# DiltheyLab/HLA-LA

Measured on AMD Instinct MI355X. Metric: paired reads/sec aligned to PRG graph, higher is better.
Workload: dtype int32

## Files before the change

hla-la_amd/csrc/batch.h:

```cpp
#pragma once
#include "device_common.h"

namespace hlala {

struct DevBatch {
    int n_pairs, n_reads, n_chains, stride;
    int from_seeds;
    int unpaired;
    const int* read_off;
    const uint8_t* read_bases;
    const uint8_t* read_quals;
    const int* chain_off;
    const int* read_primary;
    const int* chain_read;
    const int* chain_contig;
    const int* chain_pos;
    const int* chain_offset;
    const int* chain_as;
    const uint8_t* chain_reverse;
    const int* cigar_off;
    const u32* cigar;
    int* seed_status;
    int* seed_ncols;
    int* seed_begin;
    int* seed_end;
    int* seed_removed;
    int* seed_level;
    int* seed_edge;
    uint8_t* seed_g;
    uint8_t* seed_s;
    int* ext_status;
    int* ext_ncols;
    int* ext_begin;
    int* ext_end;
    double* ext_ll;
    int* dp_iters;
    int* dp_score;
    int* dp_ncols;
    int* dp_sb;
    int* dp_se;
    int* dp_err;
    int* dp_alias_head;
    int* dp_alias_next;
    int* ext_level;
    int* ext_edge;
    uint8_t* ext_g;
    uint8_t* ext_s;
    uint8_t* ext_fromseed;
    int* ext_firstlast;
    int* pair_status;
    int* best_chain;
    int* n_comb;
    double* pair_ll;
    double* pair_mapq;
    double* mate_mapq;
    uint8_t* strands_valid;
    uint8_t* sel_mapq;
    u64* counters;
    int* work_counter;
    int* retry_list;
    int* pair_multi;
    uint8_t* pair_deferred;
    int* chain_order;
    int* chain_bucket;
    int* order_hist;
    int order_shift, order_nb;
    int long_chunk_nodes, long_max_segs;
    int order_cost;
    int* chain_row;
    int n_rows;
    int* dp_blk;
    int* dp_list;
    int dp_nblk;
    int dp_band;
    int dp_band_risky;
    int dp_jf;
    void* dp_items;
    int* dbg;
};

__device__ __forceinline__ int ordered_chains(const DevBatch& B) { return B.chain_order ? __builtin_amdgcn_readfirstlane(B.order_hist[B.order_nb - 1]) : B.n_chains; }

__device__ __forceinline__ size_t row_base(const DevBatch& B, int c) { return (size_t)(B.chain_row ? B.chain_row[c] : c) * (size_t)B.stride; }

enum { DPL_BAND16 = 0, DPL_BAND32 = 2, DPL_BAND64 = 4, DPL_JF = 6, DPL_GEN = 8, DPL_N = 10 };
__host__ __device__ inline int dpl_of_class(int cls) { return cls == 0 ? DPL_GEN : (cls == 1 ? DPL_JF : (cls == 2 ? DPL_BAND16 : (cls == 3 ? DPL_BAND32 : DPL_BAND64))); }
enum { WC_PAIR_MULTI = 40, WC_BAND_FETCH = 48, WC_FO_COUNT = 54, WC_FO_FETCH = 56, WC_BAND_FAILED = 58, WC_BAND_CALLS = 59, WC_JF_FAILED = 60, WC_BAND_WHY = 62, WC_BAND_TIED = 68,
       WC_N = 88 };
constexpr int BAND_MAXJ16 = 15, BAND_MAXJ32 = 31, BAND_MAXJ64 = 48;

enum {
    CNT_CHAINS_EXT = 0, CNT_DP_CALLS, CNT_DP_ITERS, CNT_DP_CELLS, CNT_SEED_COLS, CNT_OUT_COLS, CNT_EDGES, CNT_ERRORS, CNT_DP_SHARED
};

}
```

hla-la_amd/csrc/device_common.h:

```cpp
#pragma once
#include <hip/hip_runtime.h>
#include <stdint.h>

namespace hlala {

typedef unsigned long long u64;
typedef unsigned int u32;

struct DevGraph {
    int L, N, E, P;
    const int* level_off;
    const int* node_level;
    const int* node_orig;
    const int* out_off;
    const int* out_to;
    const uint8_t* out_label;
    const int* out_eid;
    const int* in_off;
    const int* in_from;
    const uint8_t* in_label;
    const int* in_eid;
    const unsigned int* in_rec;
    const uint8_t* level_fast;
    const int* edge_from_new;
    const int* edge_to_new;
    const uint8_t* edge_label;
    const int* jf_off; const int* jf_node; const int* jf_path; const int* jf_lvl;
    const int* jb_off; const int* jb_node; const int* jb_path; const int* jb_lvl;
    const uint8_t* out_prank; const uint8_t* in_prank; const uint8_t* jf_prank; const uint8_t* jb_prank;
    const uint8_t* jfree_out; const uint8_t* jfree_in;
    const u32* lin_label; const uint8_t* lin_out; const uint8_t* lin_in; const int* lin_eid;
    const int4* nrec_out;
    const int4* nrec_in;
    const int* path_len;
    const long long* path_off;
    const int* path_edges;
    const uint8_t* gap_stretch;
    const long long* lp_off;
    const int* lp_seqid;
    const int* lp_pos;
};

struct DevTables {
    double ll_match[256];
    double ll_mismatch[256];
    double rate_indel;
    double rate_ins_quarter;
    double rate_match_mismatch;
    double is_penalty;
    int    is_dmin, is_n;
    const double* is_logpdf;
    double phred_thr[256];
    double pcorrect[256];
};

constexpr int DP_WCAP      = 128;
constexpr int DP_HC        = 512;
constexpr int DP_SEQCAP    = 1024;
constexpr int DP_CELLS     = 16384;
constexpr int DP_EARLY     = 4096;
constexpr int DP_STEPS     = 8192;
constexpr int DP_COMPLETED = 2048;
constexpr int DP_CELLS_LARGE     = 65536;
constexpr int DP_COMPLETED_LARGE = 16384;
constexpr int DP_MAX_PARALLEL = 127;
constexpr int DP_NEG       = -30000;

__device__ __forceinline__ int lane_id() { return threadIdx.x & 63; }
#define HLALA_AS_GLOBAL __attribute__((address_space(1)))
template <class T> struct GPtr {
    typedef HLALA_AS_GLOBAL T GT;
    T* p;
    __device__ __forceinline__ GPtr& operator=(T* q) { p = q; return *this; }
    __device__ __forceinline__ GT* g() const { return (GT*)p; }
    __device__ __forceinline__ GT& operator[](int i) const { return g()[i]; }
    __device__ __forceinline__ GT& operator[](unsigned i) const { return g()[i]; }
    __device__ __forceinline__ GT& operator[](long long i) const { return g()[i]; }
    __device__ __forceinline__ GT& operator[](size_t i) const { return g()[i]; }
    __device__ __forceinline__ operator GT*() const { return g(); }
};
template <class T> __device__ __forceinline__ HLALA_AS_GLOBAL T* glob(T* p) { return (HLALA_AS_GLOBAL T*)p; }
#define WSYNC() do { __builtin_amdgcn_fence(__ATOMIC_RELEASE, "wavefront"); __builtin_amdgcn_wave_barrier(); __builtin_amdgcn_fence(__ATOMIC_ACQUIRE, "wavefront"); } while(0)
__device__ __forceinline__ int uni(int v) { return __builtin_amdgcn_readfirstlane(v); }
__device__ __forceinline__ int next_work(int* counter)
{
    int w = 0;
    if(lane_id() == 0) w = atomicAdd(counter, 1);
    return __builtin_amdgcn_readfirstlane(w);
}

template <int CTRL>
__device__ __forceinline__ int dpp_mov(int oldv, int v) { return __builtin_amdgcn_update_dpp(oldv, v, CTRL, 0xF, 0xF, false); }
#define HLALA_DPP_REDUCE(v, IDENT, OP)                                                     \
    do {                                                                                    \
        int t_;                                                                             \
        t_ = dpp_mov<0x111>(IDENT, v); v = OP(v, t_);                        \
        t_ = dpp_mov<0x112>(IDENT, v); v = OP(v, t_);                        \
        t_ = dpp_mov<0x114>(IDENT, v); v = OP(v, t_);                        \
        t_ = dpp_mov<0x118>(IDENT, v); v = OP(v, t_);                        \
        t_ = __builtin_amdgcn_update_dpp(IDENT, v, 0x142, 0xA, 0xF, false); v = OP(v, t_);   \
        t_ = __builtin_amdgcn_update_dpp(IDENT, v, 0x143, 0xC, 0xF, false); v = OP(v, t_);   \
    } while(0)
__device__ __forceinline__ int op_max_(int a, int b) { return a > b ? a : b; }
__device__ __forceinline__ int op_add_(int a, int b) { return a + b; }
__device__ __forceinline__ int wave_max_i32(int v)
{
    HLALA_DPP_REDUCE(v, (int)0x80000000, op_max_);
    return __builtin_amdgcn_readlane(v, 63);
}
__device__ __forceinline__ int wave_sum_i32(int v)
{
    HLALA_DPP_REDUCE(v, 0, op_add_);
    return __builtin_amdgcn_readlane(v, 63);
}
__device__ __forceinline__ u64 wave_min_u64(u64 v)
{
    int hi = (int)(~(u32)(v >> 32) ^ 0x80000000u);
    int mh = wave_max_i32(hi);
    int lo = (hi == mh) ? (int)(~(u32)v ^ 0x80000000u) : (int)0x80000000;
    int ml = wave_max_i32(lo);
    return ((u64)(~((u32)mh ^ 0x80000000u)) << 32) | (u64)(~((u32)ml ^ 0x80000000u));
}
__device__ inline double exp_cr_nonpos(double x)
{
#pragma clang fp contract(off)
    if(!(x < 0.0)) return 1.0;
    if(x < -700.0) return exp(x);
    const double n = rint(x * 0x1.71547652b82fep+0);
    const double r0 = fma(-n, 0x1.62e42fee00000p-1, x);
    const double t1 = n * 0x1.a39ef35600000p-33;
    double rh = r0 - t1; double bb = rh - r0; double rl = (r0 - (rh - bb)) + (-t1 - bb);
    const double t2 = n * 0x1.93c7673007e5fp-65;
    { double s = rh - t2; double b2 = s - rh; double e = (rh - (s - b2)) + (-t2 - b2); e += rl; rh = s + e; rl = e - (rh - s); }
    const double ch[25] = {0x1.0000000000000p+0, 0x1.0000000000000p+0, 0x1.0000000000000p-1, 0x1.5555555555555p-3, 0x1.5555555555555p-5, 0x1.1111111111111p-7, 0x1.6c16c16c16c17p-10,
        0x1.a01a01a01a01ap-13, 0x1.a01a01a01a01ap-16, 0x1.71de3a556c734p-19, 0x1.27e4fb7789f5cp-22, 0x1.ae64567f544e4p-26, 0x1.1eed8eff8d898p-29, 0x1.6124613a86d09p-33,
        0x1.93974a8c07c9dp-37, 0x1.ae7f3e733b81fp-41, 0x1.ae7f3e733b81fp-45, 0x1.952c77030ad4ap-49, 0x1.6827863b97d97p-53, 0x1.2f49b46814157p-57, 0x1.e542ba4020225p-62,
        0x1.71b8ef6dcf572p-66, 0x1.0ce396db7f853p-70, 0x1.761b41316381ap-75, 0x1.f2cf01972f578p-80};
    const double cl[25] = {0.0, 0.0, 0.0, 0x1.5555555555555p-57, 0x1.5555555555555p-59, 0x1.1111111111111p-63, -0x1.f49f49f49f49fp-65, 0x1.a01a01a01a01ap-73, 0x1.a01a01a01a01ap-76,
        -0x1.c154f8ddc6c00p-73, 0x1.cbbc05b4fa99ap-76, -0x1.c062e06d1f209p-80, -0x1.2aec959e14c06p-83, 0x1.f28e0cc748ebep-87, 0x1.05d6f8a2efd1fp-92, 0x1.1d8656b0ee8cbp-97,
        0x1.1d8656b0ee8cbp-101, 0x1.ac981465ddc6cp-103, 0x1.eec01221a8b0bp-107, 0x1.2650f61dbdcb4p-112, 0x1.ea72b4afe3c2fp-120, -0x1.d043ae40c4647p-120, -0x1.aebcdbd20331cp-124,
        -0x1.3423c7d91404fp-130, -0x1.9ada5fcc1ab14p-135};
    double ph = ch[24], pl = cl[24];
#pragma unroll
    for(int k = 23; k >= 0; k--) {
        const double m = ph * rh; double e = fma(ph, rh, -m); e = fma(ph, rl, e); e = fma(pl, rh, e);
        double mh = m + e; double ml = e - (mh - m);
        const double s = mh + ch[k]; const double b2 = s - mh; double e2 = (mh - (s - b2)) + (ch[k] - b2); e2 += ml + cl[k];
        ph = s + e2; pl = e2 - (ph - s);
    }
    return ldexp(ph, (int)n);
}

__device__ __forceinline__ unsigned long long wave_sum_u64(unsigned long long v)
{
    for(int o = 32; o > 0; o >>= 1) {
        const unsigned lo = (unsigned)__shfl_xor((int)(unsigned)v, o), hi = (unsigned)__shfl_xor((int)(unsigned)(v >> 32), o);
        v += ((unsigned long long)hi << 32) | lo;
    }
    return v;
}

__device__ __forceinline__ int wave_incl_scan_add(int v) { HLALA_DPP_REDUCE(v, 0, op_add_); return v; }
__device__ __forceinline__ int wave_incl_scan_max(int v) { HLALA_DPP_REDUCE(v, (int)0x80000000, op_max_); return v; }
__device__ __forceinline__ int wave_excl_scan(int v, int& total)
// ... 31 lines not shown
```

hla-la_amd/csrc/hlala_api.hip:

```cpp
#include <cmath>
#include <cstdio>
#include <cstring>
#include <cstdlib>
#include <algorithm>
#include <map>
#include <mutex>
#include <chrono>
#include <thread>
#include <set>
#include <string>
#include <unordered_map>
#include <vector>

#include "../../include/hlala_gpu.h"
#include "batch.h"
#include "flat_graph.hpp"
#include "host_internal.h"

#include "kernel_dp.hip"
#include "kernel_project.hip"
#include "kernel_order.hip"
#include "kernel_pair.hip"
#include "kernel_typer.hip"
#include "kernel_call.hip"
// ... 739 lines not shown
    for(int k = 0; k < nc; k++) {
        int n = in->col_off[k + 1] - in->col_off[k];
        if(in->chain_read[k] < 0 || in->chain_read[k] >= nr) { c->err = "chain_read out of range"; return fail(HLALA_E_ARG); }
        if(n > stride || n < 1) { st[k] = HLALA_CHAIN_ERR_COLUMNS; ncols[k] = 0; continue; }
        ncols[k] = n;
        for(int j = 0; j < n; j++) {
            size_t o = (size_t)k * stride + j; int i = in->col_off[k] + j;
            lev[o] = in->col_level[i]; edg[o] = in->col_edge[i]; g[o] = in->col_gchar[i]; s[o] = in->col_schar[i];
        }
    }
    HIP_TRY_F(c, hipMemcpyAsync(B.seed_status, st.data(), (size_t)nc * 4, hipMemcpyHostToDevice, c->active), fail);
    HIP_TRY_F(c, hipMemcpyAsync(B.seed_ncols, ncols.data(), (size_t)nc * 4, hipMemcpyHostToDevice, c->active), fail);
    HIP_TRY_F(c, hipMemcpyAsync(B.seed_begin, in->chain_seq_begin, (size_t)nc * 4, hipMemcpyHostToDevice, c->active), fail);
    HIP_TRY_F(c, hipMemcpyAsync(B.seed_end, in->chain_seq_end, (size_t)nc * 4, hipMemcpyHostToDevice, c->active), fail);
    HIP_TRY_F(c, hipMemcpyAsync(B.seed_level, lev.data(), lev.size() * 4, hipMemcpyHostToDevice, c->active), fail);
    HIP_TRY_F(c, hipMemcpyAsync(B.seed_edge, edg.data(), edg.size() * 4, hipMemcpyHostToDevice, c->active), fail);
    HIP_TRY_F(c, hipMemcpyAsync(B.seed_g, g.data(), g.size(), hipMemcpyHostToDevice, c->active), fail);
    HIP_TRY_F(c, hipMemcpyAsync(B.seed_s, s.data(), s.size(), hipMemcpyHostToDevice, c->active), fail);
    HIP_TRY_F(c, hipStreamSynchronize(c->active), fail);
    b->staged = 1; b->outputs_ready = true;
    *out = b;
    return HLALA_OK;
}

int hlala_batch_set_first_chain(hlala_batch* b, uint32_t first_chain)
{
    if(!b) return HLALA_E_ARG;
    b->first_chain = first_chain;
    return HLALA_OK;
}

void hlala_batch_destroy(hlala_batch* b)
{
    if(!b) return;
    hlala_ctx* c = b->ctx;
    DEV_GUARD(c);
    if(c) {
        if(b->tail_pooled) (void)flush_tail(c);
        c->tail.erase(std::remove(c->tail.begin(), c->tail.end(), b), c->tail.end());
        c->batches.erase(b);
        if(b->side_inflight) (void)hipEventSynchronize(b->evDone);
        if(b->mainValid) (void)hipEventSynchronize(b->evMain);
        for(void* p : b->allocs) pool_release(c, p);
    } else for(void* p : b->allocs) if(p) (void)hipFree(p);
    if(b->evDone) (void)hipEventDestroy(b->evDone);
    if(b->evMain) (void)hipEventDestroy(b->evMain);
    for(int i = 0; i < 14; i++) { if(b->ev[i]) (void)hipEventDestroy(b->ev[i]); if(b->evC[i / 2][i % 2]) (void)hipEventDestroy(b->evC[i / 2][i % 2]); }
    for(int i = 0; i < 8; i++) if(b->evSide[i]) (void)hipEventDestroy(b->evSide[i]);
    if(b->evJF) (void)hipEventDestroy(b->evJF);
    for(int i = 0; i < 2; i++) if(b->evBand[i]) (void)hipEventDestroy(b->evBand[i]);
    delete b;
}

static int check_launch(hlala_ctx* c, const char* what)
{
    hipError_t e = hipGetLastError();
    if(e != hipSuccess) { c->err = std::string(what) + ": " + hipGetErrorString(e); return HLALA_E_DEVICE; }
    return 0;
}

int hlala_project_chains(hlala_ctx* c, hlala_batch* b)
{
    DEV_GUARD(c);
    if(!c || !b) return HLALA_E_ARG;
    { int rj = join_side(c, b); if(rj) return rj; }
    if(b->B.from_seeds) { c->err = "batch was created from seeds: stage A not available"; return HLALA_E_STATE; }
    { int re = batch_events(c, b); if(re) return re; }
    { int ro = ensure_outputs(c, b); if(ro) return ro; }
    DevBatch& B = b->B;
    HIP_TRY(c, hipMemsetAsync(B.work_counter, 0, WC_N * sizeof(int), c->active));
    HIP_TRY(c, hipMemsetAsync(B.counters, 0, 32 * sizeof(u64), c->active));
    HIP_TRY(c, hipEventRecord(b->ev[0], c->active));
    if(B.n_chains > 0) {
        int threads = 256, blocks = (B.n_reads + threads - 1) / threads;
        if(!b->prepared && B.order_hist) HIP_TRY(c, hipMemsetAsync(B.order_hist, 0, ((size_t)B.order_nb + 1) * sizeof(int), c->active));
        if(!b->prepared) hipLaunchKernelGGL(k_filter_chains, dim3(blocks), dim3(threads), 0, c->active, c->dG, b->dB, c->d_contig_off, c->d_contig_level);
        if(!b->prepared && B.order_hist) {
            hipLaunchKernelGGL(k_order_scan, dim3(1), dim3(ORDER_SCAN_THREADS), 0, c->active, B.order_hist, B.order_nb);
            hipLaunchKernelGGL(k_order_scatter, dim3((B.n_chains + 255) / 256), dim3(256), 0, c->active, b->dB);
            int rco = check_launch(c, "k_order_scatter"); if(rco) return rco;
        }
        int grid = B.n_chains < c->proj_grid ? B.n_chains : c->proj_grid;
        if(c->proj_long_slabs)
            hipLaunchKernelGGL((k_project_chains<ProjLdsLong>), dim3(grid), dim3(64), 0, c->active, c->dG, b->dB, c->d_contig_off, c->d_contig_seq, c->d_contig_level,
                               c->proj_slabs, c->proj_slab_bytes, c->proj_long_slabs, c->proj_long_slab_bytes, 0);
        else
            if(c->params.max_columns <= PROJ_CAP_SHORT)
                hipLaunchKernelGGL((k_project_chains<ProjLdsShort>), dim3(grid), dim3(64), 0, c->active, c->dG, b->dB, c->d_contig_off, c->d_contig_seq, c->d_contig_level,
                                   c->proj_slabs, c->proj_slab_bytes, (char*)nullptr, (size_t)0, c->rethread_slabs ? 1 : 0);
            else
                hipLaunchKernelGGL((k_project_chains<ProjLds>), dim3(grid), dim3(64), 0, c->active, c->dG, b->dB, c->d_contig_off, c->d_contig_seq, c->d_contig_level,
                               c->proj_slabs, c->proj_slab_bytes, (char*)nullptr, (size_t)0, c->rethread_slabs ? 1 : 0);
        int rc = check_launch(c, "k_project_chains"); if(rc) return rc;
        if(c->rethread_slabs) {
            hipLaunchKernelGGL(k_rethread_chains, dim3(c->rethread_grid), dim3(64), 0, c->active, c->dG, b->dB, c->rethread_slabs, c->rethread_slab_bytes);
            rc = check_launch(c, "k_rethread_chains"); if(rc) return rc;
        }
    }
    HIP_TRY(c, hipEventRecord(b->ev[1], c->active));
    b->staged |= 1;
    return mark_main(c, b);
}

static int extend_impl(hlala_ctx* c, hlala_batch* b, bool fused, int phase = 0);
int hlala_extend_chains(hlala_ctx* c, hlala_batch* b) { return extend_impl(c, b, false); }

static int extend_impl(hlala_ctx* c, hlala_batch* b, bool fused, int phase)
{
    DEV_GUARD(c);
    if(!c || !b) return HLALA_E_ARG;
    if(!(b->staged & 1)) { c->err = "hlala_extend_chains before seed chains exist"; return HLALA_E_STATE; }
    const bool sidePartOnly = phase == 2 || phase == 4;
    if(!sidePartOnly) { int rj = join_side(c, b); if(rj) return rj; }
    { int re = batch_events(c, b); if(re) return re; }
    DevBatch& B = b->B;
    if(B.unpaired || B.from_seeds || B.n_pairs <= 0 || B.n_chains <= 0) { fused = false; if(sidePartOnly) return HLALA_OK; phase = 0; }
    const bool mainPart = !sidePartOnly;
    if(mainPart) {
    b->side_used = false; b->side_pending = false;
    if(B.n_pairs > 0) HIP_TRY(c, hipMemsetAsync(B.pair_deferred, 0, (size_t)B.n_pairs, c->active));
    HIP_TRY(c, hipMemsetAsync(B.work_counter + 1, 0, sizeof(int), c->active));
    HIP_TRY(c, hipMemsetAsync(B.work_counter + 4, 0, (WC_N - 4) * sizeof(int), c->active));
    if(B.from_seeds) HIP_TRY(c, hipMemsetAsync(B.counters, 0, 32 * sizeof(u64), c->active));
    HIP_TRY(c, hipEventRecord(b->ev[2], c->active));
    }
    if(B.n_chains > 0) {
        DpItem* items = (DpItem*)B.dp_items;
        const u32 seed = c->params.rng_seed + 2u * b->first_chain;
        int rc = 0;
        if(mainPart) {
        HIP_TRY(c, hipMemsetAsync(B.dp_alias_head, 0xFF, (size_t)2 * B.n_chains * sizeof(int), c->active));
        HIP_TRY(c, hipMemsetAsync(B.dp_alias_next, 0xFF, (size_t)2 * B.n_chains * sizeof(int), c->active));
        HIP_TRY(c, hipMemsetAsync(B.dp_blk, 0, ((size_t)DPL_N * B.dp_nblk + 1) * sizeof(int), c->active));
        hipLaunchKernelGGL(k_dp_items, dim3(B.dp_nblk), dim3(256), 0, c->active, c->dG, b->dB, items);
        rc = check_launch(c, "k_dp_items"); if(rc) return rc;
        hipLaunchKernelGGL(k_order_scan, dim3(1), dim3(ORDER_SCAN_THREADS), 0, c->active, B.dp_blk, DPL_N * B.dp_nblk + 1);
        hipLaunchKernelGGL(k_dp_lists, dim3(B.dp_nblk), dim3(256), 0, c->active, b->dB, (const DpItem*)items);
        rc = check_launch(c, "k_dp_lists"); if(rc) return rc;
        }
        hipStream_t ws = c->active;
        const DpPoolArgs noPool{};
        DpPoolArgs one{}; one.n = 1; one.seed[0] = seed; one.B[0] = b->dB; one.items[0] = items; one.bases[0] = (const uint8_t*)B.read_bases;
        auto run_class = [&](int tier) -> int {
            if(fused && tier == DP_SIDE_TIER) {
                if(!b->evDone) HIP_TRY(c, hipEventCreateWithFlags(&b->evDone, hipEventDisableTiming));
                HIP_TRY(c, hipEventRecord(b->evSide[0], c->active)); HIP_TRY(c, hipStreamWaitEvent(c->side, b->evSide[0], 0));
                ws = c->side;
                HIP_TRY(c, hipEventRecord(b->evSide[1], c->side));
            }
            if(!fused && tier == DP_SIDE_TIER && c->sideTailValid) HIP_TRY(c, hipStreamWaitEvent(c->stream, c->evSideTail, 0));
            HIP_TRY(c, hipEventRecord(b->evC[tier][0], ws));
            switch(tier) {
            case 0: {
                hipLaunchKernelGGL((k_dp<DpTinyJF, 0>), dim3(c->jf_grid), dim3(DpTinyJF::THREADS), 0, ws, c->dG, b->dB, items, c->tiny_slabs, c->tiny_slab_bytes, seed, c->G.nrec_out, c->G.nrec_in, B.read_bases, noPool);
                int rcj = check_launch(c, "k_dp<DpTinyJF>"); if(rcj) return rcj;
                HIP_TRY(c, hipEventRecord(b->evJF, ws));
                hipLaunchKernelGGL((k_dp<DpTiny, 0>), dim3(c->tiny_grid), dim3(DpTiny::THREADS), 0, ws, c->dG, b->dB, items, c->tiny_slabs, c->tiny_slab_bytes, seed, c->G.nrec_out, c->G.nrec_in, B.read_bases, noPool); break; }
            case 1: hipLaunchKernelGGL((k_dp<DpMid, 1>), dim3(c->mid_grid), dim3(DpMid::THREADS), 0, ws, c->dG, b->dB, items, c->mid_slabs, c->mid_slab_bytes, seed, c->G.nrec_out, c->G.nrec_in, B.read_bases, noPool); break;
            case 2: hipLaunchKernelGGL((k_dp<DpSmall, 2>), dim3(c->ext_grid), dim3(DpSmall::THREADS), 0, ws, c->dG, b->dB, items, c->ext_slabs, c->ext_slab_bytes, seed, c->G.nrec_out, c->G.nrec_in, B.read_bases, noPool); break;
            case 3: hipLaunchKernelGGL((k_dp<DpWide, 3>), dim3(c->wide_grid), dim3(DpWide::THREADS), 0, ws, c->dG, b->dB, items, c->wide_slabs, c->ext_slab_bytes, seed, c->G.nrec_out, c->G.nrec_in, B.read_bases, noPool); break;
            case 4: hipLaunchKernelGGL((k_dp<DpBroad, 4>), dim3(c->broad_grid), dim3(DpBroad::THREADS), 0, ws, c->dG, b->dB, items, c->large_slabs, c->large_slab_bytes, seed, c->G.nrec_out, c->G.nrec_in, B.read_bases, one); break;
            case 5: hipLaunchKernelGGL((k_dp<DpLarge, 5>), dim3(c->retry_grid), dim3(DpLarge::THREADS), 0, ws, c->dG, b->dB, items, c->large_slabs + c->large_slab_bytes * (size_t)c->broad_grid, c->large_slab_bytes, seed, c->G.nrec_out, c->G.nrec_in, B.read_bases, one); break;
            default: hipLaunchKernelGGL((k_dp<DpHuge, 6>), dim3(c->huge_grid), dim3(DpHuge::THREADS), 0, ws, c->dG, b->dB, items, c->huge_slabs, c->huge_slab_bytes, seed, c->G.nrec_out, c->G.nrec_in, B.read_bases, one); break;
            }
            int rc_ = check_launch(c, "k_dp"); if(rc_) return rc_;
            HIP_TRY(c, hipEventRecord(b->evC[tier][1], ws));
            return 0;
        };
        if(mainPart) {
        b->band_used = c->band_grid > 0;
        if(b->band_used) {
            HIP_TRY(c, hipEventRecord(b->evBand[0], c->active));
            hipLaunchKernelGGL((k_dp_band<16>), dim3(c->band_grid), dim3(64), 0, c->active, c->dG, b->dB, (const DpItem*)items, seed, (const uint8_t*)B.read_bases, c->G.lin_label, c->G.lin_eid);
            hipLaunchKernelGGL((k_dp_band<32>), dim3(c->band_grid), dim3(64), 0, c->active, c->dG, b->dB, (const DpItem*)items, seed, (const uint8_t*)B.read_bases, c->G.lin_label, c->G.lin_eid);
            hipLaunchKernelGGL((k_dp_band<64>), dim3(c->band_grid), dim3(64), 0, c->active, c->dG, b->dB, (const DpItem*)items, seed, (const uint8_t*)B.read_bases, c->G.lin_label, c->G.lin_eid);
            rc = check_launch(c, "k_dp_band"); if(rc) return rc;
            HIP_TRY(c, hipEventRecord(b->evBand[1], c->active));
        }
        HIP_TRY(c, hipEventRecord(b->ev[7], c->active));
        rc = run_class(0); if(rc) return rc;
        HIP_TRY(c, hipEventRecord(b->ev[6], c->active));
        }
        for(int tier = 1; tier <= DP_LAST_TIER; tier++) {
            if(phase == 4) break;
            if(phase == 1 && tier >= DP_SIDE_TIER) break;
            if(phase == 2 && tier < DP_SIDE_TIER) continue;
            if(phase == 3 && tier >= DP_POOL_TIER) break;
            rc = run_class(tier); if(rc) return rc;
            if(tier == 2) HIP_TRY(c, hipEventRecord(b->ev[10], c->active));
        }
        if(!fused) HIP_TRY(c, hipEventRecord(b->ev[8], c->active));
        const int sgrid = B.n_chains < c->stitch_grid ? B.n_chains : c->stitch_grid;
        if(fused && phase == 1) b->side_pending = true;
        if(fused && phase == 3) { b->side_pending = true; b->side_used = true; }
        if(fused && phase != 1 && phase != 3) {
            { const int pgrid = (B.n_pairs + 63) / 64, cap = c->stitch_grid / 20;
              hipLaunchKernelGGL(k_stitch_chains, dim3(pgrid < cap ? (pgrid > 0 ? pgrid : 1) : cap), dim3(64), 0, c->side, c->dG, c->dT, b->dB, (const uint8_t*)B.pair_deferred, 2, 0, 0); }
            rc = check_launch(c, "k_stitch_chains (side)"); if(rc) return rc;
            HIP_TRY(c, hipEventRecord(b->evDone, c->side));
            HIP_TRY(c, hipEventRecord(c->evSideTail, c->side)); c->sideTailValid = true;
            b->side_inflight = true; b->side_used = true; b->side_pending = true;
        }
        if(mainPart) {
        hipLaunchKernelGGL(k_stitch_chains, dim3(sgrid), dim3(64), 0, c->active, c->dG, c->dT, b->dB, (const uint8_t*)B.pair_deferred, fused ? 1 : 0, c->stitch_draw, c->stitch_by_row);
        rc = check_launch(c, "k_stitch_chains"); if(rc) return rc;
        }
    }
    if(sidePartOnly) return HLALA_OK;
    HIP_TRY(c, hipEventRecord(b->ev[3], c->active));
    b->staged |= 2;
    return mark_main(c, b);
}

static int pair_impl(hlala_ctx* c, hlala_batch* b, int phase);
int hlala_pair_chains(hlala_ctx* c, hlala_batch* b) { return pair_impl(c, b, 0); }
static int pair_impl(hlala_ctx* c, hlala_batch* b, int phase)
{
    DEV_GUARD(c);
    if(!c || !b) return HLALA_E_ARG;
    if(b->B.from_seeds) { c->err = "batch was created from seeds: stage C not available"; return HLALA_E_STATE; }
    if(!(b->staged & 2)) { c->err = "hlala_pair_chains before hlala_extend_chains"; return HLALA_E_STATE; }
    { int re = batch_events(c, b); if(re) return re; }
    DevBatch& B = b->B;
    const bool fused = b->side_pending;
    if(!fused) { if(phase == 2) return HLALA_OK; phase = 0; }
    if(!fused) { int rj = join_side(c, b); if(rj) return rj; }
    if(phase != 2) {
    HIP_TRY(c, hipMemsetAsync(B.work_counter + 2, 0, sizeof(int), c->active));
    HIP_TRY(c, hipEventRecord(b->ev[4], c->active));
    }
    if(B.n_pairs > 0) {
        const int grid = B.n_pairs < c->pair_grid ? B.n_pairs : c->pair_grid;
        auto launch_pair = [&](hipStream_t st, int mode, int counterIdx) -> int {
            const int pass = st == c->side ? 1 : 0, multiBase = WC_PAIR_MULTI + 4 * pass;
            int* multiList = B.pair_multi + (size_t)pass * 2 * (size_t)B.n_pairs;
            double* scratch = c->pair_scratch + (pass ? (size_t)c->pair_grid * PAIR_COMB : 0);
            if(!fused) HIP_TRY(c, hipMemsetAsync(B.work_counter + multiBase, 0, 4 * sizeof(int), st));
            const int lean = B.n_pairs < c->pair_lean_grid ? B.n_pairs : c->pair_lean_grid;
            const int g0 = mode == 2 ? (grid < c->pair_grid / 5 ? grid : c->pair_grid / 5) : grid, g1 = grid < c->pair_grid / 5 ? grid : c->pair_grid / 5;
            if(B.unpaired) {
                hipLaunchKernelGGL((k_pair_chains<true>), dim3(lean), dim3(64), 0, st, c->dG, c->dT, b->dB, (const uint8_t*)B.pair_deferred, mode, counterIdx, multiList, multiBase);
                hipLaunchKernelGGL((k_pair_multi<true, false>), dim3(g0), dim3(64), 0, st, c->dG, c->dT, b->dB, (const int*)multiList, multiBase, scratch);
                hipLaunchKernelGGL((k_pair_multi<true, true>), dim3(g1), dim3(64), 0, st, c->dG, c->dT, b->dB, (const int*)multiList, multiBase, scratch);
            } else {
                hipLaunchKernelGGL((k_pair_chains<false>), dim3(lean), dim3(64), 0, st, c->dG, c->dT, b->dB, (const uint8_t*)B.pair_deferred, mode, counterIdx, multiList, multiBase);
                hipLaunchKernelGGL((k_pair_multi<false, false>), dim3(g0), dim3(64), 0, st, c->dG, c->dT, b->dB, (const int*)multiList, multiBase, scratch);
                hipLaunchKernelGGL((k_pair_multi<false, true>), dim3(g1), dim3(64), 0, st, c->dG, c->dT, b->dB, (const int*)multiList, multiBase, scratch);
            }
            return check_launch(c, "k_pair_chains / k_pair_multi");
        };
        int rc = 0;
        if(phase != 2) { rc = launch_pair(c->active, fused ? 1 : 0, 2); if(rc) return rc; }
        if(fused && phase != 1) {
            rc = launch_pair(c->side, 2, 37); if(rc) return rc;
            HIP_TRY(c, hipEventRecord(b->evSide[6], c->side));
            HIP_TRY(c, hipEventRecord(b->evDone, c->side));
            HIP_TRY(c, hipEventRecord(c->evSideTail, c->side)); c->sideTailValid = true;
            b->side_inflight = true; b->side_pending = false;
        }
    }
    if(phase == 2) return HLALA_OK;
    HIP_TRY(c, hipEventRecord(b->ev[5], c->active));
    b->staged |= 4;
    return mark_main(c, b);
}

static int flush_tail(hlala_ctx* c)
{
    if(c->tail.empty()) return HLALA_OK;
    DEV_GUARD(c);
    std::vector<hlala_batch*> pool; pool.swap(c->tail);
    for(hlala_batch* b : pool) b->tail_pooled = false;
    DpPoolArgs a{}; a.n = (int)pool.size();
    for(int i = 0; i < a.n; i++) { hlala_batch* b = pool[i]; a.seed[i] = c->params.rng_seed + 2u * b->first_chain; a.B[i] = b->dB; a.items[i] = (const DpItem*)b->B.dp_items; a.bases[i] = (const uint8_t*)b->B.read_bases; }
    const hipStream_t ws = c->side;
    for(int tier = DP_POOL_TIER; tier <= DP_LAST_TIER; tier++) {
        for(hlala_batch* b : pool) HIP_TRY(c, hipEventRecord(b->evC[tier][0], ws));
        hlala_batch* b0 = pool[0];
        switch(tier) {
        case 4: hipLaunchKernelGGL((k_dp<DpBroad, 4>), dim3(c->broad_grid), dim3(DpBroad::THREADS), 0, ws, c->dG, b0->dB, (DpItem*)b0->B.dp_items, c->large_slabs, c->large_slab_bytes, a.seed[0], c->G.nrec_out, c->G.nrec_in, b0->B.read_bases, a); break;
        case 5: hipLaunchKernelGGL((k_dp<DpLarge, 5>), dim3(c->retry_grid), dim3(DpLarge::THREADS), 0, ws, c->dG, b0->dB, (DpItem*)b0->B.dp_items, c->large_slabs + c->large_slab_bytes * (size_t)c->broad_grid, c->large_slab_bytes, a.seed[0], c->G.nrec_out, c->G.nrec_in, b0->B.read_bases, a); break;
        default: hipLaunchKernelGGL((k_dp<DpHuge, 6>), dim3(c->huge_grid), dim3(DpHuge::THREADS), 0, ws, c->dG, b0->dB, (DpItem*)b0->B.dp_items, c->huge_slabs, c->huge_slab_bytes, a.seed[0], c->G.nrec_out, c->G.nrec_in, b0->B.read_bases, a); break;
        }
        int rc_ = check_launch(c, "k_dp (pooled)"); if(rc_) return rc_;
        for(hlala_batch* b : pool) HIP_TRY(c, hipEventRecord(b->evC[tier][1], ws));
    }
    for(hlala_batch* b : pool) {
        int rc = extend_impl(c, b, true, 4); if(rc) return rc;
        rc = pair_impl(c, b, 2); if(rc) return rc;
    }
    return HLALA_OK;
}

int hlala_set_tail_pool(hlala_ctx* c, int k)
{
    if(!c || k < 1 || k > DP_POOL_MAX) { if(c) c->err = "hlala_set_tail_pool: k must be 1 .. " + std::to_string(DP_POOL_MAX); return HLALA_E_ARG; }
    if(k < (int)c->tail.size() || k == 1) { int rf = flush_tail(c); if(rf) return rf; }
    c->tail_pool_k = k;
    return HLALA_OK;
}
int hlala_flush(hlala_ctx* c)
{
    if(!c) return HLALA_E_ARG;
    return flush_tail(c);
}

int hlala_align_batch(hlala_ctx* c, hlala_batch* b)
{
    int rc = hlala_project_chains(c, b); if(rc) return rc;
    if(c->tail_pool_k > 1 && DP_POOL_TIER > DP_SIDE_TIER) {
        rc = extend_impl(c, b, true, 3); if(rc) return rc;
        if(!b->side_pending) return hlala_pair_chains(c, b);
        rc = pair_impl(c, b, 1); if(rc) return rc;
        c->tail.push_back(b); b->tail_pooled = true;
        if((int)c->tail.size() >= c->tail_pool_k) return flush_tail(c);
        return HLALA_OK;
    }
    if(!c->side_after_pair) {
        rc = extend_impl(c, b, true); if(rc) return rc;
        return hlala_pair_chains(c, b);
    }
    rc = extend_impl(c, b, true, 1); if(rc) return rc;
    rc = pair_impl(c, b, 1); if(rc) return rc;
    rc = extend_impl(c, b, true, 2); if(rc) return rc;
    return pair_impl(c, b, 2);
}

int hlala_batch_get_chains(hlala_ctx* c, hlala_batch* b, int stage, hlala_chains_out* o)
{
    DEV_GUARD(c);
// ... 1211 lines not shown
```

hla-la_amd/csrc/kernel_dp.hip:

```cpp
#include "batch.h"
#include "../../include/hlala_gpu.h"

namespace hlala {

enum { K_DIAG = 0, K_GGAP = 1, K_SGAP = 2, K_HOP = 3, K_JUMP = 4 };
enum { M_D = 0, M_GG = 1, M_SG = 2 };
enum { PH_IDLE = 0, PH_RUN, PH_SELECT, PH_BT, PH_EXPAND, PH_DONE };

constexpr u64 HKEY_EMPTY = ~0ull;
#ifndef HLALA_DP_PROFILE_LOG2
#define HLALA_DP_PROFILE_LOG2 18
#endif
#ifndef HLALA_EARLY_GEN_MAX
#define HLALA_EARLY_GEN_MAX 0xFFFFFE
#endif
constexpr int DP_EARLY_GEN_MAX = HLALA_EARLY_GEN_MAX;
constexpr int EXT_PENDING = 0x7FFFFFFF;
constexpr int DP_BT_STEPS_PER_TRIP = 32;

#ifndef HLALA_DP_TAIL_THREADS
#define HLALA_DP_TAIL_THREADS 128
#endif
constexpr int DP_TAIL_THREADS = HLALA_DP_TAIL_THREADS;
#ifndef HLALA_DP_TINY_WAVES
// ... 387 lines not shown
    u32 h = early_hash<C>(key);
    const u64 w = early_word(gen, key);
    for(int probe = 0; probe < C::EARLY; probe++) {
        u64 cur = __hip_atomic_load(&sl.early_key()[h], __ATOMIC_RELAXED, __HIP_MEMORY_SCOPE_AGENT);
        if(cur == w) return __hip_atomic_load(&sl.early_val()[h], __ATOMIC_RELAXED, __HIP_MEMORY_SCOPE_AGENT);
        if((int)(cur >> 40) != gen) return -1;
        h = (h + 1) & (C::EARLY - 1);
    }
    return -1;
}
template <class C>
__device__ inline bool early_insert(const DpSlabT<C>& sl, int gen, u64 key, int slot)
{
    u32 h = early_hash<C>(key);
    const u64 w = early_word(gen, key);
    for(int probe = 0; probe < C::EARLY; probe++) {
        u64 cur = __hip_atomic_load(&sl.early_key()[h], __ATOMIC_RELAXED, __HIP_MEMORY_SCOPE_AGENT);
        while((int)(cur >> 40) != gen) {
            const u64 old = atomicCAS(&sl.early_key()[h], cur, w);
            if(old == cur) { cur = w; break; }
            cur = old;
        }
        if(cur == w) { __hip_atomic_store(&sl.early_val()[h], slot, __ATOMIC_RELAXED, __HIP_MEMORY_SCOPE_AGENT); return true; }
        h = (h + 1) & (C::EARLY - 1);
    }
    return false;
}

__device__ inline int dec_len(int v) { int n = 1; while(v >= 10) { v /= 10; n++; } return n; }
__device__ inline int pow10i(int n) { int p = 1; while(n-- > 0) p *= 10; return p; }
__device__ __forceinline__ int dec_len_cmp(int v)
{
    return 1 + (v >= 10) + (v >= 100) + (v >= 1000) + (v >= 10000) + (v >= 100000) + (v >= 1000000) + (v >= 10000000) + (v >= 100000000) + (v >= 1000000000);
}
__device__ __forceinline__ u32 pow10_u32(int k)
{
    u32 p = (k & 1) ? 10u : 1u;
    if(k & 2) p *= 100u;
    if(k & 4) p *= 10000u;
    if(k & 8) p *= 100000000u;
    return p;
}
__device__ __forceinline__ int xz_part(int a, int b)
{
    if(a == b) return 0;
    const int la = dec_len_cmp(a), lb = dec_len_cmp(b);
    u64 A = (u64)(u32)a, Bv = (u64)(u32)b;
    if(la < lb) A *= (u64)pow10_u32(lb - la); else if(lb < la) Bv *= (u64)pow10_u32(la - lb);
    if(A != Bv) return A < Bv ? -1 : 1;
    return la < lb ? -1 : 1;
}
__device__ __forceinline__ bool xz_less(int x1, int z1, int x2, int z2)
{
    const int c = xz_part(x1, x2);
    if(c) return c < 0;
    return xz_part(z1, z2) < 0;
}

__device__ inline u64 xz_key(int x, int z)
{
    const int lx = dec_len(x), lz = dec_len(z);
    u64 k = 0; int n = 0;
    for(int i = 0; i < lx; i++, n++) k = k * 12 + (u64)(2 + (x / pow10i(lx - 1 - i)) % 10);
    k = k * 12 + 1; n++;
    for(int i = 0; i < lz && n < 14; i++, n++) k = k * 12 + (u64)(2 + (z / pow10i(lz - 1 - i)) % 10);
    for(; n < 14; n++) k *= 12;
    return k;
}

struct __align__(16) DpItem { int item, rOff, seqLen, start_seq, startLevel, startNode, pad0, pad1; };

#ifndef HLALA_DP_SIDE_TIER
#define HLALA_DP_SIDE_TIER 3
#endif
constexpr int DP_SIDE_TIER = HLALA_DP_SIDE_TIER;
constexpr int DP_LAST_TIER = 6;
constexpr int DP_POOL_TIER = DP_SIDE_TIER > 4 ? DP_SIDE_TIER : 4;
constexpr int DP_POOL_MAX = 8;
__device__ __forceinline__ int tier_for_frontier(int n) { return n <= DpMid::WCAP ? 1 : (n <= DpSmall::WCAP ? 2 : (n <= DpWide::WCAP ? 3 : (n <= DpBroad::WCAP ? 4 : (n <= DpLarge::WCAP ? 5 : 6)))); }
__device__ __forceinline__ int tier_for_targets(int n) { return n <= (DpMid::HC * 3) / 4 ? 1 : (n <= (DpSmall::HC * 3) / 4 ? 2 : (n <= (DpWide::HC * 3) / 4 ? 3 : (n <= (DpBroad::HC * 3) / 4 ? 4 : (n <= (DpLarge::HC * 3) / 4 ? 5 : 6)))); }

#define DP_FAIL(code) do { if(gl == 0 && S.err == 0) S.err = (code); } while(0)

template <class C>
__device__ inline int dp_begin(DpLdsT<C>& S, const DpSlabT<C>& sl, const DevGraph& G, const DpItem& it, int itemIdx)
{
    constexpr int GW = C::GW;
    const int gl = grp_lane<GW>();
    for(int i = gl; i < C::HC; i += GW) { S.hkey[i] = HKEY_EMPTY; S.hbest[0][i] = 0; S.hbest[1][i] = 0; S.hbest[2][i] = 0; }
    if(gl == 0) {
        DpState& st = S.st;
        st.itemIdx = itemIdx;
        st.item = it.item; st.rOff = it.rOff; st.seqLen = it.seqLen; st.start_seq = it.start_seq; st.startLevel = it.startLevel; st.startNode = it.startNode;
        st.diagonals = it.seqLen + G.L - 1;
        st.d = 1; st.b1 = 0; st.b2 = 1; st.n1 = 1; st.n2 = 0; st.nCells = 1; st.nCompleted = 0;
        st.curMax = 0; st.firstMaxSlot = 0; st.lastInc = 0; st.earlyInit = 0; st.earlyMaxNat = -1; st.itersRun = 0;
        st.cellsEvaluated = 0;
        st.endSlot = -1; st.endScore = 0; st.nSteps = 0; st.nCols = 0;
        st.have = 0; st.sb = 0; st.se = -1; st.err = 0; st.needTier = 0; st.isAlias = 0;
        S.err = 0; S.nTa = 0; S.jumpMet = 0;
#ifdef HLALA_DP_PROFILE
        S.pfStart = clock64(); S.pfSlow = 0; S.pfImp = 0; S.pfPre = 0; S.pfMaxNT = 0; S.pfMaxF = 0; for(int i = 0; i < 16; i++) S.pfPh[i] = 0;
#endif
        CellRec c0; c0.key = mk_key(it.startLevel, it.start_seq, it.startNode);
        c0.sc[0] = 0; c0.sc[1] = (short)DP_NEG; c0.sc[2] = (short)DP_NEG; c0.sc[3] = 0; c0.bt[0] = 0; c0.bt[1] = 0; c0.bt[2] = 0; c0.pad = 0;
        sl.cell()[0] = c0;
        S.fkey[0][0] = mk_key(it.startLevel, it.start_seq, it.startNode); S.fslot[0][0] = 0;
        S.fD[0][0] = 0; S.fG[0][0] = (short)DP_NEG; S.fS[0][0] = (short)DP_NEG;
    }
    DSYNC();
    return PH_RUN;
}

template <class C>
__device__ inline int dp_iterate(DpLdsT<C>& S, const DpSlabT<C>& sl, const DevGraph& G, const int4* nrec, const uint8_t* readBases, const bool fwd, int& edgesAcc, u64* sortScratch)
{
    constexpr int GW = C::GW;
    const int gl = grp_lane<GW>();
    DpState& st = S.st;
    const int dir = fwd ? 1 : -1;
    const int seqLen = guni<GW>(st.seqLen);
    const int max_levelI = G.L - 1, max_seqI = seqLen;
    const int limitY = fwd ? seqLen : 0;
    const int d = guni<GW>(st.d);
    const int n1 = guni<GW>(st.n1), n2 = guni<GW>(st.n2);
    const int b1 = guni<GW>(st.b1), b2 = guni<GW>(st.b2), bn = b2;
    const int lastInc0 = guni<GW>(st.lastInc), diagonals = guni<GW>(st.diagonals);
    const uint8_t* seqp = readBases + guni<GW>(st.rOff);

    if(d > diagonals || (d - lastInc0) > 40) return PH_SELECT;
    if(n1 == 0 && n2 == 0) {
        int last = lastInc0 + 40; if(last > diagonals) last = diagonals;
        if(gl == 0) st.itersRun = last;
        DSYNC();
        return PH_SELECT;
    }
    if(d > 60000) { if(gl == 0) { st.itersRun = d; st.err = __LINE__; } DSYNC(); return PH_DONE; }

#if defined(HLALA_DP_TIMING)
    long long tq0 = clock64();
#define DP_TQ(i) do { __builtin_amdgcn_s_waitcnt(0); long long t_ = clock64(); if(gl == 0) S.tPh[i] += t_ - tq0; tq0 = t_; } while(0)
#elif defined(HLALA_DP_PROFILE)
    long long tq0 = clock64();
#define DP_TQ(i) do { __builtin_amdgcn_s_waitcnt(0); long long t_ = clock64(); if(gl == 0) S.pfPh[i] += t_ - tq0; tq0 = t_; } while(0)
#else
#define DP_TQ(i) do { } while(0)
#endif
    const int* eoff = fwd ? G.out_off : G.in_off; const int* eto = fwd ? G.out_to : G.in_from; const uint8_t* elab = fwd ? G.out_label : G.in_label;
    const int* joff = fwd ? G.jf_off : G.jb_off; const int* jnode = fwd ? G.jf_node : G.jb_node; const int* jlvl = fwd ? G.jf_lvl : G.jb_lvl;
    const uint8_t* eprk = fwd ? G.out_prank : G.in_prank; const uint8_t* jprk = fwd ? G.jf_prank : G.jb_prank;
    int edges = 0;
    const int nMax = n1 > n2 ? n1 : n2;
    constexpr bool APPEND = (GW >= 64) && (C::WCAP > 64);
    typedef typename TlistT<(C::HC <= 256)>::type TlT;
    int nTa = 0;
    auto append = [&](const bool claimed, const u32 h) {
        if constexpr (APPEND && GW == 64) {
            const u64 m = __ballot(claimed);
            if(claimed) S.tlist[nTa + (int)__builtin_amdgcn_mbcnt_hi((u32)(m >> 32), __builtin_amdgcn_mbcnt_lo((u32)m, 0u))] = (TlT)h;
            nTa += __popcll(m);
        } else if constexpr (APPEND) {
            const u64 m = __ballot(claimed);
            if(m) {
                int base = 0;
                if(lane_id() == 0) base = atomicAdd(&S.nTa, (int)__popcll(m));
                base = __builtin_amdgcn_readfirstlane(base);
                const int pos = base + (int)__builtin_amdgcn_mbcnt_hi((u32)(m >> 32), __builtin_amdgcn_mbcnt_lo((u32)m, 0u));
                if(claimed && pos < C::HC) S.tlist[pos] = (TlT)h;
            }
        }
    };
    for(int i = gl; i < nMax; i += GW) {
        const bool hasA = i < n2, hasB = i < n1;
        u64 pkA = hasA ? S.fkey[b2][i] : 0, pkB = hasB ? S.fkey[b1][i] : 0;
        const int pxA = key_x(pkA), pyA = key_y(pkA), nodeA = key_node(pkA);
        const int pxB = key_x(pkB), pyB = key_y(pkB), nodeB = key_node(pkB);
        const int nxA = pxA + dir, nyA = pyA + dir;
        const bool doA = hasA && !(nxA > max_levelI || nyA > max_seqI || nxA < 0 || nyA < 0);
        const int pDA = hasA ? (int)S.fD[b2][i] : 0;
        const int pD = hasB ? (int)S.fD[b1][i] : 0, pG = hasB ? (int)S.fG[b1][i] : 0, pS = hasB ? (int)S.fS[b1][i] : 0;
        int4 ra0 = make_int4(0, 0, 0, 0), ra1 = ra0, rb0 = ra0, rb1 = ra0; unsigned char rc = 0;
        if(doA) { ra0 = nrec[2 * (size_t)nodeA]; ra1 = nrec[2 * (size_t)nodeA + 1]; rc = fwd ? seqp[pyA] : seqp[pyA - 1]; }
        if(hasB) { rb0 = nrec[2 * (size_t)nodeB]; rb1 = nrec[2 * (size_t)nodeB + 1]; }
        const int a0 = ra0.x, degA = ra0.y & 0xFFFF, tnA0 = ra0.z, tnA1 = ra0.w;
        const unsigned char labA0 = (unsigned char)(ra1.w & 0xFF), labA1 = (unsigned char)((ra1.w >> 8) & 0xFF);
        const int rkA1 = (ra1.w >> 16) & 1, rkB1 = (rb1.w >> 16) & 1;
        const int e0 = rb0.x, degB = rb0.y & 0xFFFF, tnB0 = rb0.z, tnB1 = rb0.w;
        const int j0 = rb1.x, j1 = j0 + (int)((u32)rb0.y >> 16), jn0 = rb1.y, jx0 = rb1.z;
        const unsigned char labB0 = (unsigned char)(rb1.w & 0xFF), labB1 = (unsigned char)((rb1.w >> 8) & 0xFF);
        DP_TQ(4);
        const int ord0 = (1 << (C::IBITS + 8)) | (i << 8);
        const int nyG = pyB + dir, nxB = pxB + dir;
        const bool okA = doA, okB = hasB;
        const bool sgB = okB && nxB >= 0 && nxB <= max_levelI;
        typedef typename C::Best BestT;
        {
            bool cv[3]; u64 ck[3]; u32 ch[3]; u64 cold[3];
            cv[0] = okA && degA > 0; ck[0] = mk_key(nxA, nyA, tnA0);
// ... 360 lines not shown
        for(int t = gl; t < nT; t += GW) { int h = S.tlist[t]; if((u32)S.hbest[0][h] != 0xFFFFFFFFu) { int v = (short)((u32)S.hbest[1][h] & 0xFFFF); mx = max(mx, v); } }
        mx = grp_max_i32<GW>(mx);
    }
    int nNew = 0;
    for(int t0 = 0; t0 < nT; t0 += GW) {
        int t = t0 + gl;
        bool pass = false; u64 key = 0; int h = 0;
        if(t < nT) { h = S.tlist[t]; key = S.hkey[h]; if((u32)S.hbest[0][h] != 0xFFFFFFFFu) { int v = (short)((u32)S.hbest[1][h] & 0xFFFF); pass = (mx - v) <= 15; } }
        int passTot; const int pos = nNew + grp_rank<GW>(pass, passTot);
        if(pass && pos < C::WCAP) {
            S.fkey[bn][pos] = key; S.fslot[bn][pos] = (typename C::Slot)(int)S.hbest[0][h];
            S.fD[bn][pos] = (short)((u32)S.hbest[1][h] & 0xFFFF); S.fG[bn][pos] = (short)((u32)S.hbest[1][h] >> 16); S.fS[bn][pos] = (short)((u32)S.hbest[2][h] & 0xFFFF);
        }
        nNew += passTot;
    }
    if(nNew > C::WCAP) { if(gl == 0) { st.itersRun = d; st.err = __LINE__; st.needTier = tier_for_frontier(nNew); } DSYNC(); return PH_DONE; }
    DSYNC();
    const bool wideSort = C::WCAP > GW && nNew > GW;
    if(wideSort) for(int t = gl; t < nT; t += GW) { int h = S.tlist[t]; S.hkey[h] = HKEY_EMPTY; S.hbest[0][h] = 0; S.hbest[1][h] = 0; S.hbest[2][h] = 0; }
    if(nNew > 1 && nNew <= GW) {
        const bool act = gl < nNew;
        u64 key = 0; typename C::Slot vs = 0; short vD = 0, vG = 0, vS = 0; int rank = 0;
        if(act) {
            key = S.fkey[bn][gl]; vs = S.fslot[bn][gl]; vD = S.fD[bn][gl]; vG = S.fG[bn][gl]; vS = S.fS[bn][gl];
            for(int u = 0; u < nNew; u++) rank += (S.fkey[bn][u] < key) ? 1 : 0;
        }
        DSYNC();
        if(act) { S.fkey[bn][rank] = key; S.fslot[bn][rank] = vs; S.fD[bn][rank] = vD; S.fG[bn][rank] = vG; S.fS[bn][rank] = vS; }
    } else if(wideSort) {
        DSYNC();
        int Pn = GW * 2; while(Pn < nNew) Pn <<= 1;
        u64* keys; u64* pay;
        if constexpr (C::IN_MEMORY) {
            if(Pn <= DP_SORT_SCRATCH) { keys = sortScratch; pay = sortScratch + DP_SORT_SCRATCH; }
            else { keys = sl.sort_spill(); pay = keys + C::WCAP; }
        } else { keys = &S.fkey[bn][0]; pay = (u64*)&S.hbest[2][0]; }
        auto enc = [](int v) -> u64 { return v == DP_NEG ? 0ull : (u64)(u32)(v + 64); };
        auto dec = [](u64 e) -> short { return e == 0 ? (short)DP_NEG : (short)((int)e - 64); };
        for(int i = gl; i < Pn; i += GW) {
            if(i < nNew) {
                pay[i] = ((u64)(u32)(int)S.fslot[bn][i] << 36) | (enc(S.fD[bn][i]) << 24) | (enc(S.fG[bn][i]) << 12) | enc(S.fS[bn][i]);
                if constexpr (C::IN_MEMORY) keys[i] = S.fkey[bn][i];
            } else { keys[i] = ~0ull; pay[i] = 0; }
        }
        DSYNC();
        for(int k = 2; k <= Pn; k <<= 1)
            for(int j = k >> 1; j > 0; j >>= 1) {
                for(int idx = gl; idx < (Pn >> 1); idx += GW) {
                    const int i = ((idx & ~(j - 1)) << 1) | (idx & (j - 1)), l = i | j;
                    const bool up = (i & k) == 0;
                    const u64 ka = keys[i], kb = keys[l];
                    if((ka > kb) == up) { const u64 pa = pay[i], pb = pay[l]; keys[i] = kb; keys[l] = ka; pay[i] = pb; pay[l] = pa; }
                }
                if constexpr (C::IN_MEMORY) { if(Pn <= DP_SORT_SCRATCH) { if constexpr (GW > 64) blk_barrier(); else { WSYNC(); } } else DSYNC(); }
                else DSYNC();
            }
        for(int i = gl; i < Pn; i += GW) {
            const u64 pv = pay[i];
            if(i < nNew) {
                S.fD[bn][i] = dec((pv >> 24) & 0xFFF); S.fG[bn][i] = dec((pv >> 12) & 0xFFF); S.fS[bn][i] = dec(pv & 0xFFF); S.fslot[bn][i] = (typename C::Slot)(int)(pv >> 36);
                if constexpr (C::IN_MEMORY) S.fkey[bn][i] = keys[i];
            }
            if constexpr (!C::IN_MEMORY) pay[i] = 0;
        }
    }
    DSYNC();
    if(!wideSort) for(int t = gl; t < nT; t += GW) { int h = S.tlist[t]; S.hkey[h] = HKEY_EMPTY; S.hbest[0][h] = 0; S.hbest[1][h] = 0; S.hbest[2][h] = 0; }
    if(gl == 0) {
        st.b2 = b1; st.b1 = bn;
        st.n2 = n1; st.n1 = nNew;
        st.d = d + 1; st.itersRun = d;
        st.nCells = nCells; st.nCompleted = nCompletedNew; st.earlyInit = earlyInit; st.earlyMaxNat = earlyMaxNat;
        st.curMax = curMax; st.lastInc = lastInc; if(firstMaxSlot >= 0) st.firstMaxSlot = firstMaxSlot;
        st.cellsEvaluated += (u32)nT;
#ifdef HLALA_DP_PROFILE
        if(slow) S.pfSlow++; S.pfImp += S.nImp; if(prepass) S.pfPre++; if(nT > S.pfMaxNT) S.pfMaxNT = nT; if(nNew > S.pfMaxF) S.pfMaxF = nNew;
#endif
    }
    DSYNC();
    DP_TQ(2);
    return PH_RUN;
}

template <class C>
__device__ inline int dp_select_many(const DpSlabT<C>& sl, const DevGraph& G, int nCompleted, int best, int selectedIndex)
{
    constexpr int GW = C::GW;
    const int gl = grp_lane<GW>();
    int found = -1;
    int nt = 0;
    for(int i0 = 0; i0 < nCompleted; i0 += GW) {
        int i = i0 + gl; bool tie = false; int s = 0; u64 kk = 0;
        if(i < nCompleted) { s = sl.completed()[i]; if(sl.cell()[s].sc[0] == best) { tie = true; u64 k = sl.cell()[s].key; kk = xz_key(key_x(k), key_node(k) - G.level_off[key_x(k)]); } }
        int tieTot; const int rk = grp_rank<GW>(tie, tieTot);
        if(tie) { const int pos = nt + rk; sl.tie_slot()[pos] = s; sl.tie_key()[pos] = kk; }
        nt += tieTot;
    }
    dp_sync<C>();
    u64 prefix = 0; int k = selectedIndex;
    for(int bit = 51; bit >= 0; bit--) {
        int cnt = 0;
        for(int i = gl; i < nt; i += GW) { const u64 kk = sl.tie_key()[i]; if((kk >> (bit + 1)) == (prefix >> (bit + 1)) && !((kk >> bit) & 1ull)) cnt++; }
        cnt = grp_sum_i32<GW>(cnt);
        if(k >= cnt) { k -= cnt; prefix |= 1ull << bit; }
    }
    for(int i = gl; i < nt; i += GW) if(sl.tie_key()[i] == prefix) found = sl.tie_slot()[i];
    return found;
}

template <class C>
__device__ inline int dp_select(DpLdsT<C>& S, const DpSlabT<C>& sl, const DevGraph& G, u32 rng_seed, const bool fwd)
{
    constexpr int GW = C::GW;
    const int gl = grp_lane<GW>();
    DpState& st = S.st;
    const int nCompleted = guni<GW>(st.nCompleted);
    const u32 seed = rng_seed + (u32)guni<GW>(st.item);
    const int curMax = guni<GW>(st.curMax), firstMaxSlot = guni<GW>(st.firstMaxSlot), start_seq = guni<GW>(st.start_seq);
    int endSlot = -1, endScore = 0;
    if(GW <= 64 && nCompleted > 0 && nCompleted <= GW) {
        int s = -1, sc0 = DP_NEG; u64 k = 0;
        if(gl < nCompleted) { s = sl.completed()[gl]; const CellRec* cr = sl.cell() + s; sc0 = cr->sc[0]; k = cr->key; }
        const int best = grp_max_i32<GW>(sc0);
        const bool tie = gl < nCompleted && sc0 == best;
        const int nTies = grp_sum_i32<GW>(tie ? 1 : 0);
        u32 sd = seed;
        const int selectedIndex = glibc_rand_r(&sd) % nTies;
        int found = -1;
        if(nTies == 1) { if(tie) found = s; }
        else {
            const int kx = key_x(k), kz = tie ? key_node(k) - G.level_off[kx] : 0;
            const int l0 = (int)(lane_id() & ~(u32)(GW - 1));
            int rank = 0;
            for(int u = 0; u < nCompleted; u++) {
                const int ux = __shfl(kx, l0 + u), uz = __shfl(kz, l0 + u), ut = __shfl(tie ? 1 : 0, l0 + u);
                if(ut && u != gl && xz_less(ux, uz, kx, kz)) rank++;
            }
            if(tie && rank == selectedIndex) found = s;
        }
        endSlot = grp_max_i32<GW>(found); endScore = best;
    } else if(nCompleted > 0) {
        int best = DP_NEG;
        for(int i = gl; i < nCompleted; i += GW) best = max(best, (int)sl.cell()[sl.completed()[i]].sc[0]);
        best = grp_max_i32<GW>(best);
        int nTies = 0;
        for(int i = gl; i < nCompleted; i += GW) if(sl.cell()[sl.completed()[i]].sc[0] == best) nTies++;
        nTies = grp_sum_i32<GW>(nTies);
        u32 sd = seed;
        int selectedIndex = glibc_rand_r(&sd) % nTies;
        int found = -1;
        if(C::WCAP <= 64 || nTies <= 2 * GW) {
            for(int i0 = 0; i0 < nCompleted; i0 += GW) {
                int i = i0 + gl;
                if(i < nCompleted) {
                    int s = sl.completed()[i];
                    if(sl.cell()[s].sc[0] == best) {
                        u64 k = sl.cell()[s].key; int rank = 0;
                        if(nTies > 1) {
                            int kz = key_node(k) - G.level_off[key_x(k)];
                            for(int u = 0; u < nCompleted; u++) { int su = sl.completed()[u]; if(su != s && sl.cell()[su].sc[0] == best) { u64 ku = sl.cell()[su].key;
                                if(xz_less(key_x(ku), key_node(ku) - G.level_off[key_x(ku)], key_x(k), kz)) rank++; } }
                        }
                        if(rank == selectedIndex) found = s;
                    }
                }
            }
        } else if constexpr (C::WCAP > 64) found = dp_select_many<C>(sl, G, nCompleted, best, selectedIndex);
        endSlot = grp_max_i32<GW>(found); endScore = best;
    } else if(curMax > 0) {
        endSlot = firstMaxSlot; endScore = sl.cell()[firstMaxSlot].sc[0];
    }
    if(endSlot < 0) return PH_DONE;
    u64 ek = sl.cell()[endSlot].key;
    const int yEnd = key_y(ek);
    if(gl == 0) {
        st.endSlot = endSlot; st.endScore = endScore;
        if(fwd) { st.sb = start_seq; st.se = yEnd - 1; }
        else { st.sb = yEnd; st.se = start_seq - 1; }
        S.btSlot = endSlot; S.btM = 0; S.btX = key_x(ek); S.btY = yEnd; S.btGuard = 0; S.btDone = 0; S.nNew = 0; S.nKeepF = 0;
    }
    DSYNC();
    return PH_BT;
}

template <class C>
__device__ inline int dp_backtrace(DpLdsT<C>& S, const DpSlabT<C>& sl, int maxSteps, const bool fwd)
{
    constexpr int GW = C::GW;
    const int gl = grp_lane<GW>();
    DpState& st = S.st;
    const int dir = fwd ? 1 : -1;
    if(gl == 0) {
        const int startLevel = st.startLevel, start_seq = st.start_seq;
        int slot = S.btSlot, m = S.btM, x = S.btX, y = S.btY, guardSteps = S.btGuard;
        int nSteps = S.nNew, nCols = S.nKeepF;
        int done = 0;
        for(int it = 0; it < maxSteps; it++) {
            if(!((x != startLevel || y != start_seq) && nSteps < C::STEPS && guardSteps++ < 4 * C::STEPS)) { done = 1; break; }
            const CellRec* cr = sl.cell() + slot;
            u32 b = cr->bt[m]; const u64 ckey = cr->key;
            int kind = bt_kind(b);
            int prev = bt_prev(b);
            int px = 0;
            if(kind == K_JUMP) px = key_x(sl.cell()[prev].key);
            if(kind != K_HOP) {
                int len = 1;
                if(kind == K_JUMP) len = px > x ? px - x : x - px;
                sl.step_bt()[nSteps] = b; sl.step_xy()[nSteps] = ckey; nSteps++; nCols += len;
            }
            if(kind == K_DIAG) { x -= dir; y -= dir; }
            else if(kind == K_GGAP) { y -= dir; }
            else if(kind == K_SGAP) { x -= dir; }
            else if(kind == K_JUMP) { x = px; }
            slot = prev; m = bt_src(b);
        }
        if(!done && !(x != startLevel || y != start_seq)) done = 1;
        S.btSlot = slot; S.btM = m; S.btX = x; S.btY = y; S.btGuard = guardSteps; S.nNew = nSteps; S.nKeepF = nCols;
        if(done) {
            if(nSteps >= C::STEPS || guardSteps >= 4 * C::STEPS) st.err = __LINE__;
            st.nSteps = nSteps; st.nCols = nCols;
        }
        S.btDone = done;
    }
    DSYNC();
    if(guni<GW>(S.btDone)) return guni<GW>(st.err) ? PH_DONE : PH_EXPAND;
    return PH_BT;
}

template <class C>
__device__ inline int dp_expand(DpLdsT<C>& S, const DpSlabT<C>& sl, const DevGraph& G, const DevBatch& B, const int4* nrec, const bool fwd)
{
    constexpr int GW = C::GW;
    const int gl = grp_lane<GW>();
    DpState& st = S.st;
    const int nSteps = guni<GW>(st.nSteps), nCols = guni<GW>(st.nCols);
    const int stride = B.stride;
    const int max_seqI = guni<GW>(st.seqLen);
    const int sb = guni<GW>(st.sb), se = guni<GW>(st.se);
    const uint8_t* seqp = B.read_bases + guni<GW>(st.rOff);
    if(nCols > stride) { if(gl == 0) st.err = -1000000 - nCols; DSYNC(); return PH_DONE; }
    if(sb > se) { if(gl == 0) { st.err = __LINE__; st.have = 0; } DSYNC(); return PH_DONE; }
    if(gl == 0) st.have = 1;
    DSYNC();
    const int c = guni<GW>(st.item) >> 1;
    const int rowOff = fwd ? stride - nCols : sb;
    if(rowOff + nCols > stride) return PH_DONE;
    const size_t cb = row_base(B, c) + rowOff;
    int* oL = B.ext_level + cb; int* oE = B.ext_edge + cb; uint8_t* oG = B.ext_g + cb; uint8_t* oS = B.ext_s + cb;
    int base = 0;
    for(int s0 = 0; s0 < nSteps; s0 += GW) {
        int s = s0 + gl; bool act = s < nSteps;
        u32 b = act ? sl.step_bt()[s] : 0; u64 xy = act ? sl.step_xy()[s] : 0;
        int kind = bt_kind(b);
        int pnode = 0, robj = -1, recLab = -1;
        if(act && kind != K_GGAP) {
            u64 pkey = sl.cell()[bt_prev(b)].key; pnode = key_node(pkey);
            const int node = key_node(xy);
            int j = bt_edge(b);
            const int4 r0 = nrec[2 * (size_t)pnode], r1 = nrec[2 * (size_t)pnode + 1];
            if(kind == K_JUMP) {
                const int* jn = fwd ? G.jf_node : G.jb_node;
                const int nj = (int)((u32)r0.y >> 16); int q = r1.x; const int q1 = q + nj;
                if(!(nj > 0 && r1.y == node && j == 0)) for(; q < q1; q++) if(jn[q] == node && j-- == 0) break;
                if(q < q1) robj = (fwd ? G.jf_path : G.jb_path)[q];
            } else {
                const int* et = fwd ? G.out_to : G.in_from;
                const int deg = r0.y & 0xFFFF; int q = r0.x; const int q1 = q + deg;
                if(deg > 0 && r0.z == node && j == 0) recLab = r1.w & 0xFF;
                else if(deg > 1 && r0.w == node && j == ((r1.w >> 16) & 1)) { q++; recLab = (r1.w >> 8) & 0xFF; }
                else for(; q < q1; q++) if(et[q] == node && j-- == 0) break;
                if(q < q1) robj = (fwd ? G.out_eid : G.in_eid)[q];
            }
            if(robj < 0) { st.err = __LINE__; act = false; }
        }
        int len = act ? (kind == K_JUMP ? G.path_len[robj] : 1) : 0;
        int total; int off = grp_excl_scan<GW>(len, total);
        if(act) {
            int x = key_x(xy), y = key_y(xy);
            int start = fwd ? (nCols - (base + off) - len) : (base + off);
            if(kind == K_JUMP) {
                int p = robj; long long po = G.path_off[p];
                int lvl0 = G.node_level[G.edge_from_new[G.path_edges[po]]];
                for(int j = 0; j < len; j++) { oL[start + j] = lvl0 + j; oE[start + j] = G.path_edges[po + j]; oG[start + j] = '_'; oS[start + j] = '_'; }
            } else {
                int eid = robj;
                unsigned char sc = fwd ? (y >= 1 ? seqp[y - 1] : 0) : (y < max_seqI ? seqp[y] : 0);
                int lvl = fwd ? x - 1 : x;
                const unsigned char gch = kind == K_GGAP ? (unsigned char)'_' : (recLab >= 0 ? (unsigned char)recLab : G.edge_label[eid]);
                if(kind == K_DIAG) { oL[start] = lvl; oE[start] = eid; oG[start] = gch; oS[start] = sc; }
                else if(kind == K_GGAP) { oL[start] = -1; oE[start] = -1; oG[start] = '_'; oS[start] = sc; }
                else { oL[start] = lvl; oE[start] = eid; oG[start] = gch; oS[start] = '_'; }
            }
        }
        base += total;
    }
    return PH_DONE;
}

__device__ inline bool dp_item_for(const DevGraph& G, const DevBatch& B, int c, int d, DpItem& it)
{
    if(B.unpaired) return false;
    if(B.seed_status[c] != HLALA_CHAIN_OK) return false;
    const int r = B.chain_read[c];
    const int rOff = B.read_off[r], seqLen = B.read_off[r + 1] - rOff;
    const int nSeed = B.seed_ncols[c], sBegin = B.seed_begin[c], sEnd = B.seed_end[c];
    if(seqLen > DP_SEQCAP || seqLen < 1 || nSeed < 1 || sBegin < 0 || sEnd >= seqLen || sBegin > sEnd) return false;
    const size_t cb = row_base(B, c);
    const int e0 = B.seed_edge[cb], e1 = B.seed_edge[cb + nSeed - 1];
    if(e0 < 0 || e1 < 0 || e0 >= G.E || e1 >= G.E) return false;
    it.rOff = rOff; it.seqLen = seqLen; it.pad0 = 0; it.pad1 = 0; it.item = 2 * c + d;
    if(d == 0) {
        if(sBegin == 0) return false;
        const int firstNode = G.edge_from_new[e0]; const int lvl = G.node_level[firstNode];
        if(lvl <= 0) return false;
        it.start_seq = sBegin; it.startLevel = lvl; it.startNode = firstNode;
    } else {
        if(sEnd == seqLen - 1) return false;
        const int lastNode = G.edge_to_new[e1]; const int lvl = G.node_level[lastNode];
        if(lvl >= G.L - 1) return false;
        it.start_seq = sEnd + 1; it.startLevel = lvl; it.startNode = lastNode;
    }
    return true;
}

__global__ void k_dp_items(const DevGraph* __restrict__ Gp, const DevBatch* __restrict__ Bp, DpItem* items)
{
    const DevGraph& G = *Gp;
    const DevBatch& B = *Bp;
    const int t = blockIdx.x * blockDim.x + threadIdx.x;
    if(t < B.n_chains) {
        const int st = B.seed_status[t];
        B.dp_iters[2 * t] = 0; B.dp_iters[2 * t + 1] = 0; B.dp_score[2 * t] = INT32_MIN; B.dp_score[2 * t + 1] = INT32_MIN;
        B.dp_ncols[2 * t] = -1; B.dp_ncols[2 * t + 1] = -1; B.dp_err[2 * t] = 0; B.dp_err[2 * t + 1] = 0;
        if(st != HLALA_CHAIN_OK) {
            B.ext_status[t] = st; B.ext_ncols[t] = 0;
            if(st < 0) atomicAdd(&B.counters[CNT_ERRORS], 1ull);
        }
    }
    const int nOrd = ordered_chains(B);
    const int c = t < nOrd ? (B.chain_order ? B.chain_order[t] : t) : -1;
    bool needL = false, needR = false;
    int nShared = 0;
    DpItem itL, itR;
    if(c >= 0 && B.seed_status[c] == HLALA_CHAIN_OK) {
        const int stride = B.stride;
        const int r = B.chain_read[c];
        const int rOff = B.read_off[r], seqLen = B.read_off[r + 1] - rOff;
        const size_t cb = row_base(B, c);
        const int nSeed = B.seed_ncols[c], sBegin = B.seed_begin[c], sEnd = B.seed_end[c];
        int err = 0;
        if((!B.unpaired && seqLen > DP_SEQCAP) || seqLen < 1 || nSeed < 1 || sBegin < 0 || sEnd >= seqLen || sBegin > sEnd) err = HLALA_CHAIN_ERR_INPUT;
        if(!err) {
            const int e0 = B.seed_edge[cb], e1 = B.seed_edge[cb + nSeed - 1];
            if(e0 < 0 || e1 < 0 || e0 >= G.E || e1 >= G.E) err = HLALA_CHAIN_ERR_INPUT;
        }
        if(err) { B.ext_status[c] = err; B.ext_ncols[c] = 0; B.ext_ll[c] = 0.0; atomicAdd(&B.counters[CNT_ERRORS], 1ull); }
        else {
            B.ext_status[c] = EXT_PENDING;
            needL = dp_item_for(G, B, c, 0, itL);
            needR = dp_item_for(G, B, c, 1, itR);
            if(!B.from_seeds && (needL || needR)) {
                for(int c2 = B.chain_off[r]; c2 < c && (needL || needR); c2++) {
                    DpItem o;
                    if(needL && dp_item_for(G, B, c2, 0, o) && o.start_seq == itL.start_seq && o.startNode == itL.startNode) { B.dp_alias_next[2 * c] = atomicExch(&B.dp_alias_head[2 * c2], 2 * c); needL = false; nShared++; }
                    if(needR && dp_item_for(G, B, c2, 1, o) && o.start_seq == itR.start_seq && o.startNode == itR.startNode) { B.dp_alias_next[2 * c + 1] = atomicExch(&B.dp_alias_head[2 * c2 + 1], 2 * c + 1); needR = false; nShared++; }
                }
            }
        }
    }
    bool jfL = false, jfR = false;
    if(needL && B.dp_jf) { const int reach = itL.start_seq + B.dp_jf - 1; jfL = reach < 255 && (int)G.jfree_in[itL.startLevel] > reach; }
    if(needR && B.dp_jf) { const int reach = itR.seqLen - itR.start_seq + B.dp_jf - 1; jfR = reach < 255 && (int)G.jfree_out[itR.startLevel] > reach; }
    bool bdL = false, bdR = false;
    int runL = 0, runR = 0;
    int clsL = jfL ? 1 : 0, clsR = jfR ? 1 : 0;
    if(needL && B.dp_band) { const int jm = itL.start_seq, reach = jm + B.dp_band - 1; runL = (int)G.lin_in[itL.startLevel]; bdL = jm <= BAND_MAXJ64 && runL >= (B.dp_band_risky ? jm : reach + min(jm + 6, 40)); if(bdL) clsL = jm <= BAND_MAXJ16 ? 2 : (jm <= BAND_MAXJ32 ? 3 : 4); }
    if(needR && B.dp_band) { const int jm = itR.seqLen - itR.start_seq, reach = jm + B.dp_band - 1; runR = (int)G.lin_out[itR.startLevel]; bdR = jm <= BAND_MAXJ64 && runR >= (B.dp_band_risky ? jm : reach + min(jm + 6, 40)); if(bdR) clsR = jm <= BAND_MAXJ16 ? 2 : (jm <= BAND_MAXJ32 ? 3 : 4); }
    if(t < nOrd) {
        int4* sl = (int4*)(items + t); int4* sr = (int4*)(items + (size_t)B.n_chains + t);
        if(needL) { sl[0] = make_int4(itL.item, itL.rOff, itL.seqLen, itL.start_seq); sl[1] = make_int4(itL.startLevel, itL.startNode, clsL, runL); } else sl[0] = make_int4(-1, 0, 0, 0);
        if(needR) { sr[0] = make_int4(itR.item, itR.rOff, itR.seqLen, itR.start_seq); sr[1] = make_int4(itR.startLevel, itR.startNode, clsR, runR); } else sr[0] = make_int4(-1, 0, 0, 0);
    }
    __shared__ int blkCnt[DPL_N];
    if(threadIdx.x < DPL_N) blkCnt[threadIdx.x] = 0;
    __syncthreads();
    const int lane = lane_id();
    nShared = wave_sum_i32(nShared);
    if(lane == 0 && nShared) atomicAdd(&B.counters[CNT_DP_SHARED], (u64)nShared);
    const u64 mL = __ballot(needL), mR = __ballot(needR);
    const int kL = needL ? dpl_of_class(clsL) : -1, kR = needR ? dpl_of_class(clsR) + 1 : -1;
    const u64 mJL = __ballot(needL && clsL == 1), mJR = __ballot(needR && clsR == 1), mBL = __ballot(needL && clsL >= 2), mBR = __ballot(needR && clsR >= 2);
    if(lane == 0) {
        if(mL) atomicAdd(&B.work_counter[8], __popcll(mL));
        if(mR) atomicAdd(&B.work_counter[9], __popcll(mR));
        if(mJL | mJR) atomicAdd(&B.work_counter[6], __popcll(mJL) + __popcll(mJR));
        if(mBL | mBR) atomicAdd(&B.work_counter[WC_BAND_CALLS], __popcll(mBL) + __popcll(mBR));
    }
#pragma unroll
    for(int k = 0; k < DPL_N; k++) {
        const u64 mk = __ballot((k & 1) ? kR == k : kL == k);
        if(lane == 0 && mk) atomicAdd(&blkCnt[k], __popcll(mk));
    }
    __syncthreads();
    if(threadIdx.x < DPL_N) B.dp_blk[(size_t)threadIdx.x * gridDim.x + blockIdx.x] = blkCnt[threadIdx.x];
}

__global__ void k_dp_lists(const DevBatch* __restrict__ Bp, const DpItem* __restrict__ items)
{
    const DevBatch& B = *Bp;
    const int t = blockIdx.x * blockDim.x + threadIdx.x;
    const int nOrd = ordered_chains(B);
    int kL = -1, kR = -1;
    if(t < nOrd) {
        const int4* sl = (const int4*)(items + t); const int4* sr = (const int4*)(items + (size_t)B.n_chains + t);
        if(sl[0].x >= 0) kL = dpl_of_class(sl[1].z);
        if(sr[0].x >= 0) kR = dpl_of_class(sr[1].z) + 1;
    }
    __shared__ int waveCnt[DPL_N][4];
    const int lane = lane_id(), wv = (int)(threadIdx.x >> 6);
    u64 m[DPL_N];
#pragma unroll
    for(int k = 0; k < DPL_N; k++) m[k] = __ballot((k & 1) ? kR == k : kL == k);
    if(lane == 0) {
#pragma unroll
        for(int k = 0; k < DPL_N; k++) waveCnt[k][wv] = (int)__popcll(m[k]);
    }
    __syncthreads();
    const u64 below = (1ull << lane) - 1ull;
#pragma unroll
    for(int k = 0; k < DPL_N; k++) {
        const bool mine = (k & 1) ? kR == k : kL == k;
        if(mine) {
            int before = 0;
            for(int w2 = 0; w2 < wv; w2++) before += waveCnt[k][w2];
            const int pos = B.dp_blk[(size_t)k * gridDim.x + blockIdx.x] + before + (int)__popcll(m[k] & below);
            B.dp_list[pos] = (k & 1) ? B.n_chains + t : t;
        }
    }
}

struct DpPoolArgs {
    int n;
    u32 seed[DP_POOL_MAX];
    const DevBatch* B[DP_POOL_MAX];
    const DpItem* items[DP_POOL_MAX];
    const uint8_t* bases[DP_POOL_MAX];
};

template <class C, int TIER>
__device__ __forceinline__ void dp_class_run(const DevGraph& G, const DevBatch& B, const DpItem* __restrict__ items, DpLdsT<C>& S, DpSlabT<C> sl, u64* sortScratch, const u32 rng_seed,
                                             const int4* __restrict__ nrecOut, const int4* __restrict__ nrecIn, const uint8_t* __restrict__ readBases);

template <class C, int TIER>
__global__ __launch_bounds__(C::THREADS, C::WAVES) void k_dp(const DevGraph* __restrict__ Gp, const DevBatch* __restrict__ Bp, const DpItem* __restrict__ items,
                                                        char* slabs, size_t slabBytes, u32 rng_seed,
                                                        const int4* __restrict__ nrecOut, const int4* __restrict__ nrecIn, const uint8_t* __restrict__ readBasesArg, const DpPoolArgs pool)
{
    constexpr int GW = C::GW;
    constexpr int NG = GW >= 64 ? 1 : 64 / GW;
    static_assert(C::THREADS == (GW >= 64 ? GW : 64), "block size");
    const DevGraph& G = *Gp;
    const int g = (int)((threadIdx.x & 63) / GW);
    DpLdsT<C>* Sp; DpSlabT<C> sl; u64* sortScratch = nullptr;
    if constexpr (C::IN_MEMORY) {
        __shared__ u64 scratch[2 * DP_SORT_SCRATCH];
        char* base = slabs + (size_t)blockIdx.x * slabBytes;
        Sp = (DpLdsT<C>*)base; sl.base = base + ((sizeof(DpLdsT<C>) + 255) & ~(size_t)255); sortScratch = scratch;
    } else {
        __shared__ DpLdsT<C> SS[NG];
        Sp = &SS[g]; sl.base = slabs + ((size_t)blockIdx.x * NG + g) * slabBytes;
    }
    if constexpr (TIER >= DP_POOL_TIER) {
        const int nB = __builtin_amdgcn_readfirstlane(pool.n);
        for(int bi = 0; bi < nB; bi++) {
            dp_class_run<C, TIER>(G, *pool.B[bi], pool.items[bi], *Sp, sl, sortScratch, pool.seed[bi], nrecOut, nrecIn, pool.bases[bi]);
            DSYNC();
        }
    } else dp_class_run<C, TIER>(G, *Bp, items, *Sp, sl, sortScratch, rng_seed, nrecOut, nrecIn, readBasesArg);
}

template <class C, int TIER>
__device__ __forceinline__ void dp_class_run(const DevGraph& G, const DevBatch& B, const DpItem* __restrict__ items, DpLdsT<C>& S, DpSlabT<C> sl, u64* sortScratch, const u32 rng_seed,
                                             const int4* __restrict__ nrecOut, const int4* __restrict__ nrecIn, const uint8_t* __restrict__ readBases)
{
    constexpr int GW = C::GW;
    constexpr int NG = GW >= 64 ? 1 : 64 / GW;
#ifndef HLALA_DP_DRAW0
#define HLALA_DP_DRAW0 8
#endif
    constexpr int DRAW = (TIER == 0 && C::JF) ? HLALA_DP_DRAW0 : 1;
    const int gl = grp_lane<GW>();

    if(gl == 0) { S.accCalls = 0; S.accIters = 0; S.accCells = 0; S.accEdges = 0; }
#ifdef HLALA_DP_TIMING
    if(gl == 0) { for(int i = 0; i < 16; i++) S.tPh[i] = 0; }
#endif
#ifdef HLALA_DP_TIMING
    long long tAcc[6] = {0, 0, 0, 0, 0, 0}; long long trips = 0, runGroups = 0; long long tMark = clock64();
#define DP_T(i) do { long long t_ = clock64(); tAcc[i] += t_ - tMark; tMark = t_; } while(0)
#else
#define DP_T(i) do { } while(0)
#endif

    constexpr int NPASS = (TIER == 0 && !C::JF) ? 4 : 2;
    for(int pass = 0; pass < NPASS; pass++) {
        const int dirPass = pass & 1;
        const bool foPass = pass >= 2;
        int* fetchCounter = foPass ? &B.work_counter[WC_FO_FETCH + dirPass]
                          : &B.work_counter[TIER == 0 ? (C::JF ? 4 + dirPass : (dirPass ? 10 : 1)) : 13 + 4 * (TIER - 1) + 2 * dirPass];
        const int seg = (C::JF ? DPL_JF : DPL_GEN) + dirPass;
        const bool dense = TIER == 0 && !foPass;
        const int segStart = dense ? uni(B.dp_blk[(size_t)seg * B.dp_nblk]) : 0;
        const int nItems = dense ? uni(B.dp_blk[(size_t)(seg + 1) * B.dp_nblk]) - segStart
                         : (foPass ? uni(B.work_counter[WC_FO_COUNT + dirPass]) : uni(B.work_counter[12 + 4 * (TIER > 0 ? TIER - 1 : 0) + 2 * dirPass]));
        const int* srcList = dense ? B.dp_list + segStart
                           : (foPass ? B.retry_list + (size_t)(14 + dirPass) * (size_t)B.n_chains
                           : B.retry_list + (size_t)(2 * (TIER > 0 ? TIER - 1 : 0) + dirPass) * (size_t)B.n_chains);
        const bool fwd = dirPass != 0;
        if constexpr (DRAW > 1) { if(gl == 0) { S.chunkNext = 0; S.chunkEnd = 0; } DSYNC(); }
        int phase = PH_IDLE;
        bool more = true;
        int edgesAcc = 0;

        for(;;) {
            if(phase == PH_RUN) phase = dp_iterate<C>(S, sl, G, fwd ? nrecOut : nrecIn, readBases, fwd, edgesAcc, sortScratch);
            DP_T(5);
            if(phase == PH_SELECT) phase = dp_select<C>(S, sl, G, rng_seed, fwd);
            DP_T(4);
            if(phase == PH_BT) phase = dp_backtrace<C>(S, sl, DP_BT_STEPS_PER_TRIP, fwd);
            DP_T(3);
            if(phase == PH_EXPAND) phase = dp_expand<C>(S, sl, G, B, fwd ? nrecOut : nrecIn, fwd);
            DP_T(2);
            if(phase == PH_DONE) {
                const int edges = grp_sum_i32<GW>(edgesAcc);
                if(gl == 0) {
                    DpState& st = S.st;
                    S.nextPhase = PH_IDLE;
#ifdef HLALA_DP_PROFILE
                    if(B.dbg && TIER == HLALA_DP_PROFILE && !C::JF) {
                        const long long cyc = clock64() - S.pfStart;
                        if(cyc > (1ll << HLALA_DP_PROFILE_LOG2) && (HLALA_DP_PROFILE_LOG2 >= 12 || (((u32)st.item * 2654435761u) >> 24) == 0)) { int q = atomicAdd(&B.dbg[0], 1); if(q < 500) { int* r = B.dbg + 16 + 16 * q; r[0] = st.item; r[1] = st.itersRun; r[2] = (int)st.cellsEvaluated; r[3] = st.nCells;
                            r[4] = S.pfSlow; r[5] = S.pfImp; r[6] = S.pfPre; r[7] = (int)(cyc >> 10); r[8] = S.pfMaxNT;
                            r[9] = (int)(S.pfPh[4] >> 10); r[10] = (int)(S.pfPh[5] >> 10); r[11] = (int)(S.pfPh[0] >> 10); r[12] = (int)(S.pfPh[3] >> 10); r[13] = (int)(S.pfPh[6] >> 10); r[14] = (int)(S.pfPh[1] >> 10); r[15] = (int)(S.pfPh[2] >> 10); } }
                    }
#endif
                    const bool capacity = st.err != 0 && st.err > -1000000;
                    bool handed = false;
                    if constexpr (C::JF && TIER == 0) if(capacity && S.jumpMet) {
                        if(st.isAlias) ((int*)(items + st.itemIdx))[0] = st.item;
                        const int q = atomicAdd(&B.work_counter[WC_FO_COUNT + dirPass], 1); B.retry_list[(size_t)(14 + dirPass) * (size_t)B.n_chains + q] = st.itemIdx;
                        atomicAdd(&B.work_counter[WC_JF_FAILED], 1);
                        handed = true;
                    }
                    if(handed) { }
                    else if(capacity && TIER < DP_LAST_TIER) {
                        int to = TIER + 1; if(st.needTier > to) to = st.needTier; if(to > DP_LAST_TIER) to = DP_LAST_TIER;
                        int* cnt = &B.work_counter[12 + 4 * (to - 1) + 2 * dirPass]; int* lst = B.retry_list + (size_t)(2 * (to - 1) + dirPass) * (size_t)B.n_chains;
                        if(st.isAlias) ((int*)(items + st.itemIdx))[0] = st.item;
                        int q = atomicAdd(cnt, 1); lst[q] = st.itemIdx;
                        if(to >= DP_SIDE_TIER && B.n_pairs > 0 && !B.unpaired) B.pair_deferred[B.chain_read[st.item >> 1] >> 1] = 1;
                    } else {
                        const int item = st.item;
                        B.dp_iters[item] = st.itersRun; B.dp_score[item] = st.have ? st.endScore : INT32_MIN;
                        B.dp_ncols[item] = st.have ? st.nCols : -1; B.dp_sb[item] = st.sb; B.dp_se[item] = st.se; B.dp_err[item] = st.err;
                        S.accCalls++; S.accIters += (u64)st.itersRun; S.accCells += (u64)st.cellsEvaluated; S.accEdges += (u64)edges;
                        int nx = B.dp_alias_head[item]; if(nx < 0) nx = B.dp_alias_next[item];
                        const bool failed = st.err != 0 && st.err > -1000000;
                        while(nx >= 0 && failed) {
                            B.dp_iters[nx] = st.itersRun; B.dp_score[nx] = INT32_MIN; B.dp_ncols[nx] = -1; B.dp_sb[nx] = st.sb; B.dp_se[nx] = st.se; B.dp_err[nx] = st.err;
                            S.accCalls++; S.accIters += (u64)st.itersRun; S.accCells += (u64)st.cellsEvaluated; S.accEdges += (u64)edges;
                            nx = B.dp_alias_next[nx];
                        }
                        if(nx >= 0) {
                            st.item = nx; st.isAlias = 1;
                            st.endSlot = -1; st.endScore = 0; st.nSteps = 0; st.nCols = 0; st.have = 0; st.sb = 0; st.se = -1; st.err = 0;
                            S.nextPhase = PH_SELECT;
                        }
                    }
                }
                DSYNC();
                phase = guni<GW>(S.nextPhase);
            }
            DP_T(1);
            if(phase == PH_IDLE && more) {
                int w = 0;
                if(gl == 0) {
                    if constexpr (DRAW > 1) {
                        int nx = S.chunkNext;
                        if(nx >= S.chunkEnd) { nx = atomicAdd(fetchCounter, DRAW); S.chunkEnd = nx + DRAW; }
                        S.chunkNext = nx + 1; w = nx;
                    } else w = atomicAdd(fetchCounter, 1);
                }
                w = grp_bcast0<GW>(w);
                if(w >= nItems) more = false;
                else {
                    const int idx = guni<GW>(srcList[w]);
                    const int4* ip = (const int4*)(items + idx);
                    int4 a = ip[0], b = ip[1];
                    DpItem it; it.item = a.x; it.rOff = a.y; it.seqLen = a.z; it.start_seq = a.w; it.startLevel = b.x; it.startNode = b.y; it.pad0 = 0; it.pad1 = 0;
                    phase = dp_begin<C>(S, sl, G, it, idx);
                    edgesAcc = 0;
                }
            }
            DP_T(0);
            if(!__ballot(phase != PH_IDLE)) break;
#ifdef HLALA_DP_TIMING
            trips++; runGroups += __popcll(__ballot(phase == PH_RUN)) / GW;
#endif
            DP_T(5);
        }
    }
    if(gl == 0 && S.accCalls) {
        atomicAdd(&B.counters[CNT_DP_CALLS], S.accCalls); atomicAdd(&B.counters[CNT_DP_ITERS], S.accIters);
        atomicAdd(&B.counters[CNT_DP_CELLS], S.accCells); atomicAdd(&B.counters[CNT_EDGES], S.accEdges);
    }
#ifdef HLALA_DP_TIMING
    if(TIER == 0 && (threadIdx.x & 63) == 0) { for(int i = 0; i < 8; i++) atomicAdd(&B.counters[24 + i], (u64)S.tPh[i]); for(int i = 0; i < 8; i++) atomicAdd(&B.counters[16 + i], (u64)S.tPh[8 + i]);
        for(int i = 0; i < 6; i++) atomicAdd(&B.counters[8 + i], (u64)tAcc[i]); atomicAdd(&B.counters[14], (u64)trips); atomicAdd(&B.counters[15], (u64)runGroups); }
#endif
}

template <int PER>
__device__ __forceinline__ void stitch_rounds(const DevBatch& B, const DevTables& T, const size_t cb, const int rOff, const int total, const int padL, const int nL, const int nSeed,
                                              const int nR, const int newEnd, const int stride, const int lane, double& llOut, int& f0, int& f1, int& l0, int& l1)
{
    const int seedAt = padL + nL, rightAt = seedAt + nSeed, padRAt = rightAt + nR;
    const int srcShift = (stride - nR) - rightAt;
    double carry = 0.0; int baseIdx = 0;
    f0 = -1; f1 = -1; l0 = -1; l1 = -1;
    for(int c0 = 0; c0 < total; c0 += 64 * PER) {
        const int chunk = min(64 * PER, total - c0);
        const int per = (chunk + 63) / 64;
        const int j0 = c0 + lane * per, j1 = min(c0 + chunk, j0 + per);
        int lv[PER], ed[PER]; unsigned char gcv[PER], scv[PER], kind[PER];
#pragma unroll
        for(int k = 0; k < PER; k++) {
            const int j = j0 + k; const bool in = k < per && j < j1;
            lv[k] = -1; ed[k] = -1; gcv[k] = '_'; scv[k] = '_'; kind[k] = 4;
            if(in) {
                if(j < padL) { kind[k] = 0; scv[k] = B.read_bases[rOff + j]; }
                else if(j < seedAt) { kind[k] = 1; lv[k] = B.ext_level[cb + j]; gcv[k] = B.ext_g[cb + j]; scv[k] = B.ext_s[cb + j]; }
                else if(j < rightAt) { const int q = j - seedAt; kind[k] = 2; lv[k] = B.seed_level[cb + q]; ed[k] = B.seed_edge[cb + q]; gcv[k] = B.seed_g[cb + q]; scv[k] = B.seed_s[cb + q]; }
                else if(j < padRAt) { const size_t p = cb + j + srcShift; kind[k] = 3; lv[k] = B.ext_level[p]; ed[k] = B.ext_edge[p]; gcv[k] = B.ext_g[p]; scv[k] = B.ext_s[p]; }
                else { kind[k] = 0; scv[k] = B.read_bases[rOff + newEnd + 1 + (j - padRAt)]; }
            }
        }
        WSYNC();
        int nb = 0;
#pragma unroll
        for(int k = 0; k < PER; k++) if(kind[k] != 4 && scv[k] != '_') nb++;
        int tot; const int before = baseIdx + wave_excl_scan(nb, tot);
        unsigned char qv[PER];
        {
            int idx = before;
#pragma unroll
            for(int k = 0; k < PER; k++) {
                qv[k] = 0;
                if(kind[k] != 4 && scv[k] != '_') { if(gcv[k] != '_') qv[k] = B.read_quals[rOff + idx]; idx++; }
            }
        }
#pragma unroll
        for(int k = 0; k < PER; k++) {
            const size_t o = cb + j0 + k;
            if(kind[k] == 1) B.ext_fromseed[o] = 0;
            else if(kind[k] != 4) {
                if(kind[k] != 3 || srcShift != 0) { B.ext_level[o] = lv[k]; B.ext_edge[o] = ed[k]; B.ext_g[o] = gcv[k]; B.ext_s[o] = scv[k]; }
                B.ext_fromseed[o] = kind[k] == 2 ? 1 : 0;
            }
        }
        double t1[PER], t2[PER];
#pragma unroll
        for(int k = 0; k < PER; k++) {
            const unsigned char sc = scv[k], gc = gcv[k];
            double a1 = 0.0, a2 = 0.0;
            if(kind[k] != 4) {
                if(sc != '_') {
                    if(gc == '_') a1 = T.rate_ins_quarter;
                    else { a1 = T.rate_match_mismatch; a2 = (sc == gc) ? T.ll_match[qv[k]] : T.ll_mismatch[qv[k]]; }
                } else if(gc != '_') a1 = T.rate_indel;
            }
            t1[k] = a1; t2[k] = a2;
        }
        const int lanesUsed = (chunk + per - 1) / per;
        double acc = 0.0;
        for(int l = 0; l < lanesUsed; l++) {
            double in = __shfl(acc, l > 0 ? l - 1 : 0);
            if(lane == l) {
                double a = (l == 0) ? carry : in;
#pragma unroll
                for(int k = 0; k < PER; k++) { a += t1[k]; a += t2[k]; }
                acc = a;
            }
        }
        carry = __shfl(acc, lanesUsed - 1); baseIdx += tot;
        {
            int cnt = 0, a0 = -1, a1 = -1, z0 = -1, z1 = -1;
#pragma unroll
            for(int k = 0; k < PER; k++) if(kind[k] != 4 && lv[k] != -1) { if(cnt == 0) a0 = lv[k]; else if(cnt == 1) a1 = lv[k]; z1 = z0; z0 = lv[k]; cnt++; }
            const u64 m1 = __ballot(cnt >= 1);
            if(m1) {
                const int F = __ffsll((long long)m1) - 1, Lz = 63 - __clzll((long long)m1);
                if(f1 < 0) {
                    const int fa0 = __shfl(a0, F), fa1 = __shfl(a1, F);
                    int nx = -1; { const u64 m2 = m1 & ~(1ull << F); if(m2) nx = __shfl(a0, __ffsll((long long)m2) - 1); }
                    if(f0 < 0) { f0 = fa0; f1 = fa1 >= 0 ? fa1 : nx; }
                    else f1 = fa0;
                }
                const int lz0 = __shfl(z0, Lz), lz1 = __shfl(z1, Lz);
                int pv = -1; { const u64 m2 = m1 & ~(1ull << Lz); if(m2) pv = __shfl(z0, 63 - __clzll((long long)m2)); }
                const int second = lz1 >= 0 ? lz1 : (pv >= 0 ? pv : l0);
                l0 = lz0; l1 = second;
            }
        }
    }
    llOut = carry;
}

__device__ __forceinline__ void stitch_draw(const DevBatch& B, const DevTables& T, const uint8_t* __restrict__ deferPairs, const int deferMode, const int lane, const int cq,
                                            u64& accChains, u64& accCols)
{
    const int stride = B.stride;
    const bool has = cq >= 0;
    int dSt = 0, dRead = 0, dNSeed = 0, dSB = 0, dSE = 0, dNcL = -1, dNcR = -1, dErrL = 0, dErrR = 0, dSbL = 0, dSeR = 0;
    if(has) dSt = B.ext_status[cq];
    if(has && dSt == EXT_PENDING) {
        dRead = B.chain_read[cq]; dNSeed = B.seed_ncols[cq]; dSB = B.seed_begin[cq]; dSE = B.seed_end[cq];
        const int2 nc = ((const int2*)B.dp_ncols)[cq], er = ((const int2*)B.dp_err)[cq];
        dNcL = nc.x; dNcR = nc.y; dErrL = er.x; dErrR = er.y; dSbL = B.dp_sb[2 * cq]; dSeR = B.dp_se[2 * cq + 1];
    }
    int dR0 = 0, dR1 = 0; bool dMine = has && dSt == EXT_PENDING;
    if(dMine) {
        dR0 = B.read_off[dRead]; dR1 = B.read_off[dRead + 1];
        if(deferMode == 1) dMine = deferPairs[dRead >> 1] == 0;
    }
    u64 mine = __ballot(dMine);
    for(; mine; mine &= mine - 1) {
        const int q = __ffsll((long long)mine) - 1;
        const int c = __builtin_amdgcn_readlane(cq, q);
        const int rOff = __builtin_amdgcn_readlane(dR0, q), seqLen = __builtin_amdgcn_readlane(dR1, q) - rOff;
        const size_t cb = row_base(B, c);
        const int nSeed = __builtin_amdgcn_readlane(dNSeed, q), sBegin = __builtin_amdgcn_readlane(dSB, q), sEnd = __builtin_amdgcn_readlane(dSE, q);
        const int ncL = __builtin_amdgcn_readlane(dNcL, q), ncR = __builtin_amdgcn_readlane(dNcR, q);
        const int errL = __builtin_amdgcn_readlane(dErrL, q), errR = __builtin_amdgcn_readlane(dErrR, q);
        int err = 0;
        if(errL || errR) err = ((errL <= -1000000) || (errR <= -1000000)) ? HLALA_CHAIN_ERR_COLUMNS : HLALA_CHAIN_ERR_FRONTIER;
        const bool haveL = ncL >= 0 && !errL, haveR = ncR >= 0 && !errR;
        const int nL = haveL ? ncL : 0, nR = haveR ? ncR : 0;
        const int newBegin = haveL ? __builtin_amdgcn_readlane(dSbL, q) : sBegin, newEnd = haveR ? __builtin_amdgcn_readlane(dSeR, q) : sEnd;
        const int padL = newBegin, padR = seqLen - 1 - newEnd;
        const int total = padL + nL + nSeed + nR + padR;
        if(!err && total > stride) err = HLALA_CHAIN_ERR_COLUMNS;
        if(err) {
            if(lane == 0) { B.ext_status[c] = err; B.ext_ncols[c] = 0; B.ext_ll[c] = (double)(errL ? errL : errR); atomicAdd(&B.counters[CNT_ERRORS], 1ull); }
        } else {
            double ll; int f0, f1, l0, l1;
            if(total <= 192) stitch_rounds<3>(B, T, cb, rOff, total, padL, nL, nSeed, nR, newEnd, stride, lane, ll, f0, f1, l0, l1);
            else stitch_rounds<8>(B, T, cb, rOff, total, padL, nL, nSeed, nR, newEnd, stride, lane, ll, f0, f1, l0, l1);
            if(lane == 0) {
                ((int4*)B.ext_firstlast)[c] = make_int4(f0, f1, l0, l1);
                B.ext_status[c] = HLALA_CHAIN_OK; B.ext_ncols[c] = total; B.ext_begin[c] = 0; B.ext_end[c] = seqLen - 1; B.ext_ll[c] = ll;
                accChains++; accCols += (u64)total;
            }
        }
        WSYNC();
    }
}

__global__ __launch_bounds__(64, 5) void k_stitch_chains(const DevGraph* __restrict__ Gp, const DevTables* __restrict__ Tp, const DevBatch* __restrict__ Bp,
                                                        const uint8_t* __restrict__ deferPairs, const int deferMode, const int draw, const int byRow)
{
    const DevBatch& B = *Bp;
    const DevTables& T = *Tp;
    const int lane = lane_id();
    u64 accChains = 0, accCols = 0;
    if(deferMode == 2) {
        const int nP = B.n_pairs;
        for(int p0 = (int)blockIdx.x * 64; p0 < nP; p0 += (int)gridDim.x * 64) {
            const int p = p0 + lane;
            u64 dm = __ballot(p < nP && deferPairs[p] != 0);
            for(; dm; dm &= dm - 1) {
                const int q = __ffsll((long long)dm) - 1;
                const int pp = p0 + q;
                const int c0 = uni(B.chain_off[2 * pp]), c1 = uni(B.chain_off[2 * pp + 2]);
                for(int cb = c0; cb < c1; cb += 64) stitch_draw(B, T, deferPairs, 0, lane, cb + lane < c1 ? cb + lane : -1, accChains, accCols);
            }
        }
    } else {
        const bool rows = byRow && B.chain_order && B.chain_row;
        const int nList = rows ? ordered_chains(B) : B.n_chains;
        for(;;) {
            int w0 = 0;
            if(lane == 0) w0 = atomicAdd(&B.work_counter[7], draw);
            w0 = __builtin_amdgcn_readfirstlane(w0);
            if(w0 >= nList) break;
            const int wq = w0 + lane;
            int cq = (lane < draw && wq < nList) ? wq : -1;
            if(rows && cq >= 0) cq = B.chain_order[cq];
            stitch_draw(B, T, deferPairs, deferMode, lane, cq, accChains, accCols);
        }
    }
    if(lane == 0 && accChains) { atomicAdd(&B.counters[CNT_CHAINS_EXT], accChains); atomicAdd(&B.counters[CNT_OUT_COLS], accCols); }
}

}
```

hla-la_amd/csrc/kernel_dp_band.hip:

```cpp
#include "batch.h"

namespace hlala {

constexpr int BAND_ABSENT = -20000;
constexpr int BAND_DRAW = 16;
constexpr int BAND_TIES = 16;

template <int GW_> struct BandCfg;
template <> struct BandCfg<16> { static constexpr int GW = 16, MAXJ = BAND_MAXJ16, REACH = 64, MAXD = 96, WAVES = 5; };
template <> struct BandCfg<32> { static constexpr int GW = 32, MAXJ = BAND_MAXJ32, REACH = 96, MAXD = 128, WAVES = 5; };
template <> struct BandCfg<64> { static constexpr int GW = 64, MAXJ = BAND_MAXJ64, REACH = 112, MAXD = 160, WAVES = 5; };

template <class C>
struct __align__(16) BandLds {
    u32 bt[C::MAXD / 8][C::GW];
    unsigned short steps[C::MAXD];
    unsigned short tieD[BAND_TIES];
    u32 ls[C::REACH];
};

template <int GW> __device__ __forceinline__ int band_prev(int v, int gl)
{
    if(GW == 16) return dpp_mov<0x111>(DP_NEG, v);
    int r = __builtin_amdgcn_update_dpp(DP_NEG, v, 0x138, 0xF, 0xF, false);
    if(GW == 32) r = (gl == 0) ? DP_NEG : r;
    return r;
}

#ifdef HLALA_BAND_TIMING
#define BAND_T(i) do { __builtin_amdgcn_s_waitcnt(0); const long long t_ = clock64(); tAcc[i] += t_ - tMark; tMark = t_; } while(0)
#else
#define BAND_T(i) do { } while(0)
#endif

template <class C, bool FWD>
__device__ __forceinline__ void band_pass(const DevGraph& G, const DevBatch& B, const DpItem* __restrict__ items, const u32 rng_seed, const uint8_t* __restrict__ readBases,
                                          const u32* __restrict__ linLabel, const int* __restrict__ linEid, BandLds<C>& S,
                                          u64& accCalls, u64& accIters, u64& accCells, u64& accEdges)
{
    constexpr int GW = C::GW, NG = 64 / GW;
    const int lane = lane_id(), g = lane / GW, gl = lane & (GW - 1), rowBase = lane & ~(GW - 1);
    constexpr int dirPass = FWD ? 1 : 0;
    constexpr int listK = (GW == 16 ? DPL_BAND16 : (GW == 32 ? DPL_BAND32 : DPL_BAND64)) + dirPass;
    const int segStart = uni(B.dp_blk[(size_t)listK * B.dp_nblk]);
    const int nItems = uni(B.dp_blk[(size_t)(listK + 1) * B.dp_nblk]) - segStart;
    const int* srcList = B.dp_list + segStart;
    int* fetchCounter = &B.work_counter[WC_BAND_FETCH + (GW == 16 ? 0 : (GW == 32 ? 2 : 4)) + dirPass];
    const int stride = B.stride;
    const int levelsL = G.L;
#ifdef HLALA_BAND_TIMING
    long long tAcc[6] = {0, 0, 0, 0, 0, 0}; long long tMark = clock64();
#endif
    int chunkNext = 0, chunkEnd = 0;
    for(;;) {
        BAND_T(4);
        if(chunkNext >= chunkEnd) {
            int w0 = 0;
            if(lane == 0) w0 = atomicAdd(fetchCounter, NG * BAND_DRAW);
            chunkNext = __builtin_amdgcn_readfirstlane(w0); chunkEnd = chunkNext + NG * BAND_DRAW;
        }
        if(chunkNext >= nItems) break;
        const int w = chunkNext + g;
        chunkNext += NG;
        const bool has = w < nItems;
        int idx = 0; int4 a = make_int4(-1, 0, 0, 0), b4 = make_int4(0, 0, 0, 0);
        if(has) { idx = srcList[w]; const int4* ip = (const int4*)(items + idx); a = ip[0]; b4 = ip[1]; }
        const int item0 = a.x, rOff = a.y, seqLen = a.z, y0 = a.w, x0 = b4.x;
        const int linRun = b4.w;
        const int jmax = has ? (FWD ? seqLen - y0 : y0) : 0;
        const int reach = min(linRun, C::REACH);
        int myRc = 0;
        if(has) {
            for(int t = gl; t < reach; t += GW) S.ls[t] = linLabel[FWD ? x0 + t : x0 - 1 - t];
            if(gl >= 1 && gl <= jmax) myRc = readBases[rOff + (FWD ? y0 + gl - 1 : y0 - gl)];
        }
        const u32 rcRep = (u32)myRc * 0x01010101u;
        WSYNC();
        BAND_T(0);

        int D1 = (has && gl == 0) ? 0 : DP_NEG, G1 = DP_NEG, S1 = DP_NEG, D2 = DP_NEG;
        int curMax = 0, lastInc = 0, firstPos = 0;
        int cBest = DP_NEG, cCount = 0, cFirstD = 0;
        u32 btAcc = 0;
        int cellsAcc = 0, edgesAcc = 0, itersRun = 0;
        int fail = 0; bool running = has;
        const int diagonals = seqLen + levelsL - 1;
        const bool inRead = gl <= jmax;
        int d = 1;
        for(;; d++) {
            const bool anyLive = grp_ballot<GW>(D1 > BAND_ABSENT || D2 > BAND_ABSENT) != 0;
            if(running) {
                if(d > diagonals || d - lastInc > 40) running = false;
                else if(!anyLive) { running = false; itersRun = min(lastInc + 40, diagonals); }
                else if(d > C::MAXD) { running = false; fail = 4; }
            }
            if(__ballot(running) == 0) break;
            const int i = d - gl;
            const u32 lw = S.ls[min(max(i - 1, 0), C::REACH - 1)], lx = lw ^ rcRep;
            const int m = ((lx - 0x01010101u) & ~lx & 0x80808080u) ? 2 : -5;
            const int nPar = 4 - (__clz((int)lw) >> 3);
            const int Dd = band_prev<GW>(D2, gl), Dg = band_prev<GW>(D1, gl), Gg = band_prev<GW>(G1, gl);
            const int Ds = D1, Ss = S1;
            const int cD = Dd + m;
            const int gO = Dg - 6, gE = Gg - 2; const bool gbit = gE > gO; const int GGv = gbit ? gE : gO;
            const int sO = Ds - 6, sE = Ss - 2; const bool sbit = sE > sO; const int SGv = sbit ? sE : sO;
            int Dv = cD, dsel = 0;
            if(GGv > Dv) { Dv = GGv; dsel = 1; }
            if(SGv > Dv) { Dv = SGv; dsel = 2; }
            if(!inRead) Dv = DP_NEG;
            const bool exists = Dv > BAND_ABSENT;
            const bool keep = Dv >= -16;
            const int mk = grp_max_i32<GW>(keep ? (((Dv + 64) << 6) | (FWD ? gl : GW - 1 - gl)) : 0);
            const int mx = (mk >> 6) - 64;
            const bool survive = keep && (mx - Dv) <= 15;
            if(running) {
                itersRun = d;
                cellsAcc += exists ? 1 : 0;
                edgesAcc += ((Dd > BAND_ABSENT && inRead) ? nPar : 0) + ((Ds > BAND_ABSENT) ? nPar : 0);
                if(mk != 0) {
// ... 56 lines not shown
                        if(__ballot(go) == 0) break;
                        if(go) {
                            guard++;
                            const int dd = d_ - 1;
                            const int bits = (int)((S.bt[dd >> 3][l_ & (GW - 1)] >> (4 * (dd & 7))) & 15u);
                            const int i_ = d_ - l_, j_ = l_;
                            int kind = -1;
                            if(m_ == 0) { const int ds = bits >> 2; if(ds == 0) { kind = K_DIAG; d_ -= 2; l_ -= 1; } else m_ = ds; }
                            else if(m_ == 1) { kind = K_GGAP; d_ -= 1; l_ -= 1; m_ = (bits & 1) ? 1 : 0; }
                            else { kind = K_SGAP; d_ -= 1; m_ = (bits & 2) ? 2 : 0; }
                            if(kind >= 0) { if(gl == 0 && n < C::MAXD) S.steps[n] = (unsigned short)(kind | (i_ << 2) | (j_ << 9)); n++; }
                        }
                    }
                    nSteps = n;
                    WSYNC();
                }
            }
            BAND_T(2);
            const int endScore = nTies > 0 ? best : curMax;
            bool have = endPos >= 0;
            int sb = 0, se = -1, err = 0;
            if(have) {
                const int jE = endPos & 63;
                if(FWD) { sb = y0; se = y0 + jE - 1; } else { sb = y0 - jE; se = y0 - 1; }
                const int nCols = nSteps;
                if(nCols > stride || nCols > C::MAXD) { err = -1000000 - nCols; have = false; }
                else if(sb > se) { err = __LINE__; have = false; }
                else {
                    const int rowOff = FWD ? stride - nCols : sb;
#ifdef BAND_X_NOCOLS
                    if(false) {
#else
                    if(live && rowOff + nCols <= stride) {
#endif
                        const size_t cb = row_base(B, item >> 1) + rowOff;
                        int* oL = B.ext_level + cb; int* oE = B.ext_edge + cb; uint8_t* oG = B.ext_g + cb; uint8_t* oS = B.ext_s + cb;
                        for(int s = gl; s < nCols; s += GW) {
                            const int st = S.steps[s]; const int kind = st & 3, i_ = (st >> 2) & 127, j_ = st >> 9;
                            const int lvl = FWD ? x0 + i_ - 1 : x0 - i_;
                            const int at = FWD ? nCols - 1 - s : s;
                            const unsigned char sc = j_ > 0 ? readBases[rOff + (FWD ? y0 + j_ - 1 : y0 - j_)] : (unsigned char)0;
                            const u32 lw = S.ls[i_ > 0 ? i_ - 1 : 0];
                            int par = 0;
                            if(kind == K_DIAG) { if(((lw >> 8) & 255u) == sc) par = 1; if(((lw >> 16) & 255u) == sc && par == 0) par = 2; if((lw >> 24) == sc && par == 0) par = 3; if((lw & 255u) == sc) par = 0; }
                            if(kind == K_GGAP) { oL[at] = -1; oE[at] = -1; oG[at] = '_'; oS[at] = sc; }
                            else {
                                oL[at] = lvl; oE[at] = par == 0 ? linEid[lvl] : G.out_eid[G.out_off[G.level_off[lvl]] + par];
                                oG[at] = (unsigned char)((lw >> (8 * par)) & 255u); oS[at] = (kind == K_DIAG) ? sc : (unsigned char)'_';
                            }
                        }
                    }
                }
            }
            int nx = -1;
            if(live && gl == 0) {
                B.dp_iters[item] = itersRun; B.dp_score[item] = have ? endScore : INT32_MIN; B.dp_ncols[item] = have ? nSteps : -1;
                B.dp_sb[item] = sb; B.dp_se[item] = se; B.dp_err[item] = err;
                accCalls++; accIters += (u64)itersRun; accCells += (u64)nCells; accEdges += (u64)nEdges;
#ifndef BAND_X_NOALIAS
                nx = B.dp_alias_head[item]; if(nx < 0) nx = B.dp_alias_next[item];
#endif
            }
            nx = __shfl(nx, rowBase);
            if(nx < 0) live = false; else item = nx;
            first = false;
            BAND_T(3);
        }
        if(has && fail && gl == 0) {
            const int q = atomicAdd(&B.work_counter[WC_FO_COUNT + dirPass], 1);
            B.retry_list[(size_t)(14 + dirPass) * (size_t)B.n_chains + q] = idx;
            atomicAdd(&B.work_counter[WC_BAND_FAILED], 1); atomicAdd(&B.work_counter[WC_BAND_WHY + fail], 1);
        }
        WSYNC();
#ifdef HLALA_BAND_TIMING
        tAcc[4] += 0; if(lane == 0) atomicAdd(&B.counters[22], 1ull);
#endif
    }
#ifdef HLALA_BAND_TIMING
    if(lane == 0 && GW == 16) { for(int i = 0; i < 5; i++) atomicAdd(&B.counters[16 + i], (u64)tAcc[i]); atomicAdd(&B.counters[21], (u64)tAcc[5]); }
#endif
}

template <int GW>
__global__ __launch_bounds__(64, BandCfg<GW>::WAVES) void k_dp_band(const DevGraph* __restrict__ Gp, const DevBatch* __restrict__ Bp, const DpItem* __restrict__ items, const u32 rng_seed,
                                                                    const uint8_t* __restrict__ readBases, const u32* __restrict__ linLabel, const int* __restrict__ linEid)
{
    typedef BandCfg<GW> C;
    const DevGraph& G = *Gp;
    const DevBatch& B = *Bp;
    __shared__ BandLds<C> SS[64 / GW];
    BandLds<C>& S = SS[lane_id() / GW];
    u64 accCalls = 0, accIters = 0, accCells = 0, accEdges = 0;
    band_pass<C, false>(G, B, items, rng_seed, readBases, linLabel, linEid, S, accCalls, accIters, accCells, accEdges);
    band_pass<C, true>(G, B, items, rng_seed, readBases, linLabel, linEid, S, accCalls, accIters, accCells, accEdges);
    if((lane_id() & (GW - 1)) == 0 && accCalls) {
        atomicAdd(&B.counters[CNT_DP_CALLS], accCalls); atomicAdd(&B.counters[CNT_DP_ITERS], accIters);
        atomicAdd(&B.counters[CNT_DP_CELLS], accCells); atomicAdd(&B.counters[CNT_EDGES], accEdges);
    }
}

}
```

hla-la_amd/csrc/kernel_pair.hip:

```cpp
#include "batch.h"
#include "../../include/hlala_gpu.h"

namespace hlala {

constexpr int PAIR_CHAINS = 64;
constexpr int PAIR_COMB   = 1024;
#ifndef HLALA_PAIR_COMB_LDS
#define HLALA_PAIR_COMB_LDS 128
#endif
constexpr int PAIR_COMB_LDS = HLALA_PAIR_COMB_LDS;
#ifndef PAIR_LEAN_WAVES
#define PAIR_LEAN_WAVES 6
#endif
#ifndef PAIR_MULTI_WAVES
#define PAIR_MULTI_WAVES 4
#endif
constexpr int PAIR_COLS   = 512;

constexpr short PAIR_NOCOL = -32768;
constexpr short PAIR_NOLEVEL = -32767;
struct __align__(16) PairListLds {
    int list[2][PAIR_CHAINS];
    int nlist[2];
    unsigned char src[2][PAIR_CHAINS];
};
struct __align__(16) PairLds {
    PairListLds L;
    double LL[PAIR_COMB_LDS];
    double phredThr[256];
    short baseLev[PAIR_COLS];
    unsigned char baseG[PAIR_COLS];
    unsigned char levS[PAIR_COLS];
    unsigned char levG[PAIR_COLS];
    double red[4];
    int ired[8];
};

__device__ __forceinline__ unsigned char pair_phred(const PairLds& P, double pCorrect)
{
    double pWrong = 1 - pCorrect;
    if(pWrong == 0) pWrong = 1e-100;
    int lo = 0, hi = 255;
    while(lo < hi) { const int mid = (lo + hi + 1) >> 1; if(pWrong <= P.phredThr[mid]) lo = mid; else hi = mid - 1; }
    return (unsigned char)lo;
}

__device__ inline int lp_find(const DevGraph& G, int level, int id)
{
    long long lo = G.lp_off[level], hi = G.lp_off[level + 1];
    while(lo < hi) {
        const long long mid = (lo + hi) >> 1; const int v = G.lp_seqid[mid];
        if(v == id) return G.lp_pos[mid];
        if(v < id) lo = mid + 1; else hi = mid;
    }
    return -1;
}

__device__ inline double pair_insert_ll(const DevGraph& G, const DevTables& T, const int up0, const int up1, const int dn0, const int dn1)
{
    const int lane = lane_id();
    {
        const int g = lane >> 4, e = lane & 15;
        const int lvl = g == 0 ? up0 : (g == 1 ? up1 : (g == 2 ? dn0 : dn1));
        long long lo = 0; int n = 0;
        if(lvl >= 0) { lo = G.lp_off[lvl]; n = (int)(G.lp_off[lvl + 1] - lo); }
        if(__ballot(n > 16) == 0) {
            int id = -1, pos = -1;
            if(e < n) { id = G.lp_seqid[lo + e]; pos = G.lp_pos[lo + e]; }
            const int nU0 = __builtin_amdgcn_readlane(n, 0), nD0 = __builtin_amdgcn_readlane(n, 32), nD1 = __builtin_amdgcn_readlane(n, 48);
            bool cand = g < 2 && e < n;
            for(int u = 0; u < nU0; u++) {
                const int oid = __builtin_amdgcn_readlane(id, u), op = __builtin_amdgcn_readlane(pos, u);
                if(g == 1 && oid == id && op >= 0) cand = false;
            }
            int beginPos = -1;
            for(int u = 0; u < nD0; u++) {
                const int oid = __builtin_amdgcn_readlane(id, 32 + u), op = __builtin_amdgcn_readlane(pos, 32 + u);
                if(oid == id && beginPos < 0) beginPos = op;
            }
            for(int u = 0; u < nD1; u++) {
                const int oid = __builtin_amdgcn_readlane(id, 48 + u), op = __builtin_amdgcn_readlane(pos, 48 + u);
                if(oid == id && beginPos < 0) beginPos = op;
            }
            const bool have = cand && beginPos >= 0;
            double best = -1.0e300;
            if(have) {
                const long long d = (long long)beginPos - pos - 1;
                const long long k = d - T.is_dmin;
                best = (k >= 0 && k < T.is_n) ? T.is_logpdf[k] : T.is_penalty;
            }
            for(int o = 32; o; o >>= 1) { const double ov = __shfl_xor(best, o); if(ov > best) best = ov; }
            return __ballot(have) ? best : T.is_penalty;
        }
    }
    const int upL[2] = {up0, up1}, dnL[2] = {dn0, dn1};
    double best = -1.0e300; bool have = false;
    for(int a = 0; a < 2; a++) {
        if(upL[a] < 0) continue;
        const long long lo = G.lp_off[upL[a]], hi = G.lp_off[upL[a] + 1];
        for(long long ia = lo + lane; ia < hi; ia += 64) {
            const int id = G.lp_seqid[ia]; const int endPos = G.lp_pos[ia];
            if(a == 1 && upL[0] >= 0 && lp_find(G, upL[0], id) >= 0) continue;
            int beginPos = -1;
            if(dnL[0] >= 0) beginPos = lp_find(G, dnL[0], id);
            if(beginPos < 0 && dnL[1] >= 0) beginPos = lp_find(G, dnL[1], id);
            if(beginPos < 0) continue;
            const long long d = (long long)beginPos - endPos - 1;
            const long long k = d - T.is_dmin;
            const double v = (k >= 0 && k < T.is_n) ? T.is_logpdf[k] : T.is_penalty;
            if(!have || v > best) { best = v; have = true; }
        }
    }
    if(!have) best = -1.0e300;
    for(int o = 32; o; o >>= 1) { const double ov = __shfl_xor(best, o); if(ov > best) best = ov; }
    return __ballot(have) ? best : T.is_penalty;
}

constexpr int PAIR_MAXDIST = 32;
__global__ void k_pair_distances(const DevGraph* __restrict__ Gp, const DevBatch* __restrict__ Bp, int* __restrict__ out_n, int* __restrict__ out_d)
{
    const DevGraph& G = *Gp; const DevBatch& B = *Bp;
    const int p = blockIdx.x * blockDim.x + threadIdx.x;
    if(p >= B.n_pairs) return;
    const int ca = 2 * p, cb = 2 * p + 1;
    if(B.ext_status[ca] != HLALA_CHAIN_OK || B.ext_status[cb] != HLALA_CHAIN_OK) { out_n[p] = -1; return; }
    const int* fa = B.ext_firstlast + 4 * ca; const int* fb = B.ext_firstlast + 4 * cb;
    const bool ra = B.chain_reverse[ca] != 0, rb = B.chain_reverse[cb] != 0;
    bool valid = false;
    if(fa[0] != -1 && fb[0] != -1 && ra != rb) valid = (!ra) ? (fa[0] < fb[0]) : (fa[2] > fb[2]);
    if(!valid) { out_n[p] = -2; return; }
    const int* fl_up = (fa[0] < fb[0]) ? fa : fb; const int* fl_down = (fa[0] < fb[0]) ? fb : fa;
    int upL[2] = {fl_up[2], fl_up[3]}, dnL[2] = {fl_down[0], fl_down[1]};
    int n = 0;
    for(int a = 0; a < 2; a++) {
        if(upL[a] < 0) continue;
        for(long long ia = G.lp_off[upL[a]]; ia < G.lp_off[upL[a] + 1]; ia++) {
            int id = G.lp_seqid[ia]; int endPos = G.lp_pos[ia];
            if(a == 1 && upL[0] >= 0) {
                bool dup = false;
                for(long long q = G.lp_off[upL[0]]; q < G.lp_off[upL[0] + 1]; q++) if(G.lp_seqid[q] == id) { dup = true; break; }
                if(dup) continue;
            }
            int beginPos = -1;
            for(int b = 0; b < 2 && beginPos < 0; b++) {
                if(dnL[b] < 0) continue;
                for(long long q = G.lp_off[dnL[b]]; q < G.lp_off[dnL[b] + 1]; q++) if(G.lp_seqid[q] == id) { beginPos = G.lp_pos[q]; break; }
            }
            if(beginPos < 0) continue;
            const int d = beginPos - endPos - 1;
            bool seen = false;
            for(int k = 0; k < n && k < PAIR_MAXDIST; k++) if(out_d[(size_t)p * PAIR_MAXDIST + k] == d) seen = true;
            if(!seen) { if(n < PAIR_MAXDIST) out_d[(size_t)p * PAIR_MAXDIST + n] = d; n++; }
        }
    }
    out_n[p] = n;
}

struct PairChain { int4 fl; int rev, nk, row; double ll; };
__device__ __forceinline__ PairChain pair_chain_load(const DevBatch& B, const int c)
{
    PairChain x;
    x.fl = *(const int4*)(B.ext_firstlast + 4 * (size_t)c); x.rev = B.chain_reverse[c]; x.ll = B.ext_ll[c]; x.nk = B.ext_ncols[c]; x.row = B.chain_row ? B.chain_row[c] : c;
    return x;
}
__device__ __forceinline__ PairChain pair_chain_from_lane(const PairChain& x, const int srcLane)
{
    PairChain y;
    y.fl.x = __shfl(x.fl.x, srcLane); y.fl.y = __shfl(x.fl.y, srcLane); y.fl.z = __shfl(x.fl.z, srcLane); y.fl.w = __shfl(x.fl.w, srcLane);
    y.rev = __shfl(x.rev, srcLane); y.nk = __shfl(x.nk, srcLane); y.row = __shfl(x.row, srcLane);
    const long long b = __double_as_longlong(x.ll);
    y.ll = __longlong_as_double((long long)(((u64)(u32)__shfl((int)(b >> 32), srcLane) << 32) | (u64)(u32)__shfl((int)b, srcLane)));
    return y;
}

template <bool UNPAIRED, int PER>
__device__ __forceinline__ void pair_positions(const DevBatch& B, PairLds& P, const double* __restrict__ LL, const int p, const int n1, const int n2, const int nComb,
                                               const int best1, const int best2, const PairChain& cA, const PairChain& cB, const int lane, const int stride)
{
    constexpr int NM = UNPAIRED ? 1 : 2;
    for(int m = 0; m < NM; m++) {
        const int r = UNPAIRED ? p : 2 * p + m;
        const int nl = m ? n2 : n1;
        const int nkL = m ? cB.nk : cA.nk, rowL = m ? cB.row : cA.row, f0L = m ? cB.fl.x : cA.fl.x;
        const int kSel = m ? best2 : best1;
        const int nSel = __builtin_amdgcn_readlane(nkL, kSel); const size_t sb = (size_t)__builtin_amdgcn_readlane(rowL, kSel) * (size_t)stride; const size_t ob = (size_t)r * stride;
        if(nComb == 1) {
            const unsigned char ph = (unsigned char)P.ired[7];
            for(int j = lane; j < nSel; j += 64) B.sel_mapq[ob + j] = ph;
            continue;
        }
        u64 mask[PER];
        int selLv[PER], selInfo[PER];
        #pragma unroll
        for(int t = 0; t < PER; t++) { const int j = t * 64 + lane; mask[t] = 0; selLv[t] = -1; selInfo[t] = (int)((u32)'_' << 24); if(j < nSel) { selLv[t] = B.ext_level[sb + j]; selInfo[t] = (int)((u32)B.ext_g[sb + j] | ((u32)B.ext_s[sb + j] << 24)); } }
        {
            int carry = 0;
            #pragma unroll
            for(int t = 0; t < PER; t++) {
                if(t * 64 >= nSel) break;
                const int j = t * 64 + lane; const bool isBase = j < nSel && ((u32)selInfo[t] >> 24) != (u32)'_';
                const u64 bm = __ballot(isBase);
                const int ord = isBase ? carry + __popcll(bm & ((1ull << lane) - 1ull)) : 0xFFFF;
                selInfo[t] = (int)(((u32)selInfo[t] & 255u) | ((u32)ord << 8));
                carry += __popcll(bm);
            }
            #pragma unroll
            for(int t = 0; t < PER; t++) if(t * 64 >= nSel) selInfo[t] = (int)(((u32)selInfo[t] & 255u) | (0xFFFFu << 8));
        }
        for(int k = 0; k < nl; k++) {
            if(k == kSel) {
                #pragma unroll
                for(int t = 0; t < PER; t++) if(t * 64 + lane < nSel) mask[t] |= (1ull << k);
                continue;
            }
            const int nk = __builtin_amdgcn_readlane(nkL, k), firstK = __builtin_amdgcn_readlane(f0L, k);
            const size_t kb = (size_t)__builtin_amdgcn_readlane(rowL, k) * (size_t)stride;
            WSYNC();
            for(int i = lane; i < PAIR_COLS / 4; i += 64) { ((unsigned long long*)P.baseLev)[i] = 0x8000800080008000ull; }
            for(int i = lane; i < PAIR_COLS / 8; i += 64) { ((unsigned long long*)P.levS)[i] = 0ull; }
            WSYNC();
            int carry = 0;
            for(int t0 = 0; t0 * 64 < nk; t0 += 4) {
                unsigned char ks[4], kg[4]; int kl[4];
                #pragma unroll
                for(int u = 0; u < 4; u++) { const int j = (t0 + u) * 64 + lane; ks[u] = 0; kg[u] = 0; kl[u] = -1; if(j < nk) { ks[u] = B.ext_s[kb + j]; kg[u] = B.ext_g[kb + j]; kl[u] = B.ext_level[kb + j]; } }
                #pragma unroll
                for(int u = 0; u < 4; u++) {
                    if((t0 + u) * 64 >= nk) break;
                    const int j = (t0 + u) * 64 + lane; const bool act = j < nk;
                    const bool isBase = act && ks[u] != '_';
                    const u64 bm = __ballot(isBase);
                    const int rel = kl[u] == -1 ? (int)PAIR_NOLEVEL : kl[u] - firstK;
                    if(isBase) { const int bi = carry + __popcll(bm & ((1ull << lane) - 1ull)); if(bi < PAIR_COLS) { P.baseLev[bi] = (short)(rel > 32767 ? 32767 : rel); P.baseG[bi] = kg[u]; } }
                    carry += __popcll(bm);
                    if(act && kl[u] != -1 && firstK >= 0 && rel >= 0 && rel < PAIR_COLS) { P.levS[rel] = ks[u]; P.levG[rel] = kg[u]; }
                }
            }
            WSYNC();
            #pragma unroll
            for(int t = 0; t < PER; t++) {
                const int j = t * 64 + lane;
                if(j >= nSel) continue;
                const int lj = selLv[t]; const unsigned char gj = (unsigned char)(selInfo[t] & 255); const int myIdx = (int)(((u32)selInfo[t] >> 8) & 0xFFFFu);
                bool hit = false;
                if(myIdx != 0xFFFF) {
                    const short bl = myIdx < PAIR_COLS ? P.baseLev[myIdx] : PAIR_NOCOL;
                    if(bl != PAIR_NOCOL) {
                        int want = lj == -1 ? (int)PAIR_NOLEVEL : lj - firstK;
                        if(lj != -1 && (want > 32767 || want < -32766)) want = 32766;
                        hit = ((int)bl == want) && (P.baseG[myIdx] == gj);
                    }
                }
                else if(lj != -1 && firstK >= 0) { const int li = lj - firstK; if(li >= 0 && li < PAIR_COLS) hit = (P.levS[li] == '_') && (P.levG[li] == gj); }
                if(hit) mask[t] |= (1ull << k);
            }
        }
        WSYNC();
        #pragma unroll
        for(int t = 0; t < PER; t++) {
            const int j = t * 64 + lane;
            if(j >= nSel) continue;
            double Q = 0;
            if(m == 0) { for(int i1 = 0; i1 < n1; i1++) if(mask[t] & (1ull << i1)) for(int i2 = 0; i2 < n2; i2++) Q += LL[i1 * n2 + i2]; }
            else       { for(int i1 = 0; i1 < n1; i1++) for(int i2 = 0; i2 < n2; i2++) if(mask[t] & (1ull << i2)) Q += LL[i1 * n2 + i2]; }
            if(Q > 1) Q = 1;
            B.sel_mapq[ob + j] = pair_phred(P, Q);
        }
    }
}

#ifdef HLALA_PAIR_TIMING
#define PAIR_T(i) do { __builtin_amdgcn_s_waitcnt(0); const long long t_ = clock64(); tAcc[i] += t_ - tMark; tMark = t_; } while(0)
#else
#define PAIR_T(i) do { } while(0)
#endif

template <bool UNPAIRED, bool BIG>
__device__ __forceinline__ void pair_finish(const DevGraph& G, const DevTables& T, const DevBatch& B, PairLds& P, double* __restrict__ LL,
                                            const int p, const int n1, const int n2, const int nComb, const int mxc, const PairChain& cA, const PairChain& cB, const int lane, const int stride, long long* tAcc, long long& tMark)
{
    constexpr int NM = UNPAIRED ? 1 : 2;
        if(UNPAIRED) { if(lane < nComb) LL[lane] = cA.ll; }
        else {
            const int4 fA = cA.fl, fB = cB.fl; const int rA = cA.rev, rB = cB.rev; const double lA = cA.ll, lB = cB.ll;
            auto rl64 = [](double v, int l) -> double { const long long b = __double_as_longlong(v);
                return __longlong_as_double((long long)(((u64)(u32)__builtin_amdgcn_readlane((int)(b >> 32), l) << 32) | (u64)(u32)__builtin_amdgcn_readlane((int)b, l))); };
            for(int i = 0; i < nComb; i++) {
                const int i1 = i / n2, i2 = i % n2;
                const int fa0 = __builtin_amdgcn_readlane(fA.x, i1), fa1 = __builtin_amdgcn_readlane(fA.y, i1), fa2 = __builtin_amdgcn_readlane(fA.z, i1), fa3 = __builtin_amdgcn_readlane(fA.w, i1);
                const int fb0 = __builtin_amdgcn_readlane(fB.x, i2), fb1 = __builtin_amdgcn_readlane(fB.y, i2), fb2 = __builtin_amdgcn_readlane(fB.z, i2), fb3 = __builtin_amdgcn_readlane(fB.w, i2);
                const bool ra = __builtin_amdgcn_readlane(rA, i1) != 0, rb = __builtin_amdgcn_readlane(rB, i2) != 0;
                bool valid = false;
                if(fa0 != -1 && fb0 != -1 && ra != rb) valid = (!ra) ? (fa0 < fb0) : (fa2 > fb2);
                double llIS = T.is_penalty;
#ifndef PAIR_X_NOINSERT
                if(valid) llIS = (fa0 < fb0) ? pair_insert_ll(G, T, fa2, fa3, fb0, fb1) : pair_insert_ll(G, T, fb2, fb3, fa0, fa1);
#endif
                double combined = rl64(lA, i1) + rl64(lB, i2);
                combined += llIS;
                if(lane == 0) LL[i] = combined;
            }
        }
        WSYNC();
        PAIR_T(1);
        double mx = -1.0e300; int mi = 0x7FFFFFFF;
        for(int i = lane; i < nComb; i += 64) { double v = LL[i]; if(v > mx) { mx = v; mi = i; } }
        for(int o = 32; o; o >>= 1) { double ov = __shfl_xor(mx, o); int oi = __shfl_xor(mi, o); if(ov > mx || (ov == mx && oi < mi)) { mx = ov; mi = oi; } }
        const int bestI = uni(mi), best1 = bestI / n2, best2 = bestI % n2;
        const int selA = uni(P.L.list[0][best1]), selB = UNPAIRED ? selA : uni(P.L.list[1][best2]);
        double mapQ = 1, q1 = 1, q2 = 1;
        if(nComb > 1) {
            for(int i = lane; i < nComb; i += 64) LL[i] = exp_cr_nonpos(LL[i] - mx);
            WSYNC();
            if(lane == 0) {
                double S = 0; for(int i = 0; i < nComb; i++) S += LL[i];
                P.red[0] = S;
            }
            WSYNC();
            double S = P.red[0];
            for(int i = lane; i < nComb; i += 64) LL[i] = LL[i] / S;
            WSYNC();
            if(lane == 0) {
                double a = 0, b = 0;
                for(int i = 0; i < nComb; i++) { double pp = LL[i]; if(i / n2 == best1) a += pp; if(i % n2 == best2) b += pp; }
                if(a > 1) a = 1; if(b > 1) b = 1;
                P.red[1] = a; P.red[2] = b;
            }
            WSYNC();
            mapQ = LL[bestI]; q1 = P.red[1]; q2 = P.red[2];
        }
        bool svalid = false;
        if(!UNPAIRED) {
            const int fa0 = __builtin_amdgcn_readlane(cA.fl.x, best1), fa2 = __builtin_amdgcn_readlane(cA.fl.z, best1), fb0 = __builtin_amdgcn_readlane(cB.fl.x, best2), fb2 = __builtin_amdgcn_readlane(cB.fl.z, best2);
            const bool ra = __builtin_amdgcn_readlane(cA.rev, best1) != 0, rb = __builtin_amdgcn_readlane(cB.rev, best2) != 0;
            if(fa0 != -1 && fb0 != -1 && ra != rb) svalid = (!ra) ? (fa0 < fb0) : (fa2 > fb2);
        }
        if(lane == 0) {
            B.pair_status[p] = 0; B.n_comb[p] = nComb; B.pair_ll[p] = mx; B.pair_mapq[p] = mapQ;
            if(UNPAIRED) { B.best_chain[p] = selA; B.mate_mapq[p] = mapQ; B.strands_valid[p] = 0; }
            else {
            B.best_chain[2 * p] = selA; B.best_chain[2 * p + 1] = selB; B.mate_mapq[2 * p] = q1; B.mate_mapq[2 * p + 1] = q2;
            B.strands_valid[p] = svalid ? 1 : 0;
            }
        }
        PAIR_T(2);
#ifndef PAIR_X_NOPOS
        if(!BIG || mxc <= 192) pair_positions<UNPAIRED, 3>(B, P, LL, p, n1, n2, nComb, best1, best2, cA, cB, lane, stride);
        else pair_positions<UNPAIRED, PAIR_COLS / 64>(B, P, LL, p, n1, n2, nComb, best1, best2, cA, cB, lane, stride);
#endif
        PAIR_T(nComb == 1 ? 3 : 4);
#ifdef HLALA_PAIR_TIMING
        tAcc[nComb == 1 ? 5 : 6] += 1;
#endif
}

template <bool UNPAIRED>
__device__ __forceinline__ int pair_lists(const DevBatch& B, PairListLds& L, const int* cLo, const int* cHi, const int lane, int& n1, int& n2, int& mxcOut, PairChain* cL)
{
    constexpr int NM = UNPAIRED ? 1 : 2;
    int bad = 0;
    int stF[NM], ncF[NM];
    #pragma unroll
    for(int m = 0; m < NM; m++) { const int c = cLo[m] + lane; stF[m] = 1; ncF[m] = 0; if(c < cHi[m]) { stF[m] = B.ext_status[c]; ncF[m] = B.ext_ncols[c]; } }
    PairChain cF[NM];
    #pragma unroll
    for(int m = 0; m < NM; m++) { const int c = cLo[m] + lane; cF[m].fl = make_int4(-1, -1, -1, -1); cF[m].rev = 0; cF[m].nk = 0; cF[m].row = 0; cF[m].ll = 0.0; if(c < cHi[m]) { cF[m] = pair_chain_load(B, c); } }
    int mxc = 0;
    #pragma unroll
    for(int m = 0; m < NM; m++) {
        const int c0 = cLo[m], c1 = cHi[m];
        int cnt = 0;
        for(int b0 = c0; b0 < c1; b0 += 64) {
            int c = b0 + lane; int st, nc;
            if(b0 == c0) { st = stF[m]; nc = ncF[m]; } else { st = 1; nc = 0; if(c < c1) { st = B.ext_status[c]; nc = B.ext_ncols[c]; } }
            if(__ballot(st < 0)) bad = 1;
            u64 okm = __ballot(st == HLALA_CHAIN_OK);
            if(st == HLALA_CHAIN_OK) { int pos = cnt + __popcll(okm & ((1ull << lane) - 1ull)); if(pos < PAIR_CHAINS) { L.list[m][pos] = c; L.src[m][pos] = (unsigned char)lane; mxc = max(mxc, nc); } }
            cnt += __popcll(okm);
        }
        if(lane == 0) L.nlist[m] = cnt;
        if(cnt < 1 || cnt > PAIR_CHAINS) bad = 1;
    }
    WSYNC();
    n1 = uni(L.nlist[0]); n2 = UNPAIRED ? 1 : uni(L.nlist[1]);
    bad = uni(bad);
    const long long nCombLL = (long long)n1 * n2;
    if(!bad && nCombLL > PAIR_COMB) bad = 1;
    mxc = wave_max_i32(mxc);
    if(!bad && nCombLL > 1 && mxc > PAIR_COLS) bad = 1;
    mxcOut = mxc;
    if(bad) return 1;
    #pragma unroll
    for(int m = 0; m < NM; m++) {
        const int nl = m ? n2 : n1;
        if(cHi[m] - cLo[m] <= 64) cL[m] = pair_chain_from_lane(cF[m], lane < nl ? (int)L.src[m][lane] : lane);
        else { cL[m].fl = make_int4(-1, -1, -1, -1); cL[m].rev = 0; cL[m].nk = 0; cL[m].row = 0; cL[m].ll = 0.0; if(lane < nl) cL[m] = pair_chain_load(B, L.list[m][lane]); }
    }
    if(UNPAIRED) cL[1] = cL[0];
    return 0;
}

template <bool UNPAIRED>
__global__ __launch_bounds__(64, PAIR_LEAN_WAVES) void k_pair_chains(const DevGraph* __restrict__ Gp, const DevTables* __restrict__ Tp, const DevBatch* __restrict__ Bp,
                                                   const uint8_t* __restrict__ deferPairs, const int deferMode, const int counterIdx,
                                                   int* __restrict__ multiList, const int multiBase)
{
    const DevGraph& G = *Gp;
    const DevBatch& B = *Bp;
    __shared__ PairListLds L;
    const int lane = lane_id();
    const DevTables& T = *Tp;
    const int stride = B.stride;

    constexpr int CHUNK = 8;
    int sweep = 0;
    int ph1 = 0;
    if(lane == 0) { double pWrong = 1e-100; int lo = 0, hi = 255; while(lo < hi) { const int mid = (lo + hi + 1) >> 1; if(pWrong <= T.phred_thr[mid]) lo = mid; else hi = mid - 1; } ph1 = lo; }
    ph1 = __builtin_amdgcn_readfirstlane(ph1);
    for(;;) {
        int p0 = 0;
        if(deferMode == 2) { p0 = ((int)blockIdx.x + sweep * (int)gridDim.x) * CHUNK; sweep++; }
        else {
            if(lane == 0) p0 = atomicAdd(&B.work_counter[counterIdx], CHUNK);
            p0 = __builtin_amdgcn_readfirstlane(p0);
        }
        if(p0 >= B.n_pairs) break;
        const int pEnd = min(p0 + CHUNK, B.n_pairs);
        constexpr int NM = UNPAIRED ? 1 : 2;
        int hDf = 0, hC[NM + 1];
        #pragma unroll
        for(int m = 0; m <= NM; m++) hC[m] = 0;
        if(lane < CHUNK && p0 + lane < pEnd) {
            const int pq = p0 + lane;
            if(deferMode) hDf = deferPairs[pq];
            #pragma unroll
            for(int m = 0; m <= NM; m++) hC[m] = B.chain_off[NM * pq + m];
        }
        for(int p = p0; p < pEnd; p++) {
        const int hq = p - p0;
        if(deferMode) { const bool df = __builtin_amdgcn_readlane(hDf, hq) != 0; if(df == (deferMode == 1)) continue; }
        int cLo[NM], cHi[NM];
        #pragma unroll
        for(int m = 0; m < NM; m++) { cLo[m] = __builtin_amdgcn_readlane(hC[m], hq); cHi[m] = __builtin_amdgcn_readlane(hC[m + 1], hq); }
        int n1 = 0, n2 = 0, mxc = 0; PairChain cL[2];
        const int bad = pair_lists<UNPAIRED>(B, L, cLo, cHi, lane, n1, n2, mxc, cL);
        if(bad) {
            if(lane == 0) { B.pair_status[p] = -1; if(UNPAIRED) B.best_chain[p] = -1; else { B.best_chain[2 * p] = -1; B.best_chain[2 * p + 1] = -1; } B.n_comb[p] = 0; }
        } else if(n1 * n2 > 1) {
            if(lane == 0) { const int cls = (n1 * n2 <= PAIR_COMB_LDS && mxc <= 192) ? 0 : 1; const int q = atomicAdd(&B.work_counter[multiBase + 2 * cls], 1); multiList[(size_t)cls * (size_t)B.n_pairs + q] = p; }
        } else {
            double combined = cL[0].ll;
            bool svalid = false;
            if(!UNPAIRED) {
                const int fa0 = __builtin_amdgcn_readlane(cL[0].fl.x, 0), fa1 = __builtin_amdgcn_readlane(cL[0].fl.y, 0), fa2 = __builtin_amdgcn_readlane(cL[0].fl.z, 0), fa3 = __builtin_amdgcn_readlane(cL[0].fl.w, 0);
                const int fb0 = __builtin_amdgcn_readlane(cL[1].fl.x, 0), fb1 = __builtin_amdgcn_readlane(cL[1].fl.y, 0), fb2 = __builtin_amdgcn_readlane(cL[1].fl.z, 0), fb3 = __builtin_amdgcn_readlane(cL[1].fl.w, 0);
                const bool ra = __builtin_amdgcn_readlane(cL[0].rev, 0) != 0, rb = __builtin_amdgcn_readlane(cL[1].rev, 0) != 0;
                if(fa0 != -1 && fb0 != -1 && ra != rb) svalid = (!ra) ? (fa0 < fb0) : (fa2 > fb2);
                double llIS = T.is_penalty;
                if(svalid) llIS = (fa0 < fb0) ? pair_insert_ll(G, T, fa2, fa3, fb0, fb1) : pair_insert_ll(G, T, fb2, fb3, fa0, fa1);
                combined = cL[0].ll + cL[1].ll;
                combined += llIS;
            }
            const int selA = uni(L.list[0][0]), selB = UNPAIRED ? selA : uni(L.list[1][0]);
            if(lane == 0) {
                B.pair_status[p] = 0; B.n_comb[p] = 1; B.pair_ll[p] = combined; B.pair_mapq[p] = 1.0;
                if(UNPAIRED) { B.best_chain[p] = selA; B.mate_mapq[p] = 1.0; B.strands_valid[p] = 0; }
                else { B.best_chain[2 * p] = selA; B.best_chain[2 * p + 1] = selB; B.mate_mapq[2 * p] = 1.0; B.mate_mapq[2 * p + 1] = 1.0; B.strands_valid[p] = svalid ? 1 : 0; }
            }
            #pragma unroll
            for(int m = 0; m < NM; m++) {
                const int nSel = __builtin_amdgcn_readlane(cL[m].nk, 0); const size_t ob = (size_t)(UNPAIRED ? p : 2 * p + m) * stride;
                for(int j = lane; j < nSel; j += 64) B.sel_mapq[ob + j] = (unsigned char)ph1;
            }
        }
        WSYNC();
        }
    }
}

template <bool UNPAIRED, bool BIG>
__global__ __launch_bounds__(64, BIG ? 3 : PAIR_MULTI_WAVES) void k_pair_multi(const DevGraph* __restrict__ Gp, const DevTables* __restrict__ Tp, const DevBatch* __restrict__ Bp,
                                                  const int* __restrict__ multiList, const int multiBase, double* __restrict__ bigLL)
{
    const DevGraph& G = *Gp;
    const DevBatch& B = *Bp;
    __shared__ PairLds P;
    const int lane = lane_id();
    const DevTables& T = *Tp;
    const int stride = B.stride;
    constexpr int CHUNK = 4;
    constexpr int NM = UNPAIRED ? 1 : 2;
    const int* list = multiList + (BIG ? (size_t)B.n_pairs : (size_t)0);
    const int nList = uni(B.work_counter[multiBase + (BIG ? 2 : 0)]);
    int* fetch = &B.work_counter[multiBase + (BIG ? 3 : 1)];
    if(nList <= 0) return;
    for(int i = lane; i < 256; i += 64) P.phredThr[i] = T.phred_thr[i];
    WSYNC();
    if(lane == 0) P.ired[7] = (int)pair_phred(P, 1.0);
    WSYNC();
    long long tAcc[8] = {0, 0, 0, 0, 0, 0, 0, 0}; long long tMark = clock64();
    for(;;) {
        int q0 = 0;
        if(lane == 0) q0 = atomicAdd(fetch, CHUNK);
        q0 = __builtin_amdgcn_readfirstlane(q0);
        if(q0 >= nList) break;
        const int qEnd = min(q0 + CHUNK, nList);
        int hP = 0, hC[NM + 1];
        #pragma unroll
        for(int m = 0; m <= NM; m++) hC[m] = 0;
        if(lane < CHUNK && q0 + lane < qEnd) {
            hP = list[q0 + lane];
            #pragma unroll
            for(int m = 0; m <= NM; m++) hC[m] = B.chain_off[NM * hP + m];
        }
        for(int q = q0; q < qEnd; q++) {
            const int hq = q - q0;
            const int p = __builtin_amdgcn_readlane(hP, hq);
            int cLo[NM], cHi[NM];
            #pragma unroll
            for(int m = 0; m < NM; m++) { cLo[m] = __builtin_amdgcn_readlane(hC[m], hq); cHi[m] = __builtin_amdgcn_readlane(hC[m + 1], hq); }
            int n1 = 0, n2 = 0, mxc = 0; PairChain cL[2];
            const int bad = pair_lists<UNPAIRED>(B, P.L, cLo, cHi, lane, n1, n2, mxc, cL);
            if(!bad) {
                const int nComb = n1 * n2;
                PAIR_T(0);
                if(!BIG || nComb <= PAIR_COMB_LDS) pair_finish<UNPAIRED, BIG>(G, T, B, P, P.LL, p, n1, n2, nComb, mxc, cL[0], cL[1], lane, stride, tAcc, tMark);
                else pair_finish<UNPAIRED, BIG>(G, T, B, P, bigLL + (size_t)blockIdx.x * PAIR_COMB, p, n1, n2, nComb, mxc, cL[0], cL[1], lane, stride, tAcc, tMark);
            }
            WSYNC();
        }
    }
#ifdef HLALA_PAIR_TIMING
    if(lane == 0) for(int i = 0; i < 7; i++) atomicAdd(&B.counters[24 + i], (u64)tAcc[i]);
#endif
}

__global__ __launch_bounds__(64) void k_post_pairs(const DevBatch* __restrict__ Bp, int* __restrict__ cov, int nCov, const int* __restrict__ geneFirst,
                                                   const int* __restrict__ geneLast, int nGenes, uint8_t* __restrict__ include)
{
    const DevBatch& B = *Bp;
    const int lane = lane_id();
    const int stride = B.stride;
    constexpr int CHUNK = 8;
    for(;;) {
        int p0 = 0;
        if(lane == 0) p0 = atomicAdd(&B.work_counter[11], CHUNK);
        p0 = __builtin_amdgcn_readfirstlane(p0);
        if(p0 >= B.n_pairs) break;
        const int pEnd = min(p0 + CHUNK, B.n_pairs);
        for(int p = p0; p < pEnd; p++) {
            bool inc = false;
            if(uni(B.pair_status[p]) == 0) {
                const int nm = B.unpaired ? 1 : 2;
                for(int m = 0; m < nm; m++) {
                    const int ch = uni(B.best_chain[B.unpaired ? p : 2 * p + m]);
                    if(ch < 0 || ch >= B.n_chains) continue;
                    const int n = uni(B.ext_ncols[ch]);
                    const size_t so = row_base(B, ch);
                    for(int j = lane; j < n; j += 64) {
                        const int lv = B.ext_level[so + j];
                        if(lv != -1 && B.ext_g[so + j] != '_' && lv >= 0 && lv < nCov) atomicAdd(&cov[lv], 1);
                    }
                    const int first = uni(B.ext_firstlast[4 * ch + 0]), last = uni(B.ext_firstlast[4 * ch + 2]);
                    if(first != -1) {
                        bool hit = false;
                        for(int g = lane; g < nGenes; g += 64) hit = hit || (geneLast[g] >= first && geneFirst[g] <= last);
                        if(__ballot(hit)) inc = true;
                    }
// ... 69 lines not shown
```

hla-la_amd/csrc/kernel_project.hip:

```cpp
#include "batch.h"
#include "../../include/hlala_gpu.h"

namespace hlala {

constexpr int PROJ_CAP   = 512;
constexpr int PROJ_NODES = 512;
constexpr int PROJ_SN    = 640;
constexpr int PROJ_SE    = 768;
constexpr int PROJ_SEGMAX = 24;

struct ChoiceRec { int eid; short fromz; short S; };

constexpr int RT_SN = 416;
constexpr int RT_CE = 512;
constexpr int CHAIN_RETHREAD_PENDING = 64;


template <int CAP_, int SN_, int SE_>
struct __align__(16) ProjLdsT {
    static constexpr int CAP = CAP_, SN = SN_, SE = SE_; static constexpr bool LONG = false;
    typedef unsigned short LvT;
    LvT lvl[2][CAP_];
    unsigned char g[2][CAP_], s[2][CAP_];
    short Srow[2][PROJ_NODES];
// ... 75 lines not shown

__device__ inline int cigar_end_position(const u32* cig, int n, int pos)
{
    int e = pos;
    for(int i = 0; i < n; i++) { u32 op = cig[i] & 15u; if(op == 0 || op == 7 || op == 8 || op == 2 || op == 3) e += (int)(cig[i] >> 4); }
    return e - 1;
}

__global__ void k_filter_chains(const DevGraph* __restrict__ Gp, const DevBatch* __restrict__ Bp, const long long* contig_off, const int* contig_level)
{
    const DevBatch& B = *Bp;
    int r = blockIdx.x * blockDim.x + threadIdx.x;
    if(r >= B.n_reads) return;
    int c0 = B.chain_off[r], c1 = B.chain_off[r + 1];
    bool primRev = B.chain_reverse[B.read_primary[r]] != 0;
    for(int c = c0; c < c1; c++) {
        int st = HLALA_CHAIN_OK;
        int contig = B.chain_contig[c];
        long long clen = contig_off[contig + 1] - contig_off[contig];
        int a = B.chain_pos[c] - B.chain_offset[c];
        int b = cigar_end_position(B.cigar + B.cigar_off[c], B.cigar_off[c + 1] - B.cigar_off[c], B.chain_pos[c]) - B.chain_offset[c];
        int idA = -1, idB = -1;
        if(a < 0 || a >= clen || b < 0 || b >= clen) st = HLALA_CHAIN_ERR_INPUT;
        else { idA = contig_level[contig_off[contig] + a]; idB = contig_level[contig_off[contig] + b]; }
        if(st == HLALA_CHAIN_OK && (B.chain_reverse[c] != 0) != primRev) st = HLALA_CHAIN_SKIP_STRAND;
        if(st == HLALA_CHAIN_OK) {
            for(int p = c0; p < c; p++) {
                if(B.seed_status[p] != HLALA_CHAIN_OK) continue;
                int pc = B.chain_contig[p];
                int pa = B.chain_pos[p] - B.chain_offset[p];
                int pb = cigar_end_position(B.cigar + B.cigar_off[p], B.cigar_off[p + 1] - B.cigar_off[p], B.chain_pos[p]) - B.chain_offset[p];
                int pidA = contig_level[contig_off[pc] + pa], pidB = contig_level[contig_off[pc] + pb];
                if(pidA == idA && pidB == idB && B.chain_as[p] >= B.chain_as[c]) { st = HLALA_CHAIN_SKIP_DUP; break; }
            }
        }
        B.seed_status[c] = st;
        if(st != HLALA_CHAIN_OK) B.seed_ncols[c] = 0;
        if(B.chain_bucket) {
            int bk = -1;
            if(st == HLALA_CHAIN_OK) {
                if(B.order_cost) {
                    const int la = idA < idB ? idA : idB, lb = idA < idB ? idB : idA;
                    const int cost = (Gp->level_off[lb + 1] - Gp->level_off[la]) >> 5;
                    bk = B.order_nb - 2 - cost; if(bk < 0) bk = 0;
                } else { bk = (idA >= 0 ? idA : (idB >= 0 ? idB : 0)) >> B.order_shift; if(bk > B.order_nb - 2) bk = B.order_nb - 2; }
                atomicAdd(&B.order_hist[bk], 1);
            }
            B.chain_bucket[c] = bk;
        }
    }
}

template <int U, class LoadF, class StoreF>
__device__ __forceinline__ void staged_rows(int first, int end, int step, LoadF load, StoreF store)
{
    for(int base = first; base < end; base += U * step) {
        decltype(load(0)) v[U];
        #pragma unroll
        for(int u = 0; u < U; u++) { const int i = base + u * step; if(i < end) v[u] = load(i); }
        #pragma unroll
        for(int u = 0; u < U; u++) { const int i = base + u * step; if(i < end) store(i, v[u]); }
    }
}
struct FromLab { int from; unsigned char lab; };

#define PJ_FAIL(code) do { if(P.err == 0) P.err = (code); } while(0)
#ifdef HLALA_PROJ_TIMING
constexpr bool PJ_FINE = true;
#else
constexpr bool PJ_FINE = false;
#endif
#define PJ_T(i) do { if(B.dbg) tPh[i] = clock64(); } while(0)
#define LSYNC() do { asm volatile("s_waitcnt lgkmcnt(0)" ::: "memory"); __builtin_amdgcn_wave_barrier(); } while(0)
#define PJ_OK() (uni(P.err) == 0)

constexpr int PJL_U = 4;
#ifndef HLALA_PROJ_LONG_WPS
#define HLALA_PROJ_LONG_WPS 5
#endif
#ifndef HLALA_PROJ_WPS
#define HLALA_PROJ_WPS 2
#endif
template <class PL>
__global__ __launch_bounds__(64, PL::LONG ? HLALA_PROJ_LONG_WPS : HLALA_PROJ_WPS) void k_project_chains(const DevGraph* __restrict__ Gp, const DevBatch* __restrict__ Bp, const long long* contig_off, const uint8_t* contig_seq,
                                                       const int* contig_level, char* slabs, size_t slabBytes, char* longSlabs, size_t longSlabBytes,
                                                       int deferRethread)
{
    const DevGraph& G = *Gp;
    const DevBatch& B = *Bp;
    __shared__ PL P;
    const int lane = lane_id();
    if(PL::LONG) { if(lane == 0) proj_bind(P, longSlabs + (size_t)blockIdx.x * longSlabBytes); WSYNC(); }
    ChoiceRec* slabCh = (ChoiceRec*)(slabs + (size_t)blockIdx.x * slabBytes);
    const int slabEnt = (int)(slabBytes / sizeof(ChoiceRec));
    const int stride = B.stride;

    long long tAcc[7] = {0, 0, 0, 0, 0, 0, 0};
    int readOrd = -1;
    long long tSub[4] = {0, 0, 0, 0};
    long long tFine[12] = {0, 0, 0, 0, 0, 0, 0, 0, 0, 0, 0, 0}, tFineLast = 0;
#define PJ_F(i) do { if constexpr (PL::LONG && PJ_FINE) if(B.dbg) { const long long t_ = clock64(); if((i) >= 0) tFine[(i) < 0 ? 0 : (i)] += t_ - tFineLast; tFineLast = t_; } } while(0)
    u64 accCols = 0, accEdges = 0;
    constexpr int CHUNK = PL::LONG ? 1 : 4;
    const int nWork = ordered_chains(B);
    for(;;) {
        int c0 = 0;
        if(lane == 0) c0 = atomicAdd(&B.work_counter[0], CHUNK);
        c0 = __builtin_amdgcn_readfirstlane(c0);
        if(c0 >= nWork) break;
        const int cEnd = min(c0 + CHUNK, nWork);
        int hStatus = -1, hRead = 0, hContig = 0, hPos = 0, hOff = 0, hCg0 = 0, hCg1 = 0, hChain = 0;
        if(lane < CHUNK && c0 + lane < cEnd) {
            const int cq = B.chain_order ? B.chain_order[c0 + lane] : c0 + lane;
            hChain = cq;
            hStatus = B.seed_status[cq]; hRead = B.chain_read[cq]; hContig = B.chain_contig[cq]; hPos = B.chain_pos[cq]; hOff = B.chain_offset[cq];
            hCg0 = B.cigar_off[cq]; hCg1 = B.cigar_off[cq + 1];
        }
        int hR0 = 0, hR1 = 0, hC0lo = 0, hC0hi = 0, hC1lo = 0, hC1hi = 0;
        if(hStatus == HLALA_CHAIN_OK) {
            hR0 = B.read_off[hRead]; hR1 = B.read_off[hRead + 1];
            const long long a0 = contig_off[hContig], a1 = contig_off[hContig + 1];
            hC0lo = (int)(u32)a0; hC0hi = (int)(a0 >> 32); hC1lo = (int)(u32)a1; hC1hi = (int)(a1 >> 32);
        }
        for(int drawn = c0; drawn < cEnd; drawn++) {
        const int hq = drawn - c0;
        const int c = __builtin_amdgcn_readlane(hChain, hq);
        if(__builtin_amdgcn_readlane(hStatus, hq) == HLALA_CHAIN_OK) {
        const int r = __builtin_amdgcn_readlane(hRead, hq);
        const int rOff = __builtin_amdgcn_readlane(hR0, hq), readLen = __builtin_amdgcn_readlane(hR1, hq) - rOff;
        const int contig = __builtin_amdgcn_readlane(hContig, hq);
        const long long cOff = (long long)(((u64)(u32)__builtin_amdgcn_readlane(hC0hi, hq) << 32) | (u64)(u32)__builtin_amdgcn_readlane(hC0lo, hq));
        const long long cLen = (long long)(((u64)(u32)__builtin_amdgcn_readlane(hC1hi, hq) << 32) | (u64)(u32)__builtin_amdgcn_readlane(hC1lo, hq)) - cOff;
        const int pos = __builtin_amdgcn_readlane(hPos, hq), tOffset = __builtin_amdgcn_readlane(hOff, hq);
        const int cg0 = __builtin_amdgcn_readlane(hCg0, hq), nOps = __builtin_amdgcn_readlane(hCg1, hq) - cg0;
        typedef LvCodec<PL> LC;
        int lvBase = 0;
        const u32 cgFirst = lane < nOps ? B.cigar[cg0 + lane] : 0;
        if constexpr (LC::SHORT) {
            const long long t0 = (long long)pos - tOffset;
            for(long long q0 = t0 > 0 ? t0 : 0, qEnd = q0 + 2 * (long long)PL::CAP; q0 < cLen && q0 < qEnd; q0 += 64) {
                const long long q = q0 + lane;
                const int lv = q < cLen ? contig_level[cOff + q] : -1;
                const int m = -wave_max_i32(lv >= 0 ? -lv : -0x7FFFFFFF);
                if(m != 0x7FFFFFFF) { lvBase = m; break; }
            }
        }
        if(lane == 0) { P.err = 0; }
        WSYNC();
        long long tPh[7] = {0, 0, 0, 0, 0, 0, 0};
        long long tFine0[12], tSub0[4]; int dbgN[8] = {0, 0, 0, 0, 0, 0, 0, 0};
        if constexpr (PL::LONG && PJ_FINE) if(B.dbg) { for(int i = 0; i < 12; i++) tFine0[i] = tFine[i]; for(int i = 0; i < 4; i++) tSub0[i] = tSub[i]; }

        PJ_T(0); PJ_F(-1);
        if(nOps < 1) { if(lane == 0) PJ_FAIL(HLALA_CHAIN_ERR_INPUT); }
        int nCols = 0;
        if(PJ_OK()) {
            int baseCol = 0, baseRef = 0, baseRead = 0, leadH = 0, prevOp = -1;
            int firstStart = -1, lastRS = 0, lastLen = 0, lastUse = 0;
            for(int ob = 0; ob < nOps; ob += 64) {
                const int oi = ob + lane;
                u32 cg = ob == 0 ? cgFirst : (oi < nOps ? B.cigar[cg0 + oi] : 0);
                int op = (int)(cg & 15u), len = (int)(cg >> 4);
                if(oi >= nOps) { op = 6; len = 0; }
                bool isCol = (op == 0 || op == 7 || op == 8 || op == 2 || op == 1);
                bool useRef = (op == 0 || op == 7 || op == 8 || op == 2);
                bool useRead = (op == 0 || op == 7 || op == 8 || op == 1 || op == 4);
                if(ob == 0) { int lh = 0; if(lane == 0 && op == 5) lh = len; leadH = __shfl(lh, 0); }
                int tc, tr, tq;
                int colStart = baseCol + wave_excl_scan(isCol ? len : 0, tc);
                int refStart = baseRef + wave_excl_scan(useRef ? len : 0, tr);
                int readStart = baseRead + wave_excl_scan(useRead ? len : 0, tq) + leadH;
                int pop = __shfl_up(op, 1); if(lane == 0) pop = prevOp;
// ... 922 lines not shown
                    auto pick = P.lvl[1 - cur];
                    for(int j = lane; j < n1; j += 64) pick[j] = LC::pickNone();
                    WSYNC();
                    const int nbR = nb - nodeBase;
                    int z = zsel;
                    for(int k = nChunks - 1; k >= 0; k--) {
                        const int a = P.sChoice[k] & 0x7FFF; const bool wide = (P.sChoice[k] & 0x8000) != 0;
                        const int b = (k + 1 < nChunks ? (int)(P.sChoice[k + 1] & 0x7FFF) : nDef) - 1;
                        if(wide) {
                            if(lane == 0) { const ChoiceRec cr = ch[(int)P.sLev[a + 1] + z - nbR]; pick[P.colInfo[a] & 0xFFFFu] = cr.eid; z = cr.fromz; }
                        } else {
                            const int tBase = P.sLev[a + 1], nT = (int)P.sLev[b + 2] - tBase;
                            staged_rows<7>(lane, nT, 64, [&](int t) { return ch[tBase + t - nbR]; }, [&](int t, ChoiceRec cr) { P.sIn[t] = (unsigned short)cr.fromz; P.sFrom[t] = (unsigned short)cr.eid; });
                            WSYNC();
                            if(lane == 0) for(int i = b; i >= a; i--) { const int t = (int)P.sLev[i + 1] - tBase + z; pick[P.colInfo[i] & 0xFFFFu] = (int)P.sFrom[t]; z = (int)(short)P.sIn[t]; }
                        }
                        WSYNC();
                    }
                    staged_rows<6>(lane, n1, 64, [&](int j) { const typename PL::LvT pe = pick[j]; FromLab r; r.from = -1; r.lab = '_';
                                                              if(!LC::pickIsNone(pe)) { r.from = G.in_eid[eBase + (int)pe]; r.lab = G.in_label[eBase + (int)pe]; } return r; },
                        [&](int j, FromLab r) {
                            B.seed_level[cb + j] = LC::pickIsNone(pick[j]) ? -1 : LC::get(P.lvl[cur][j], lvBase); B.seed_edge[cb + j] = r.from; B.seed_g[cb + j] = r.lab;
                            B.seed_s[cb + j] = P.s[cur][j];
                        });
                } else if(lane == 0) {
                    int node = tb + zsel;
                    for(int j = n1 - 1; j >= 0; j--) {
                        int l = LC::get(P.lvl[cur][j], lvBase);
                        if(l == -1) { B.seed_level[cb + j] = -1; B.seed_edge[cb + j] = -1; B.seed_g[cb + j] = '_'; B.seed_s[cb + j] = P.s[cur][j]; continue; }
                        ChoiceRec cr = ch[node - nb];
                        B.seed_level[cb + j] = l; B.seed_edge[cb + j] = cr.eid; B.seed_g[cb + j] = G.edge_label[cr.eid]; B.seed_s[cb + j] = P.s[cur][j];
                        node = G.level_off[l] + cr.fromz;
                    }
                }
                if(lane == 0) {
                    B.seed_ncols[c] = n1; B.seed_begin[c] = P.startRaw; B.seed_end[c] = P.stopRaw; B.seed_removed[c] = removed;
                    accCols += (u64)n1;
                }
            }
        }
        PJ_T(6); PJ_F(8);
        if constexpr (PL::LONG && PJ_FINE) readOrd++;
        if(B.dbg) { for(int i = 0; i < 6; i++) if(tPh[i + 1] && tPh[i]) tAcc[i] += tPh[i + 1] - tPh[i]; tAcc[6]++; }
        if constexpr (PL::LONG && PJ_FINE) if(B.dbg && lane == 0 && tPh[6] && tPh[0]) {
            const long long cyc = tPh[6] - tPh[0]; int k = 0; while(k < 47 && (cyc >> (k + 1)) != 0) k++;
            atomicAdd(&B.dbg[4096 + k], 1); atomicAdd(&B.dbg[4160 + k], (int)(cyc >> 16));
            { const int o = readOrd < 31 ? readOrd : 31; atomicAdd(&B.dbg[4400 + o], (int)(cyc >> 16)); atomicAdd(&B.dbg[4432 + o], 1); atomicAdd(&B.dbg[4464 + o], dbgN[2] >> 4); }
            if(k >= 25) {
                { const int q = atomicAdd(&B.dbg[4318], 1); if(q < 300) { int* r = B.dbg + 5000 + 10 * q; r[0] = c; r[1] = dbgN[0]; r[2] = dbgN[1]; r[3] = dbgN[2]; r[4] = dbgN[3]; r[5] = dbgN[4]; r[6] = dbgN[5]; r[7] = dbgN[6]; r[8] = (int)(cyc >> 16); r[9] = dbgN[7] | ((int)((tPh[0] >> 20) & 0x7FFFF) << 8); } }
                atomicAdd(&B.dbg[4319], 1);
                for(int i = 0; i < 6; i++) atomicAdd(&B.dbg[4320 + i], (int)((tPh[i + 1] - tPh[i]) >> 12));
                for(int i = 0; i < 12; i++) atomicAdd(&B.dbg[4330 + i], (int)((tFine[i] - tFine0[i]) >> 12));
                for(int i = 0; i < 4; i++) atomicAdd(&B.dbg[4344 + i], (int)((tSub[i] - tSub0[i]) >> (i < 2 ? 12 : 0)));
            }
        }
        {
            int e = wave_sum_i32((int)edgesTouched);
            accEdges += (u64)e;
        }
        WSYNC();
        if(!PJ_OK() && lane == 0) { B.seed_status[c] = P.err; B.seed_ncols[c] = 0; }
        }
        WSYNC();
        }
    }
    if(lane == 0) { if(accCols) atomicAdd(&B.counters[CNT_SEED_COLS], accCols); if(accEdges) atomicAdd(&B.counters[CNT_EDGES], accEdges); }
#ifndef HLALA_DP_TIMING
    if(B.dbg && lane == 0) { for(int i = 0; i < 6; i++) atomicAdd(&B.counters[16 + i], (u64)tAcc[i]); atomicAdd(&B.counters[23], (u64)tAcc[6]); }
    if(B.dbg && lane == 0) for(int i = 0; i < 4; i++) atomicAdd(&B.counters[24 + i], (u64)tSub[i]);
    if constexpr (PL::LONG && PJ_FINE) if(B.dbg && lane == 0) for(int i = 0; i < 12; i++) atomicAdd(&B.dbg[4300 + i], (int)(tFine[i] >> 12));
#endif
}

struct __align__(16) RethreadLds {
    u32 eRec[RT_CE];
    unsigned short sIn[RT_SN + 2];
    short Srow[2][PROJ_NODES];
    unsigned short pick[PROJ_CAP];
    u64 chunkStart[PROJ_CAP / 64];
};

__global__ __launch_bounds__(64, 6) void k_rethread_chains(const DevGraph* __restrict__ Gp, const DevBatch* __restrict__ Bp, char* slabs, size_t slabBytes)
{
    const DevGraph& G = *Gp;
    const DevBatch& B = *Bp;
    __shared__ RethreadLds P;
    const int lane = lane_id();
    u32* const ch = (u32*)(slabs + (size_t)blockIdx.x * slabBytes);
    const int stride = B.stride;
    u64 accCols = 0, accEdges = 0;
    const int nWork = ordered_chains(B);
    for(;;) {
        constexpr int RT_DRAW = 16;
        int c0 = 0;
        if(lane == 0) c0 = atomicAdd(&B.work_counter[3], RT_DRAW);
        c0 = __builtin_amdgcn_readfirstlane(c0);
        if(c0 >= nWork) break;
        const int cq = (lane < RT_DRAW && c0 + lane < nWork) ? (B.chain_order ? B.chain_order[c0 + lane] : c0 + lane) : -1;
        u64 pend = __ballot(cq >= 0 && B.seed_status[cq] == CHAIN_RETHREAD_PENDING);
        for(; pend; pend &= pend - 1) {
            const int c = __builtin_amdgcn_readlane(cq, __ffsll((long long)pend) - 1);
            const size_t cb = row_base(B, c);
            const int* st = (const int*)B.dp_items + (size_t)c * 16;
            int sv = lane < 6 ? st[lane] : 0;
            const int level0 = __builtin_amdgcn_readlane(sv, 0), nDef = __builtin_amdgcn_readlane(sv, 1), nodeBase = __builtin_amdgcn_readlane(sv, 2), nb = __builtin_amdgcn_readlane(sv, 3),
                      eBase = __builtin_amdgcn_readlane(sv, 4), n1 = __builtin_amdgcn_readlane(sv, 5);
            (void)level0;
            const unsigned short* lvRow = (const unsigned short*)(B.ext_level + cb); const unsigned short* sgRow = (const unsigned short*)(B.ext_edge + cb);
            const int* ciRow = B.seed_edge + cb;
            const int nbR = nb - nodeBase;
            for(int z = lane; z < nbR; z += 64) P.Srow[0][z] = 0;
            if(lane < PROJ_CAP / 64) P.chunkStart[lane] = 0;
            WSYNC();
            int rowP = 0, err = 0;
            u64 edgesTouched = 0;
            int a = 0;
            while(a < nDef && !err) {
                const int i0 = a + lane;
                const int lvA = i0 <= nDef + 1 ? (int)lvRow[i0] : 0, lvC = i0 + 2 <= nDef + 1 ? (int)lvRow[i0 + 2] : 0;
                const int sgA = i0 <= nDef ? (int)sgRow[i0] : 0, sgB = i0 + 1 <= nDef ? (int)sgRow[i0 + 1] : 0;
                const u32 ciReg = i0 < nDef ? (u32)ciRow[i0] : 0u;
                const int lvA1 = __builtin_amdgcn_readlane(lvA, 1), sgA0 = __builtin_amdgcn_readlane(sgA, 0);
                const bool fits = i0 < nDef && lane < 62 && (lvC - lvA1) <= RT_SN && (sgB - sgA0) <= RT_CE;
                const u64 fm = __ballot(fits);
                const int cnt = __ffsll((long long)~fm) - 1;
                if(cnt == 0) { err = HLALA_CHAIN_ERR_FRONTIER; break; }
                const int b = a + cnt - 1;
                if(lane == 0) P.chunkStart[a >> 6] |= 1ull << (a & 63);
                const int tBase = lvA1, nT = __builtin_amdgcn_readlane(lvA, cnt + 1) - tBase, eC = sgA0, nE = __builtin_amdgcn_readlane(sgA, cnt) - eC;
                const int lvReg = lvA, sgReg = sgA - eC;
                {
                    constexpr int UE = RT_CE / 64, UN = (RT_SN + 1 + 63) / 64;
                    const bool needOff = __ballot(lane < cnt && ((ciReg >> 25) & 3u) == 0u) != 0;
                    u32 ve[UE]; int vn[UN];
                    #pragma unroll
                    for(int u = 0; u < UE; u++) { const int e = lane + 64 * u; if(e < nE) ve[u] = G.in_rec[eBase + eC + e]; }
                    if(needOff) {
                        #pragma unroll
                        for(int u = 0; u < UN; u++) { const int t = lane + 64 * u; if(t <= nT) vn[u] = G.in_off[nodeBase + tBase + t]; }
                    }
                    #pragma unroll
                    for(int u = 0; u < UE; u++) { const int e = lane + 64 * u; if(e < nE) P.eRec[e] = ve[u]; }
                    if(needOff) {
                        #pragma unroll
                        for(int u = 0; u < UN; u++) { const int t = lane + 64 * u; if(t <= nT) P.sIn[t] = (unsigned short)(vn[u] - eBase - eC); }
                    }
                }
                WSYNC();
                bool prevFast = false; int sReg = -1;
                u32 recN = 0;
                { const int nE0 = __builtin_amdgcn_readlane(sgReg, 1); if(lane < nE0 && nE0 <= 64) recN = P.eRec[lane]; }
                for(int k = 0; k < cnt; k++) {
                    const u32 ci = (u32)__builtin_amdgcn_readlane((int)ciReg, k);
                    const int sc = (int)((ci >> 16) & 0xFFu); const bool seedIsMatch = ((ci >> 24) & 1u) != 0;
                    const int l1 = __builtin_amdgcn_readlane(lvReg, k + 1), tm = __builtin_amdgcn_readlane(lvReg, k + 2) - l1;
                    const int eL0 = __builtin_amdgcn_readlane(sgReg, k), eL1 = __builtin_amdgcn_readlane(sgReg, k + 1), nEl = eL1 - eL0;
                    const int mode = (int)((ci >> 25) & 3u), maxd = (int)((ci >> 27) & 7u);
                    const u32 rec = recN;
                    if(k + 1 < cnt) { const int nEn = __builtin_amdgcn_readlane(sgReg, k + 2) - eL1; recN = (lane < nEn && nEn <= 64) ? P.eRec[eL1 + lane] : 0u; }
                    bool reached = false;
                    auto edge_key = [&](const u32 r, const int sp, const bool mine) -> int {
                        const int m = (int)((r >> 18) & 0xFFu) == sc ? 1 : 0;
                        const int cand = (mine && sp >= 0 && (m || !seedIsMatch)) ? sp + m + 1 : 0;
                        return (cand << 15) | ((63 - lane) << 9) | (int)(r & 511u);
                    };
                    auto node_key = [&](const u32 r, const int key) -> int {
                        const int pos = (int)((r >> 15) & 7u);
                        int bk = key, kj = key;
// ... 122 lines not shown
```

Baseline: 5.560 million.

## Pass graph and batch descriptors by value or as global-address-space views

Templates the graph and batch descriptor structs on pointer type so that device code can treat their pointers as global address space instead of generic (flat) pointers. Several kernels now take the descriptors by value as kernel arguments (kernarg/scalar loads) instead of dereferencing a device pointer, while the long-projection kernel and the rethread kernel use a global-address-space view of the in-memory descriptor. This aims to let the compiler emit global loads instead of flat loads and hoist descriptor fields into scalar registers. The cost is much larger kernel argument blocks, possible extra register pressure, and a wide template change across all kernel helpers.

```diff
diff --git a/hla-la_amd/csrc/batch.h b/hla-la_amd/csrc/batch.h
--- a/hla-la_amd/csrc/batch.h
+++ b/hla-la_amd/csrc/batch.h
@@ -3,85 +3,96 @@
 
 namespace hlala {
 
-struct DevBatch {
+template <template <class> class Ptr> struct DevBatchT {
     int n_pairs, n_reads, n_chains, stride;
     int from_seeds;
     int unpaired;
-    const int* read_off;
-    const uint8_t* read_bases;
-    const uint8_t* read_quals;
-    const int* chain_off;
-    const int* read_primary;
-    const int* chain_read;
-    const int* chain_contig;
-    const int* chain_pos;
-    const int* chain_offset;
-    const int* chain_as;
-    const uint8_t* chain_reverse;
-    const int* cigar_off;
-    const u32* cigar;
-    int* seed_status;
-    int* seed_ncols;
-    int* seed_begin;
-    int* seed_end;
-    int* seed_removed;
-    int* seed_level;
-    int* seed_edge;
-    uint8_t* seed_g;
-    uint8_t* seed_s;
-    int* ext_status;
-    int* ext_ncols;
-    int* ext_begin;
-    int* ext_end;
-    double* ext_ll;
-    int* dp_iters;
-    int* dp_score;
-    int* dp_ncols;
-    int* dp_sb;
-    int* dp_se;
-    int* dp_err;
-    int* dp_alias_head;
-    int* dp_alias_next;
-    int* ext_level;
-    int* ext_edge;
-    uint8_t* ext_g;
-    uint8_t* ext_s;
-    uint8_t* ext_fromseed;
-    int* ext_firstlast;
-    int* pair_status;
-    int* best_chain;
-    int* n_comb;
-    double* pair_ll;
-    double* pair_mapq;
-    double* mate_mapq;
-    uint8_t* strands_valid;
-    uint8_t* sel_mapq;
-    u64* counters;
-    int* work_counter;
-    int* retry_list;
-    int* pair_multi;
-    uint8_t* pair_deferred;
-    int* chain_order;
-    int* chain_bucket;
-    int* order_hist;
+    Ptr<const int> read_off;
+    Ptr<const uint8_t> read_bases;
+    Ptr<const uint8_t> read_quals;
+    Ptr<const int> chain_off;
+    Ptr<const int> read_primary;
+    Ptr<const int> chain_read;
+    Ptr<const int> chain_contig;
+    Ptr<const int> chain_pos;
+    Ptr<const int> chain_offset;
+    Ptr<const int> chain_as;
+    Ptr<const uint8_t> chain_reverse;
+    Ptr<const int> cigar_off;
+    Ptr<const u32> cigar;
+    Ptr<int> seed_status;
+    Ptr<int> seed_ncols;
+    Ptr<int> seed_begin;
+    Ptr<int> seed_end;
+    Ptr<int> seed_removed;
+    Ptr<int> seed_level;
+    Ptr<int> seed_edge;
+    Ptr<uint8_t> seed_g;
+    Ptr<uint8_t> seed_s;
+    Ptr<int> ext_status;
+    Ptr<int> ext_ncols;
+    Ptr<int> ext_begin;
+    Ptr<int> ext_end;
+    Ptr<double> ext_ll;
+    Ptr<int> dp_iters;
+    Ptr<int> dp_score;
+    Ptr<int> dp_ncols;
+    Ptr<int> dp_sb;
+    Ptr<int> dp_se;
+    Ptr<int> dp_err;
+    Ptr<int> dp_alias_head;
+    Ptr<int> dp_alias_next;
+    Ptr<int> ext_level;
+    Ptr<int> ext_edge;
+    Ptr<uint8_t> ext_g;
+    Ptr<uint8_t> ext_s;
+    Ptr<uint8_t> ext_fromseed;
+    Ptr<int> ext_firstlast;
+    Ptr<int> pair_status;
+    Ptr<int> best_chain;
+    Ptr<int> n_comb;
+    Ptr<double> pair_ll;
+    Ptr<double> pair_mapq;
+    Ptr<double> mate_mapq;
+    Ptr<uint8_t> strands_valid;
+    Ptr<uint8_t> sel_mapq;
+    Ptr<u64> counters;
+    Ptr<int> work_counter;
+    Ptr<int> retry_list;
+    Ptr<int> pair_multi;
+    Ptr<uint8_t> pair_deferred;
+    Ptr<int> chain_order;
+    Ptr<int> chain_bucket;
+    Ptr<int> order_hist;
     int order_shift, order_nb;
     int long_chunk_nodes, long_max_segs;
     int order_cost;
-    int* chain_row;
+    Ptr<int> chain_row;
     int n_rows;
-    int* dp_blk;
-    int* dp_list;
+    Ptr<int> dp_blk;
+    Ptr<int> dp_list;
     int dp_nblk;
     int dp_band;
     int dp_band_risky;
     int dp_jf;
-    void* dp_items;
-    int* dbg;
+    Ptr<void> dp_items;
+    Ptr<int> dbg;
 };
+typedef DevBatchT<HostP> DevBatch;
+typedef DevBatchT<GlobP> DevBatchG;
+static_assert(sizeof(DevBatch) == sizeof(DevBatchG), "one layout");
+__device__ __forceinline__ const DevBatchG& dev_view(const DevBatch* p) { return *(const DevBatchG*)p; }
+enum { DESC_VALUE = 0, DESC_VIEW = 1, DESC_GENERIC = 2 };
+template <int FORM, class D> __device__ __forceinline__ decltype(auto) desc_of(const D& byValue, const D* inMemory)
+{
+    if constexpr (FORM == DESC_VIEW) return dev_view(inMemory);
+    else if constexpr (FORM == DESC_GENERIC) return (*inMemory);
+    else return (byValue);
+}
 
-__device__ __forceinline__ int ordered_chains(const DevBatch& B) { return B.chain_order ? __builtin_amdgcn_readfirstlane(B.order_hist[B.order_nb - 1]) : B.n_chains; }
+template <class BT> __device__ __forceinline__ int ordered_chains(const BT& B) { return B.chain_order ? __builtin_amdgcn_readfirstlane(B.order_hist[B.order_nb - 1]) : B.n_chains; }
 
-__device__ __forceinline__ size_t row_base(const DevBatch& B, int c) { return (size_t)(B.chain_row ? B.chain_row[c] : c) * (size_t)B.stride; }
+template <class BT> __device__ __forceinline__ size_t row_base(const BT& B, int c) { return (size_t)(B.chain_row ? B.chain_row[c] : c) * (size_t)B.stride; }
 
 enum { DPL_BAND16 = 0, DPL_BAND32 = 2, DPL_BAND64 = 4, DPL_JF = 6, DPL_GEN = 8, DPL_N = 10 };
 __host__ __device__ inline int dpl_of_class(int cls) { return cls == 0 ? DPL_GEN : (cls == 1 ? DPL_JF : (cls == 2 ? DPL_BAND16 : (cls == 3 ? DPL_BAND32 : DPL_BAND64))); }
diff --git a/hla-la_amd/csrc/device_common.h b/hla-la_amd/csrc/device_common.h
--- a/hla-la_amd/csrc/device_common.h
+++ b/hla-la_amd/csrc/device_common.h
@@ -7,39 +7,50 @@
 typedef unsigned long long u64;
 typedef unsigned int u32;
 
-struct DevGraph {
+#define HLALA_AS_GLOBAL __attribute__((address_space(1)))
+template <class T> using HostP = T*;
+#if defined(__HIP_DEVICE_COMPILE__)
+template <class T> using GlobP = HLALA_AS_GLOBAL T*;
+#else
+template <class T> using GlobP = T*;
+#endif
+
+template <template <class> class Ptr> struct DevGraphT {
     int L, N, E, P;
-    const int* level_off;
-    const int* node_level;
-    const int* node_orig;
-    const int* out_off;
-    const int* out_to;
-    const uint8_t* out_label;
-    const int* out_eid;
-    const int* in_off;
-    const int* in_from;
-    const uint8_t* in_label;
-    const int* in_eid;
-    const unsigned int* in_rec;
-    const uint8_t* level_fast;
-    const int* edge_from_new;
-    const int* edge_to_new;
-    const uint8_t* edge_label;
-    const int* jf_off; const int* jf_node; const int* jf_path; const int* jf_lvl;
-    const int* jb_off; const int* jb_node; const int* jb_path; const int* jb_lvl;
-    const uint8_t* out_prank; const uint8_t* in_prank; const uint8_t* jf_prank; const uint8_t* jb_prank;
-    const uint8_t* jfree_out; const uint8_t* jfree_in;
-    const u32* lin_label; const uint8_t* lin_out; const uint8_t* lin_in; const int* lin_eid;
-    const int4* nrec_out;
-    const int4* nrec_in;
-    const int* path_len;
-    const long long* path_off;
-    const int* path_edges;
-    const uint8_t* gap_stretch;
-    const long long* lp_off;
-    const int* lp_seqid;
-    const int* lp_pos;
+    Ptr<const int> level_off;
+    Ptr<const int> node_level;
+    Ptr<const int> node_orig;
+    Ptr<const int> out_off;
+    Ptr<const int> out_to;
+    Ptr<const uint8_t> out_label;
+    Ptr<const int> out_eid;
+    Ptr<const int> in_off;
+    Ptr<const int> in_from;
+    Ptr<const uint8_t> in_label;
+    Ptr<const int> in_eid;
+    Ptr<const unsigned int> in_rec;
+    Ptr<const uint8_t> level_fast;
+    Ptr<const int> edge_from_new;
+    Ptr<const int> edge_to_new;
+    Ptr<const uint8_t> edge_label;
+    Ptr<const int> jf_off; Ptr<const int> jf_node; Ptr<const int> jf_path; Ptr<const int> jf_lvl;
+    Ptr<const int> jb_off; Ptr<const int> jb_node; Ptr<const int> jb_path; Ptr<const int> jb_lvl;
+    Ptr<const uint8_t> out_prank; Ptr<const uint8_t> in_prank; Ptr<const uint8_t> jf_prank; Ptr<const uint8_t> jb_prank;
+    Ptr<const uint8_t> jfree_out; Ptr<const uint8_t> jfree_in;
+    Ptr<const u32> lin_label; Ptr<const uint8_t> lin_out; Ptr<const uint8_t> lin_in; Ptr<const int> lin_eid;
+    Ptr<const int4> nrec_out;
+    Ptr<const int4> nrec_in;
+    Ptr<const int> path_len;
+    Ptr<const long long> path_off;
+    Ptr<const int> path_edges;
+    Ptr<const uint8_t> gap_stretch;
+    Ptr<const long long> lp_off;
+    Ptr<const int> lp_seqid;
+    Ptr<const int> lp_pos;
 };
+typedef DevGraphT<HostP> DevGraph;
+typedef DevGraphT<GlobP> DevGraphG;
+static_assert(sizeof(DevGraph) == sizeof(DevGraphG), "one layout");
 
 struct DevTables {
     double ll_match[256];
@@ -67,7 +78,6 @@
 constexpr int DP_NEG       = -30000;
 
 __device__ __forceinline__ int lane_id() { return threadIdx.x & 63; }
-#define HLALA_AS_GLOBAL __attribute__((address_space(1)))
 template <class T> struct GPtr {
     typedef HLALA_AS_GLOBAL T GT;
     T* p;
@@ -80,6 +90,7 @@
     __device__ __forceinline__ operator GT*() const { return g(); }
 };
 template <class T> __device__ __forceinline__ HLALA_AS_GLOBAL T* glob(T* p) { return (HLALA_AS_GLOBAL T*)p; }
+__device__ __forceinline__ const DevGraphG& dev_view(const DevGraph* p) { return *(const DevGraphG*)p; }
 #define WSYNC() do { __builtin_amdgcn_fence(__ATOMIC_RELEASE, "wavefront"); __builtin_amdgcn_wave_barrier(); __builtin_amdgcn_fence(__ATOMIC_ACQUIRE, "wavefront"); } while(0)
 __device__ __forceinline__ int uni(int v) { return __builtin_amdgcn_readfirstlane(v); }
 __device__ __forceinline__ int next_work(int* counter)
diff --git a/hla-la_amd/csrc/hlala_api.hip b/hla-la_amd/csrc/hlala_api.hip
--- a/hla-la_amd/csrc/hlala_api.hip
+++ b/hla-la_amd/csrc/hlala_api.hip
@@ -845,14 +845,14 @@
         }
         int grid = B.n_chains < c->proj_grid ? B.n_chains : c->proj_grid;
         if(c->proj_long_slabs)
-            hipLaunchKernelGGL((k_project_chains<ProjLdsLong>), dim3(grid), dim3(64), 0, c->active, c->dG, b->dB, c->d_contig_off, c->d_contig_seq, c->d_contig_level,
+            hipLaunchKernelGGL((k_project_chains<ProjLdsLong>), dim3(grid), dim3(64), 0, c->active, c->G, b->B, c->dG, b->dB, c->d_contig_off, c->d_contig_seq, c->d_contig_level,
                                c->proj_slabs, c->proj_slab_bytes, c->proj_long_slabs, c->proj_long_slab_bytes, 0);
         else
             if(c->params.max_columns <= PROJ_CAP_SHORT)
-                hipLaunchKernelGGL((k_project_chains<ProjLdsShort>), dim3(grid), dim3(64), 0, c->active, c->dG, b->dB, c->d_contig_off, c->d_contig_seq, c->d_contig_level,
+                hipLaunchKernelGGL((k_project_chains<ProjLdsShort>), dim3(grid), dim3(64), 0, c->active, c->G, b->B, c->dG, b->dB, c->d_contig_off, c->d_contig_seq, c->d_contig_level,
                                    c->proj_slabs, c->proj_slab_bytes, (char*)nullptr, (size_t)0, c->rethread_slabs ? 1 : 0);
             else
-                hipLaunchKernelGGL((k_project_chains<ProjLds>), dim3(grid), dim3(64), 0, c->active, c->dG, b->dB, c->d_contig_off, c->d_contig_seq, c->d_contig_level,
+                hipLaunchKernelGGL((k_project_chains<ProjLds>), dim3(grid), dim3(64), 0, c->active, c->G, b->B, c->dG, b->dB, c->d_contig_off, c->d_contig_seq, c->d_contig_level,
                                c->proj_slabs, c->proj_slab_bytes, (char*)nullptr, (size_t)0, c->rethread_slabs ? 1 : 0);
         int rc = check_launch(c, "k_project_chains"); if(rc) return rc;
         if(c->rethread_slabs) {
@@ -895,10 +895,10 @@
         HIP_TRY(c, hipMemsetAsync(B.dp_alias_head, 0xFF, (size_t)2 * B.n_chains * sizeof(int), c->active));
         HIP_TRY(c, hipMemsetAsync(B.dp_alias_next, 0xFF, (size_t)2 * B.n_chains * sizeof(int), c->active));
         HIP_TRY(c, hipMemsetAsync(B.dp_blk, 0, ((size_t)DPL_N * B.dp_nblk + 1) * sizeof(int), c->active));
-        hipLaunchKernelGGL(k_dp_items, dim3(B.dp_nblk), dim3(256), 0, c->active, c->dG, b->dB, items);
+        hipLaunchKernelGGL(k_dp_items, dim3(B.dp_nblk), dim3(256), 0, c->active, c->G, b->B, items);
         rc = check_launch(c, "k_dp_items"); if(rc) return rc;
         hipLaunchKernelGGL(k_order_scan, dim3(1), dim3(ORDER_SCAN_THREADS), 0, c->active, B.dp_blk, DPL_N * B.dp_nblk + 1);
-        hipLaunchKernelGGL(k_dp_lists, dim3(B.dp_nblk), dim3(256), 0, c->active, b->dB, (const DpItem*)items);
+        hipLaunchKernelGGL(k_dp_lists, dim3(B.dp_nblk), dim3(256), 0, c->active, b->B, (const DpItem*)items);
         rc = check_launch(c, "k_dp_lists"); if(rc) return rc;
         }
         hipStream_t ws = c->active;
@@ -934,9 +934,9 @@
         b->band_used = c->band_grid > 0;
         if(b->band_used) {
             HIP_TRY(c, hipEventRecord(b->evBand[0], c->active));
-            hipLaunchKernelGGL((k_dp_band<16>), dim3(c->band_grid), dim3(64), 0, c->active, c->dG, b->dB, (const DpItem*)items, seed, (const uint8_t*)B.read_bases, c->G.lin_label, c->G.lin_eid);
-            hipLaunchKernelGGL((k_dp_band<32>), dim3(c->band_grid), dim3(64), 0, c->active, c->dG, b->dB, (const DpItem*)items, seed, (const uint8_t*)B.read_bases, c->G.lin_label, c->G.lin_eid);
-            hipLaunchKernelGGL((k_dp_band<64>), dim3(c->band_grid), dim3(64), 0, c->active, c->dG, b->dB, (const DpItem*)items, seed, (const uint8_t*)B.read_bases, c->G.lin_label, c->G.lin_eid);
+            hipLaunchKernelGGL((k_dp_band<16>), dim3(c->band_grid), dim3(64), 0, c->active, c->G, b->B, (const DpItem*)items, seed, (const uint8_t*)B.read_bases, c->G.lin_label, c->G.lin_eid);
+            hipLaunchKernelGGL((k_dp_band<32>), dim3(c->band_grid), dim3(64), 0, c->active, c->G, b->B, (const DpItem*)items, seed, (const uint8_t*)B.read_bases, c->G.lin_label, c->G.lin_eid);
+            hipLaunchKernelGGL((k_dp_band<64>), dim3(c->band_grid), dim3(64), 0, c->active, c->G, b->B, (const DpItem*)items, seed, (const uint8_t*)B.read_bases, c->G.lin_label, c->G.lin_eid);
             rc = check_launch(c, "k_dp_band"); if(rc) return rc;
             HIP_TRY(c, hipEventRecord(b->evBand[1], c->active));
         }
@@ -958,14 +958,14 @@
         if(fused && phase == 3) { b->side_pending = true; b->side_used = true; }
         if(fused && phase != 1 && phase != 3) {
             { const int pgrid = (B.n_pairs + 63) / 64, cap = c->stitch_grid / 20;
-              hipLaunchKernelGGL(k_stitch_chains, dim3(pgrid < cap ? (pgrid > 0 ? pgrid : 1) : cap), dim3(64), 0, c->side, c->dG, c->dT, b->dB, (const uint8_t*)B.pair_deferred, 2, 0, 0); }
+              hipLaunchKernelGGL(k_stitch_chains, dim3(pgrid < cap ? (pgrid > 0 ? pgrid : 1) : cap), dim3(64), 0, c->side, c->G, c->dT, b->B, (const uint8_t*)B.pair_deferred, 2, 0, 0); }
             rc = check_launch(c, "k_stitch_chains (side)"); if(rc) return rc;
             HIP_TRY(c, hipEventRecord(b->evDone, c->side));
             HIP_TRY(c, hipEventRecord(c->evSideTail, c->side)); c->sideTailValid = true;
             b->side_inflight = true; b->side_used = true; b->side_pending = true;
         }
         if(mainPart) {
-        hipLaunchKernelGGL(k_stitch_chains, dim3(sgrid), dim3(64), 0, c->active, c->dG, c->dT, b->dB, (const uint8_t*)B.pair_deferred, fused ? 1 : 0, c->stitch_draw, c->stitch_by_row);
+        hipLaunchKernelGGL(k_stitch_chains, dim3(sgrid), dim3(64), 0, c->active, c->G, c->dT, b->B, (const uint8_t*)B.pair_deferred, fused ? 1 : 0, c->stitch_draw, c->stitch_by_row);
         rc = check_launch(c, "k_stitch_chains"); if(rc) return rc;
         }
     }
@@ -1003,12 +1003,12 @@
             const int g0 = mode == 2 ? (grid < c->pair_grid / 5 ? grid : c->pair_grid / 5) : grid, g1 = grid < c->pair_grid / 5 ? grid : c->pair_grid / 5;
             if(B.unpaired) {
                 hipLaunchKernelGGL((k_pair_chains<true>), dim3(lean), dim3(64), 0, st, c->dG, c->dT, b->dB, (const uint8_t*)B.pair_deferred, mode, counterIdx, multiList, multiBase);
-                hipLaunchKernelGGL((k_pair_multi<true, false>), dim3(g0), dim3(64), 0, st, c->dG, c->dT, b->dB, (const int*)multiList, multiBase, scratch);
-                hipLaunchKernelGGL((k_pair_multi<true, true>), dim3(g1), dim3(64), 0, st, c->dG, c->dT, b->dB, (const int*)multiList, multiBase, scratch);
+                hipLaunchKernelGGL((k_pair_multi<true, false>), dim3(g0), dim3(64), 0, st, c->G, b->B, c->dG, c->dT, b->dB, (const int*)multiList, multiBase, scratch);
+                hipLaunchKernelGGL((k_pair_multi<true, true>), dim3(g1), dim3(64), 0, st, c->G, b->B, c->dG, c->dT, b->dB, (const int*)multiList, multiBase, scratch);
             } else {
                 hipLaunchKernelGGL((k_pair_chains<false>), dim3(lean), dim3(64), 0, st, c->dG, c->dT, b->dB, (const uint8_t*)B.pair_deferred, mode, counterIdx, multiList, multiBase);
-                hipLaunchKernelGGL((k_pair_multi<false, false>), dim3(g0), dim3(64), 0, st, c->dG, c->dT, b->dB, (const int*)multiList, multiBase, scratch);
-                hipLaunchKernelGGL((k_pair_multi<false, true>), dim3(g1), dim3(64), 0, st, c->dG, c->dT, b->dB, (const int*)multiList, multiBase, scratch);
+                hipLaunchKernelGGL((k_pair_multi<false, false>), dim3(g0), dim3(64), 0, st, c->G, b->B, c->dG, c->dT, b->dB, (const int*)multiList, multiBase, scratch);
+                hipLaunchKernelGGL((k_pair_multi<false, true>), dim3(g1), dim3(64), 0, st, c->G, b->B, c->dG, c->dT, b->dB, (const int*)multiList, multiBase, scratch);
             }
             return check_launch(c, "k_pair_chains / k_pair_multi");
         };
diff --git a/hla-la_amd/csrc/kernel_dp.hip b/hla-la_amd/csrc/kernel_dp.hip
--- a/hla-la_amd/csrc/kernel_dp.hip
+++ b/hla-la_amd/csrc/kernel_dp.hip
@@ -493,8 +493,8 @@
 
 #define DP_FAIL(code) do { if(gl == 0 && S.err == 0) S.err = (code); } while(0)
 
-template <class C>
-__device__ inline int dp_begin(DpLdsT<C>& S, const DpSlabT<C>& sl, const DevGraph& G, const DpItem& it, int itemIdx)
+template <class C, class DG>
+__device__ inline int dp_begin(DpLdsT<C>& S, const DpSlabT<C>& sl, const DG& G, const DpItem& it, int itemIdx)
 {
     constexpr int GW = C::GW;
     const int gl = grp_lane<GW>();
@@ -523,8 +523,8 @@
     return PH_RUN;
 }
 
-template <class C>
-__device__ inline int dp_iterate(DpLdsT<C>& S, const DpSlabT<C>& sl, const DevGraph& G, const int4* nrec, const uint8_t* readBases, const bool fwd, int& edgesAcc, u64* sortScratch)
+template <class C, class DG>
+__device__ inline int dp_iterate(DpLdsT<C>& S, const DpSlabT<C>& sl, const DG& G, const int4* nrec, const uint8_t* readBases, const bool fwd, int& edgesAcc, u64* sortScratch)
 {
     constexpr int GW = C::GW;
     const int gl = grp_lane<GW>();
@@ -1051,8 +1051,8 @@
     return PH_RUN;
 }
 
-template <class C>
-__device__ inline int dp_select_many(const DpSlabT<C>& sl, const DevGraph& G, int nCompleted, int best, int selectedIndex)
+template <class C, class DG>
+__device__ inline int dp_select_many(const DpSlabT<C>& sl, const DG& G, int nCompleted, int best, int selectedIndex)
 {
     constexpr int GW = C::GW;
     const int gl = grp_lane<GW>();
@@ -1077,8 +1077,8 @@
     return found;
 }
 
-template <class C>
-__device__ inline int dp_select(DpLdsT<C>& S, const DpSlabT<C>& sl, const DevGraph& G, u32 rng_seed, const bool fwd)
+template <class C, class DG>
+__device__ inline int dp_select(DpLdsT<C>& S, const DpSlabT<C>& sl, const DG& G, u32 rng_seed, const bool fwd)
 {
     constexpr int GW = C::GW;
     const int gl = grp_lane<GW>();
@@ -1196,8 +1196,8 @@
     return PH_BT;
 }
 
-template <class C>
-__device__ inline int dp_expand(DpLdsT<C>& S, const DpSlabT<C>& sl, const DevGraph& G, const DevBatch& B, const int4* nrec, const bool fwd)
+template <class C, class DG, class DB>
+__device__ inline int dp_expand(DpLdsT<C>& S, const DpSlabT<C>& sl, const DG& G, const DB& B, const int4* nrec, const bool fwd)
 {
     constexpr int GW = C::GW;
     const int gl = grp_lane<GW>();
@@ -1266,7 +1266,8 @@
     return PH_DONE;
 }
 
-__device__ inline bool dp_item_for(const DevGraph& G, const DevBatch& B, int c, int d, DpItem& it)
+template <class DG, class DB>
+__device__ inline bool dp_item_for(const DG& G, const DB& B, int c, int d, DpItem& it)
 {
     if(B.unpaired) return false;
     if(B.seed_status[c] != HLALA_CHAIN_OK) return false;
@@ -1292,10 +1293,8 @@
     return true;
 }
 
-__global__ void k_dp_items(const DevGraph* __restrict__ Gp, const DevBatch* __restrict__ Bp, DpItem* items)
-{
-    const DevGraph& G = *Gp;
-    const DevBatch& B = *Bp;
+__global__ void k_dp_items(const DevGraph G, const DevBatch B, DpItem* items)
+{
     const int t = blockIdx.x * blockDim.x + threadIdx.x;
     if(t < B.n_chains) {
         const int st = B.seed_status[t];
@@ -1374,9 +1373,8 @@
     if(threadIdx.x < DPL_N) B.dp_blk[(size_t)threadIdx.x * gridDim.x + blockIdx.x] = blkCnt[threadIdx.x];
 }
 
-__global__ void k_dp_lists(const DevBatch* __restrict__ Bp, const DpItem* __restrict__ items)
-{
-    const DevBatch& B = *Bp;
+__global__ void k_dp_lists(const DevBatch B, const DpItem* __restrict__ items)
+{
     const int t = blockIdx.x * blockDim.x + threadIdx.x;
     const int nOrd = ordered_chains(B);
     int kL = -1, kR = -1;
@@ -1416,9 +1414,11 @@
     const uint8_t* bases[DP_POOL_MAX];
 };
 
-template <class C, int TIER>
-__device__ __forceinline__ void dp_class_run(const DevGraph& G, const DevBatch& B, const DpItem* __restrict__ items, DpLdsT<C>& S, DpSlabT<C> sl, u64* sortScratch, const u32 rng_seed,
+template <class C, int TIER, class DG, class DB>
+__device__ __forceinline__ void dp_class_run(const DG& G, const DB& B, const DpItem* __restrict__ items, DpLdsT<C>& S, DpSlabT<C> sl, u64* sortScratch, const u32 rng_seed,
                                              const int4* __restrict__ nrecOut, const int4* __restrict__ nrecIn, const uint8_t* __restrict__ readBases);
+
+template <class C, int TIER> __host__ __device__ constexpr int dp_desc_form() { return ((TIER == 0 && C::JF) || TIER == 3 || TIER == 5) ? DESC_VIEW : DESC_GENERIC; }
 
 template <class C, int TIER>
 __global__ __launch_bounds__(C::THREADS, C::WAVES) void k_dp(const DevGraph* __restrict__ Gp, const DevBatch* __restrict__ Bp, const DpItem* __restrict__ items,
@@ -1428,7 +1428,8 @@
     constexpr int GW = C::GW;
     constexpr int NG = GW >= 64 ? 1 : 64 / GW;
     static_assert(C::THREADS == (GW >= 64 ? GW : 64), "block size");
-    const DevGraph& G = *Gp;
+    constexpr int FORM = dp_desc_form<C, TIER>();
+    const auto& G = desc_of<FORM>(*Gp, Gp);
     const int g = (int)((threadIdx.x & 63) / GW);
     DpLdsT<C>* Sp; DpSlabT<C> sl; u64* sortScratch = nullptr;
     if constexpr (C::IN_MEMORY) {
@@ -1442,14 +1443,14 @@
     if constexpr (TIER >= DP_POOL_TIER) {
         const int nB = __builtin_amdgcn_readfirstlane(pool.n);
         for(int bi = 0; bi < nB; bi++) {
-            dp_class_run<C, TIER>(G, *pool.B[bi], pool.items[bi], *Sp, sl, sortScratch, pool.seed[bi], nrecOut, nrecIn, pool.bases[bi]);
+            dp_class_run<C, TIER>(G, desc_of<FORM>(*pool.B[bi], pool.B[bi]), pool.items[bi], *Sp, sl, sortScratch, pool.seed[bi], nrecOut, nrecIn, pool.bases[bi]);
             DSYNC();
         }
-    } else dp_class_run<C, TIER>(G, *Bp, items, *Sp, sl, sortScratch, rng_seed, nrecOut, nrecIn, readBasesArg);
-}
-
-template <class C, int TIER>
-__device__ __forceinline__ void dp_class_run(const DevGraph& G, const DevBatch& B, const DpItem* __restrict__ items, DpLdsT<C>& S, DpSlabT<C> sl, u64* sortScratch, const u32 rng_seed,
+    } else dp_class_run<C, TIER>(G, desc_of<FORM>(*Bp, Bp), items, *Sp, sl, sortScratch, rng_seed, nrecOut, nrecIn, readBasesArg);
+}
+
+template <class C, int TIER, class DG, class DB>
+__device__ __forceinline__ void dp_class_run(const DG& G, const DB& B, const DpItem* __restrict__ items, DpLdsT<C>& S, DpSlabT<C> sl, u64* sortScratch, const u32 rng_seed,
                                              const int4* __restrict__ nrecOut, const int4* __restrict__ nrecIn, const uint8_t* __restrict__ readBases)
 {
     constexpr int GW = C::GW;
@@ -1589,8 +1590,8 @@
 #endif
 }
 
-template <int PER>
-__device__ __forceinline__ void stitch_rounds(const DevBatch& B, const DevTables& T, const size_t cb, const int rOff, const int total, const int padL, const int nL, const int nSeed,
+template <int PER, class DB>
+__device__ __forceinline__ void stitch_rounds(const DB& B, const DevTables& T, const size_t cb, const int rOff, const int total, const int padL, const int nL, const int nSeed,
                                               const int nR, const int newEnd, const int stride, const int lane, double& llOut, int& f0, int& f1, int& l0, int& l1)
 {
     const int seedAt = padL + nL, rightAt = seedAt + nSeed, padRAt = rightAt + nR;
@@ -1685,7 +1686,8 @@
     llOut = carry;
 }
 
-__device__ __forceinline__ void stitch_draw(const DevBatch& B, const DevTables& T, const uint8_t* __restrict__ deferPairs, const int deferMode, const int lane, const int cq,
+template <class DB>
+__device__ __forceinline__ void stitch_draw(const DB& B, const DevTables& T, const uint8_t* __restrict__ deferPairs, const int deferMode, const int lane, const int cq,
                                             u64& accChains, u64& accCols)
 {
     const int stride = B.stride;
@@ -1735,10 +1737,9 @@
     }
 }
 
-__global__ __launch_bounds__(64, 5) void k_stitch_chains(const DevGraph* __restrict__ Gp, const DevTables* __restrict__ Tp, const DevBatch* __restrict__ Bp,
+__global__ __launch_bounds__(64, 5) void k_stitch_chains(const DevGraph G, const DevTables* __restrict__ Tp, const DevBatch B,
                                                         const uint8_t* __restrict__ deferPairs, const int deferMode, const int draw, const int byRow)
 {
-    const DevBatch& B = *Bp;
     const DevTables& T = *Tp;
     const int lane = lane_id();
     u64 accChains = 0, accCols = 0;
diff --git a/hla-la_amd/csrc/kernel_dp_band.hip b/hla-la_amd/csrc/kernel_dp_band.hip
--- a/hla-la_amd/csrc/kernel_dp_band.hip
+++ b/hla-la_amd/csrc/kernel_dp_band.hip
@@ -33,8 +33,8 @@
 #define BAND_T(i) do { } while(0)
 #endif
 
-template <class C, bool FWD>
-__device__ __forceinline__ void band_pass(const DevGraph& G, const DevBatch& B, const DpItem* __restrict__ items, const u32 rng_seed, const uint8_t* __restrict__ readBases,
+template <class C, bool FWD, class DG, class DB>
+__device__ __forceinline__ void band_pass(const DG& G, const DB& B, const DpItem* __restrict__ items, const u32 rng_seed, const uint8_t* __restrict__ readBases,
                                           const u32* __restrict__ linLabel, const int* __restrict__ linEid, BandLds<C>& S,
                                           u64& accCalls, u64& accIters, u64& accCells, u64& accEdges)
 {
@@ -257,12 +257,10 @@
 }
 
 template <int GW>
-__global__ __launch_bounds__(64, BandCfg<GW>::WAVES) void k_dp_band(const DevGraph* __restrict__ Gp, const DevBatch* __restrict__ Bp, const DpItem* __restrict__ items, const u32 rng_seed,
+__global__ __launch_bounds__(64, BandCfg<GW>::WAVES) void k_dp_band(const DevGraph G, const DevBatch B, const DpItem* __restrict__ items, const u32 rng_seed,
                                                                     const uint8_t* __restrict__ readBases, const u32* __restrict__ linLabel, const int* __restrict__ linEid)
 {
     typedef BandCfg<GW> C;
-    const DevGraph& G = *Gp;
-    const DevBatch& B = *Bp;
     __shared__ BandLds<C> SS[64 / GW];
     BandLds<C>& S = SS[lane_id() / GW];
     u64 accCalls = 0, accIters = 0, accCells = 0, accEdges = 0;
diff --git a/hla-la_amd/csrc/kernel_pair.hip b/hla-la_amd/csrc/kernel_pair.hip
--- a/hla-la_amd/csrc/kernel_pair.hip
+++ b/hla-la_amd/csrc/kernel_pair.hip
@@ -45,7 +45,8 @@
     return (unsigned char)lo;
 }
 
-__device__ inline int lp_find(const DevGraph& G, int level, int id)
+template <class DG>
+__device__ inline int lp_find(const DG& G, int level, int id)
 {
     long long lo = G.lp_off[level], hi = G.lp_off[level + 1];
     while(lo < hi) {
@@ -56,7 +57,8 @@
     return -1;
 }
 
-__device__ inline double pair_insert_ll(const DevGraph& G, const DevTables& T, const int up0, const int up1, const int dn0, const int dn1)
+template <class DG>
+__device__ inline double pair_insert_ll(const DG& G, const DevTables& T, const int up0, const int up1, const int dn0, const int dn1)
 {
     const int lane = lane_id();
     {
@@ -87,7 +89,7 @@
             if(have) {
                 const long long d = (long long)beginPos - pos - 1;
                 const long long k = d - T.is_dmin;
-                best = (k >= 0 && k < T.is_n) ? T.is_logpdf[k] : T.is_penalty;
+                best = (k >= 0 && k < T.is_n) ? glob(T.is_logpdf)[k] : T.is_penalty;
             }
             for(int o = 32; o; o >>= 1) { const double ov = __shfl_xor(best, o); if(ov > best) best = ov; }
             return __ballot(have) ? best : T.is_penalty;
@@ -107,7 +109,7 @@
             if(beginPos < 0) continue;
             const long long d = (long long)beginPos - endPos - 1;
             const long long k = d - T.is_dmin;
-            const double v = (k >= 0 && k < T.is_n) ? T.is_logpdf[k] : T.is_penalty;
+            const double v = (k >= 0 && k < T.is_n) ? glob(T.is_logpdf)[k] : T.is_penalty;
             if(!have || v > best) { best = v; have = true; }
         }
     }
@@ -157,7 +159,8 @@
 }
 
 struct PairChain { int4 fl; int rev, nk, row; double ll; };
-__device__ __forceinline__ PairChain pair_chain_load(const DevBatch& B, const int c)
+template <class DB>
+__device__ __forceinline__ PairChain pair_chain_load(const DB& B, const int c)
 {
     PairChain x;
     x.fl = *(const int4*)(B.ext_firstlast + 4 * (size_t)c); x.rev = B.chain_reverse[c]; x.ll = B.ext_ll[c]; x.nk = B.ext_ncols[c]; x.row = B.chain_row ? B.chain_row[c] : c;
@@ -173,8 +176,8 @@
     return y;
 }
 
-template <bool UNPAIRED, int PER>
-__device__ __forceinline__ void pair_positions(const DevBatch& B, PairLds& P, const double* __restrict__ LL, const int p, const int n1, const int n2, const int nComb,
+template <bool UNPAIRED, int PER, class DB>
+__device__ __forceinline__ void pair_positions(const DB& B, PairLds& P, const double* __restrict__ LL, const int p, const int n1, const int n2, const int nComb,
                                                const int best1, const int best2, const PairChain& cA, const PairChain& cB, const int lane, const int stride)
 {
     constexpr int NM = UNPAIRED ? 1 : 2;
@@ -275,8 +278,8 @@
 #define PAIR_T(i) do { } while(0)
 #endif
 
-template <bool UNPAIRED, bool BIG>
-__device__ __forceinline__ void pair_finish(const DevGraph& G, const DevTables& T, const DevBatch& B, PairLds& P, double* __restrict__ LL,
+template <bool UNPAIRED, bool BIG, class DG, class DB>
+__device__ __forceinline__ void pair_finish(const DG& G, const DevTables& T, const DB& B, PairLds& P, double* __restrict__ LL,
                                             const int p, const int n1, const int n2, const int nComb, const int mxc, const PairChain& cA, const PairChain& cB, const int lane, const int stride, long long* tAcc, long long& tMark)
 {
     constexpr int NM = UNPAIRED ? 1 : 2;
@@ -354,8 +357,8 @@
 #endif
 }
 
-template <bool UNPAIRED>
-__device__ __forceinline__ int pair_lists(const DevBatch& B, PairListLds& L, const int* cLo, const int* cHi, const int lane, int& n1, int& n2, int& mxcOut, PairChain* cL)
+template <bool UNPAIRED, class DB>
+__device__ __forceinline__ int pair_lists(const DB& B, PairListLds& L, const int* cLo, const int* cHi, const int lane, int& n1, int& n2, int& mxcOut, PairChain* cL)
 {
     constexpr int NM = UNPAIRED ? 1 : 2;
     int bad = 0;
@@ -479,11 +482,11 @@
 }
 
 template <bool UNPAIRED, bool BIG>
-__global__ __launch_bounds__(64, BIG ? 3 : PAIR_MULTI_WAVES) void k_pair_multi(const DevGraph* __restrict__ Gp, const DevTables* __restrict__ Tp, const DevBatch* __restrict__ Bp,
+__global__ __launch_bounds__(64, BIG ? 3 : PAIR_MULTI_WAVES) void k_pair_multi(const DevGraph Gv, const DevBatch Bv, const DevGraph* __restrict__ Gp, const DevTables* __restrict__ Tp, const DevBatch* __restrict__ Bp,
                                                   const int* __restrict__ multiList, const int multiBase, double* __restrict__ bigLL)
 {
-    const DevGraph& G = *Gp;
-    const DevBatch& B = *Bp;
+    const auto& G = desc_of<BIG ? DESC_GENERIC : DESC_VALUE>(Gv, Gp);
+    const auto& B = desc_of<BIG ? DESC_GENERIC : DESC_VALUE>(Bv, Bp);
     __shared__ PairLds P;
     const int lane = lane_id();
     const DevTables& T = *Tp;
diff --git a/hla-la_amd/csrc/kernel_project.hip b/hla-la_amd/csrc/kernel_project.hip
--- a/hla-la_amd/csrc/kernel_project.hip
+++ b/hla-la_amd/csrc/kernel_project.hip
@@ -181,12 +181,12 @@
 #define HLALA_PROJ_WPS 2
 #endif
 template <class PL>
-__global__ __launch_bounds__(64, PL::LONG ? HLALA_PROJ_LONG_WPS : HLALA_PROJ_WPS) void k_project_chains(const DevGraph* __restrict__ Gp, const DevBatch* __restrict__ Bp, const long long* contig_off, const uint8_t* contig_seq,
+__global__ __launch_bounds__(64, PL::LONG ? HLALA_PROJ_LONG_WPS : HLALA_PROJ_WPS) void k_project_chains(const DevGraph Gv, const DevBatch Bv, const DevGraph* __restrict__ Gp, const DevBatch* __restrict__ Bp, const long long* contig_off, const uint8_t* contig_seq,
                                                        const int* contig_level, char* slabs, size_t slabBytes, char* longSlabs, size_t longSlabBytes,
                                                        int deferRethread)
 {
-    const DevGraph& G = *Gp;
-    const DevBatch& B = *Bp;
+    const auto& G = desc_of<PL::LONG ? DESC_VIEW : DESC_VALUE>(Gv, Gp);
+    const auto& B = desc_of<PL::LONG ? DESC_VIEW : DESC_VALUE>(Bv, Bp);
     __shared__ PL P;
     const int lane = lane_id();
     if(PL::LONG) { if(lane == 0) proj_bind(P, longSlabs + (size_t)blockIdx.x * longSlabBytes); WSYNC(); }
@@ -1275,8 +1275,8 @@
 
 __global__ __launch_bounds__(64, 6) void k_rethread_chains(const DevGraph* __restrict__ Gp, const DevBatch* __restrict__ Bp, char* slabs, size_t slabBytes)
 {
-    const DevGraph& G = *Gp;
-    const DevBatch& B = *Bp;
+    const DevGraphG& G = dev_view(Gp);
+    const DevBatchG& B = dev_view(Bp);
     __shared__ RethreadLds P;
     const int lane = lane_id();
     u32* const ch = (u32*)(slabs + (size_t)blockIdx.x * slabBytes);
```

Measured after the change: 5.653 million (median of 6 runs). 1.7% higher.
